# Weepingchestnut/SAVSR

Measured on NVIDIA B200. Metric: hr_mpix_per_s, higher is better.
Workload: dtype bf16

## Files before the change

### include/savsr_b200.h

```cpp
#ifndef SAVSR_B200_H_
#define SAVSR_B200_H_

#include <stddef.h>
#include <stdint.h>

#ifdef __cplusplus
extern "C" {
#endif

#define SAVSR_ABI_VERSION 4
#define SAVSR_MAX_SRC 5
#define SAVSR_MAX_GROUPS 25
#define SAVSR_TILE_W 8
#define SAVSR_TILE_H 16

typedef struct savsr_ctx savsr_ctx;
typedef struct savsr_arena savsr_arena;
typedef void* savsr_stream;

enum savsr_format { SAVSR_FMT_BF16 = 0, SAVSR_FMT_FP16 = 1 };
enum savsr_row_order { SAVSR_ROWS_LINEAR = 0, SAVSR_ROWS_QUAD = 1 };

enum savsr_act { SAVSR_ACT_NONE = 0, SAVSR_ACT_LRELU = 1, SAVSR_ACT_RELU = 2 };

enum savsr_dst_mode {
  SAVSR_DST_ARENA = 0,
  SAVSR_DST_AUX16 = 1
};

enum savsr_conv_impl {
  SAVSR_IMPL_TCGEN05_TAP = 0,
  SAVSR_IMPL_TCGEN05_HALO = 1,
  SAVSR_IMPL_CHECK = 2
};

typedef struct savsr_conv_group {
  int32_t src_slot[SAVSR_MAX_SRC];
  int32_t nsrc;
  int32_t dst_slot;
  int32_t res1_slot;
  int32_t res2_slot;
  float res2_scale;
  int32_t act;
  float slope;
  const void* weight;
  int64_t weight_sample_stride;
  const float* bias;
  const float* mask;
  float* pool;
  void* aux_dst;
  int32_t src_channels;
  int32_t reserved_;
} savsr_conv_group;

enum savsr_option {
  SAVSR_OPT_BIGK_ALL = 0,
  SAVSR_OPT_BIGK_ISSUERS = 1,
  SAVSR_OPT_PDL = 2,
  SAVSR_OPT_COUNT = 3
};

int savsr_abi_version(void);
const char* savsr_last_error(void);
int savsr_ctx_create(int device, savsr_ctx** out);
void savsr_ctx_destroy(savsr_ctx* ctx);
int savsr_ctx_sm_count(const savsr_ctx* ctx);
int savsr_ctx_set_format(savsr_ctx* ctx, int format);
int savsr_ctx_get_format(const savsr_ctx* ctx);
int savsr_ctx_set_option(savsr_ctx* ctx, int option, int value);
int savsr_ctx_get_option(const savsr_ctx* ctx, int option);

size_t savsr_arena_bytes(int nslots, int batch, int height, int width);
int savsr_arena_create(savsr_ctx* ctx, void* base, int nslots, int batch, int height, int width,
                       savsr_arena** out);
void savsr_arena_destroy(savsr_arena* a);
int savsr_arena_tiles(const savsr_arena* a);
int savsr_arena_import(savsr_arena* a, int slot, const float* nchw, savsr_stream st);
int savsr_arena_export(savsr_arena* a, int slot, float* nchw, savsr_stream st);

size_t savsr_packed_weight_bytes(int co, int ci, int ksize);
int savsr_pack_conv_weight(const float* w_oihw, int co_real, int co, int ci, int ksize, int n_tile,
                           int format , int row_order ,
                           void* packed, savsr_stream st);

int savsr_conv(savsr_ctx* ctx, savsr_arena* arena, const savsr_conv_group* groups, int ngroups,
               int ksize, int n_tile, int dst_mode, int impl, savsr_stream st);

int savsr_pack_frames(savsr_ctx* ctx, savsr_arena* arena, const float* x, int t, int h, int w, int dst_slot,
                      savsr_stream st);

int savsr_conv_wgrad(savsr_ctx* ctx, const void* x3_nchw16, const void* dy_nchw16, int batch, int ci, int height, int width,
                     int pitch, int per_sample, float* dw, savsr_stream st);

typedef struct savsr_axpby {
  int32_t dst_slot, x_slot, y_slot;
  float alpha, beta;
} savsr_axpby;
int savsr_slot_axpby(savsr_ctx* ctx, savsr_arena* arena, const savsr_axpby* entries, int n, savsr_stream st);

typedef struct savsr_grad_prep_entry {
  int32_t dv_slot, out_slot, g_slot, gt_tslot;
  int32_t act;
  float slope;
  const float* cscale; int64_t cscale_stride;
  const float* cadd; int64_t cadd_stride; float cadd_mul;
  int32_t reserved_;
  float* dbias;
} savsr_grad_prep_entry;
int savsr_grad_prep(savsr_ctx* ctx, savsr_arena* arena, void* tbase, int ntslots, int pitch, const savsr_grad_prep_entry* entries, int n,
                    savsr_stream st);

typedef struct savsr_nchw3 { int32_t x_slot, t_slot; } savsr_nchw3;
int savsr_slot_to_nchw3(savsr_ctx* ctx, savsr_arena* arena, void* tbase, int ntslots, int pitch, const savsr_nchw3* entries, int n,
                        savsr_stream st);

typedef struct savsr_pack_chunk {
  const float* w;
  void* dst;
  int32_t co_total, ci_total, o_base, i_base, ksize, transposed;
} savsr_pack_chunk;
int savsr_pack_conv_chunks(savsr_ctx* ctx, const savsr_pack_chunk* chunks_dev, int first, int count, savsr_stream st);

enum savsr_wgrad_layout {
  SAVSR_WGRAD_OIHW = 0,
  SAVSR_WGRAD_TIO = 1
};
typedef struct savsr_wgrad_item {
  int32_t x_tslot, g_tslot;
  float* dw;
  int32_t ci_total, ci_off, o_off, ksize, per_sample, layout;
  int64_t sample_stride;
} savsr_wgrad_item;
int savsr_conv_wgrad_batched(savsr_ctx* ctx, const void* tbase, int ntslots, int batch, int height, int width, int pitch,
                             const savsr_wgrad_item* items_dev, int first, int count, savsr_stream st);

int savsr_adam_ema(savsr_ctx* ctx, float* param, const float* grad, float* exp_avg, float* exp_avg_sq, float* ema, long n, float lr,
                   float beta1, float beta2, float eps, const float* step_dev, float ema_decay, float grad_scale, savsr_stream st);

typedef struct savsr_osa_params {
  int32_t ci, co, att;
  const float* bank;
  const float* r0_w; const float* r0_b;
  const float* r2_w; const float* r2_b;
  const float* fc_w;
  const float* bn_scale; const float* bn_shift;
  const float* ch_w; const float* ch_b;
  const float* fl_w; const float* fl_b;
  const float* sp_w; const float* sp_b;
  const float* kn_w; const float* kn_b;
  const float* pool[SAVSR_MAX_SRC];
  float* scratch;
  void* packed;
} savsr_osa_params;
int savsr_osa_prologue(savsr_ctx* ctx, const savsr_osa_params* convs, int nconvs, int batch,
                       int npart, int npix, float inv_scale_h, float inv_scale_w, savsr_stream st);

typedef struct savsr_osa_train {
  const float* bn_weight; const float* bn_bias;
  float* running_mean; float* running_var;
  float momentum, eps;
  float* state;
  void* packed_t;
} savsr_osa_train;
typedef struct savsr_osa_grads {
  float* dwfold;
  float* d_bank;
  float* d_r0_w; float* d_r0_b; float* d_r2_w; float* d_r2_b;
  float* d_fc_w; float* d_bn_w; float* d_bn_b;
  float* d_ch_w; float* d_ch_b; float* d_fl_w; float* d_fl_b; float* d_sp_w; float* d_sp_b; float* d_kn_w; float* d_kn_b;
  float* datt; float* dvec; float* dpool;
} savsr_osa_grads;
size_t savsr_osa_train_state_floats(int batch);
size_t savsr_osa_train_dvec_floats(int batch, int ci);
int savsr_osa_prologue_train(savsr_ctx* ctx, const savsr_osa_params* convs, const savsr_osa_train* extra, int nconvs, int batch,
                             int npart, int npix, float inv_scale_h, float inv_scale_w, savsr_stream st);
int savsr_osa_fold_backward(savsr_ctx* ctx, const savsr_osa_params* convs, const savsr_osa_train* extra, const savsr_osa_grads* grads,
                            int nconvs, int batch, savsr_stream st);

int savsr_slot_channel_dot(savsr_ctx* ctx, savsr_arena* arena, int a_slot, int b_slot, float* out, savsr_stream st);
int savsr_ca_backward(savsr_ctx* ctx, const float* pool, int npart, int npix, int batch, const float* w1, const float* b1, const float* w2,
                      const float* b2, const float* y, float* dy, float* dw1, float* db1, float* dw2, float* db2, float* dmean,
                      savsr_stream st);

typedef struct savsr_mask_train {
  const float *w4, *b4, *w7, *b7, *w11, *b11;
  const float* bn_w[4]; const float* bn_b[4];
  float* bn_rm[4]; float* bn_rv[4];
  const float* gamma;
  float momentum, eps;
  float *m0, *t2, *m4, *t3, *m7, *t5, *m11, *mask;
  float* stat; double* sums; float* coef;
  float *d_w4, *d_b4, *d_w7, *d_b7, *d_w11, *d_b11;
  float* d_bn_w[4]; float* d_bn_b[4];
  float* d_gamma;
  float *dmask, *dm11, *dt4, *dm7, *dt3, *dm4, *dt2;
} savsr_mask_train;
int savsr_mask_forward_train(savsr_ctx* ctx, savsr_arena* arena, const savsr_mask_train* m, int r_slot, int a_slot, int share_slot, int out_slot,
                             savsr_stream st);
int savsr_mask_backward_train(savsr_ctx* ctx, savsr_arena* arena, const savsr_mask_train* m, int dh_slot, int a_slot, int share_slot, int da_slot,
                              int gshare_slot, int dm0_slot, savsr_stream st);

int savsr_sta_lrelu_forward(savsr_ctx* ctx, const float* x, const float* kpre, float* out, int batch, int channels, int height, int width,
                            float slope, savsr_stream st);
int savsr_sta_lrelu_backward(savsr_ctx* ctx, const float* x, const float* kpre, const float* dout, float* dx, float* dkpre, int batch, int channels,
                             int height, int width, float slope, savsr_stream st);

int savsr_ca_scale_residual(savsr_ctx* ctx, savsr_arena* arena, int t_slot, int x_slot, int dst_slot,
                            const float* pool, int npart, const float* w1, const float* b1,
                            const float* w2, const float* b2, float* y_scratch , savsr_stream st);

int savsr_osadapt_mask(savsr_ctx* ctx, const float* in16, int batch, int height, int width,
                       const float* wa, const float* ba, const float* wb, const float* bb,
                       const float* wc, const float* bc, float* half0, float* half1, float* mask,
                       savsr_stream st);

typedef struct savsr_satu_weights {
  const float* body0_w; const float* body0_b;
  const float* body2_w; const float* body2_b;
  const float* routing_w; const float* routing_b;
  const float* offset_w; const float* offset_b;
  const float* st_offset_w; const float* st_offset_b;
  const float* compress;
  const float* expand;
} savsr_satu_weights;

int savsr_satu_index(savsr_ctx* ctx, const savsr_satu_weights* wts, int h, int w, int H, int W,
                     float s_h, float s_w, float* rel_y, float* rel_x, int32_t* cell_y,
                     int32_t* cell_x, float* base_y, float* base_x, int32_t* corner_y,
                     int32_t* corner_x, float* table, savsr_stream st);

int savsr_satu_kconv_sta(savsr_ctx* ctx, savsr_arena* arena, int a_slot, int x_slot, int dst_slot, int h, int w,
                         const void* weights, const float* bias, float slope, savsr_stream st);

int savsr_satu_hr(savsr_ctx* ctx, savsr_arena* lr, int x_slot, int sta_slot, int h, int w, int H, int W,
                  const float* table, const float* base_y, const float* base_x, const void* weights,
                  const float* zbias, const float* tail_bias, const float* x_in, int t, int centre, float* out,
                  savsr_stream st);

typedef struct savsr_plan savsr_plan;
int savsr_plan_create(savsr_ctx* ctx, savsr_plan** out);
void savsr_plan_destroy(savsr_plan* plan);
int savsr_plan_size(const savsr_plan* plan);
int savsr_plan_set_io(savsr_plan* plan, float* x_in, size_t x_bytes, float* out, size_t out_bytes, int format );
int savsr_plan_add_pack_frames(savsr_plan* plan, savsr_arena* arena, const float* x, int t, int h, int w, int dst_slot);
int savsr_plan_add_conv(savsr_plan* plan, savsr_arena* arena, const savsr_conv_group* groups, int ngroups, int ksize, int n_tile,
                        int dst_mode, int impl);
int savsr_plan_add_osa_prologue(savsr_plan* plan, const savsr_osa_params* convs, int nconvs, int batch, int npart, int npix,
                                float inv_scale_h, float inv_scale_w);
int savsr_plan_add_ca_scale_residual(savsr_plan* plan, savsr_arena* arena, int t_slot, int x_slot, int dst_slot, const float* pool, int npart,
                                     const float* w1, const float* b1, const float* w2, const float* b2, float* y_scratch);
int savsr_plan_add_osadapt_mask(savsr_plan* plan, const float* in16, int batch, int height, int width, const float* wa, const float* ba,
                                const float* wb, const float* bb, const float* wc, const float* bc, float* half0, float* half1, float* mask);
int savsr_plan_add_satu_kconv_sta(savsr_plan* plan, savsr_arena* arena, int a_slot, int x_slot, int dst_slot, int h, int w, const void* weights,
                                  const float* bias, float slope);
int savsr_plan_add_satu_hr(savsr_plan* plan, savsr_arena* lr, int x_slot, int sta_slot, int h, int w, int H, int W, const float* table,
                           const float* base_y, const float* base_x, const void* weights, const float* zbias, const float* tail_bias,
                           const float* x_in, int t, int centre, float* out);
int savsr_plan_add_arena_export(savsr_plan* plan, savsr_arena* arena, int slot, float* nchw);
int savsr_plan_run(savsr_plan* plan, savsr_stream st);
int savsr_forward(savsr_plan* plan, const float* x, float* out, savsr_stream st);

int savsr_img_metrics_blocks(const savsr_ctx* ctx, int height, int width);
int savsr_img_metrics(savsr_ctx* ctx, const float* sr, const float* gt, int batch, int height, int width,
                      uint8_t* bgr_u8, double* sse_y, savsr_stream st);

int savsr_ssim_y_blocks(int height, int width);
int savsr_ssim_y(savsr_ctx* ctx, const float* sr, const float* gt, int batch, int height, int width,
                 double* partials, savsr_stream st);

int savsr_aa_max_taps(int in_size, int out_size);
int savsr_aa_table(savsr_ctx* ctx, int in_size, int out_size, int max_taps, int32_t* xmin, int32_t* xsize,
                   float* weights, int32_t* overflow_flag, savsr_stream st);
int savsr_lr_synthesize(savsr_ctx* ctx, const uint8_t* frames_bgr, int nframes, int height, int width,
                        int crop_h, int crop_w, int out_h, int out_w,
                        const int32_t* xmin_w, const int32_t* xsize_w, const float* weights_w, int taps_w,
                        const int32_t* xmin_h, const int32_t* xsize_h, const float* weights_h, int taps_h,
                        float* tmp, float* lr, float* gt, savsr_stream st);
int savsr_resize_aa(savsr_ctx* ctx, const float* src, int nframes, int height, int width, int out_h, int out_w,
                    const int32_t* xmin_w, const int32_t* xsize_w, const float* weights_w, int taps_w,
                    const int32_t* xmin_h, const int32_t* xsize_h, const float* weights_h, int taps_h,
                    float* tmp, float* dst, savsr_stream st);

#ifdef __cplusplus
}
#endif
#endif
```

### savsr_b200/_capi.py

```python
from __future__ import annotations

import ctypes as C
import os
from typing import Optional

ABI_VERSION = 4
MAX_SRC = 5
MAX_GROUPS = 25
TILE_W, TILE_H = 8, 16

ACT_NONE, ACT_LRELU, ACT_RELU = 0, 1, 2
DST_ARENA, DST_AUX16 = 0, 1
IMPL_TAP, IMPL_HALO, IMPL_CHECK = 0, 1, 2
IMPL_NAMES = {"tap": IMPL_TAP, "halo": IMPL_HALO, "check": IMPL_CHECK}
FMT_BF16, FMT_FP16 = 0, 1
FMT_NAMES = {"bf16": FMT_BF16, "fp16": FMT_FP16}
OPT_BIGK_ALL, OPT_BIGK_ISSUERS, OPT_PDL = 0, 1, 2
WGRAD_OIHW, WGRAD_TIO = 0, 1
ROWS_LINEAR, ROWS_QUAD = 0, 1

LIB_PATH = os.environ.get("SAVSR_LIB_PATH") or os.path.join(os.path.dirname(os.path.abspath(__file__)), "lib", "libsavsr_sm100.so")


class SavsrError(RuntimeError):
    """A libsavsr_sm100 call returned non-zero."""


class ConvGroup(C.Structure):
    _fields_ = [
        ("src_slot", C.c_int32 * MAX_SRC),
        ("nsrc", C.c_int32),
        ("dst_slot", C.c_int32),
        ("res1_slot", C.c_int32),
        ("res2_slot", C.c_int32),
        ("res2_scale", C.c_float),
        ("act", C.c_int32),
        ("slope", C.c_float),
        ("weight", C.c_void_p),
        ("weight_sample_stride", C.c_int64),
        ("bias", C.c_void_p),
        ("mask", C.c_void_p),
        ("pool", C.c_void_p),
        ("aux_dst", C.c_void_p),
        ("src_channels", C.c_int32),
        ("reserved_", C.c_int32),
    ]


class OsaParams(C.Structure):
    _fields_ = [
        ("ci", C.c_int32), ("co", C.c_int32), ("att", C.c_int32),
        ("bank", C.c_void_p),
        ("r0_w", C.c_void_p), ("r0_b", C.c_void_p), ("r2_w", C.c_void_p), ("r2_b", C.c_void_p),
        ("fc_w", C.c_void_p), ("bn_scale", C.c_void_p), ("bn_shift", C.c_void_p),
        ("ch_w", C.c_void_p), ("ch_b", C.c_void_p), ("fl_w", C.c_void_p), ("fl_b", C.c_void_p),
        ("sp_w", C.c_void_p), ("sp_b", C.c_void_p), ("kn_w", C.c_void_p), ("kn_b", C.c_void_p),
        ("pool", C.c_void_p * MAX_SRC),
        ("scratch", C.c_void_p),
        ("packed", C.c_void_p),
    ]


class SatuWeights(C.Structure):
    _fields_ = [(n, C.c_void_p) for n in (
        "body0_w", "body0_b", "body2_w", "body2_b", "routing_w", "routing_b", "offset_w", "offset_b",
        "st_offset_w", "st_offset_b", "compress", "expand")]


class Axpby(C.Structure):
    _fields_ = [("dst_slot", C.c_int32), ("x_slot", C.c_int32), ("y_slot", C.c_int32), ("alpha", C.c_float), ("beta", C.c_float)]


class GradPrep(C.Structure):
    _fields_ = [("dv_slot", C.c_int32), ("out_slot", C.c_int32), ("g_slot", C.c_int32), ("gt_tslot", C.c_int32),
                ("act", C.c_int32), ("slope", C.c_float),
                ("cscale", C.c_void_p), ("cscale_stride", C.c_int64),
                ("cadd", C.c_void_p), ("cadd_stride", C.c_int64), ("cadd_mul", C.c_float), ("reserved_", C.c_int32),
                ("dbias", C.c_void_p)]


class Nchw3(C.Structure):
    _fields_ = [("x_slot", C.c_int32), ("t_slot", C.c_int32)]


class PackChunk(C.Structure):
    _fields_ = [("w", C.c_void_p), ("dst", C.c_void_p), ("co_total", C.c_int32), ("ci_total", C.c_int32), ("o_base", C.c_int32),
                ("i_base", C.c_int32), ("ksize", C.c_int32), ("transposed", C.c_int32)]


class WgradItem(C.Structure):
    _fields_ = [("x_tslot", C.c_int32), ("g_tslot", C.c_int32), ("dw", C.c_void_p), ("ci_total", C.c_int32), ("ci_off", C.c_int32),
                ("o_off", C.c_int32), ("ksize", C.c_int32), ("per_sample", C.c_int32), ("layout", C.c_int32),
                ("sample_stride", C.c_int64)]


class OsaTrain(C.Structure):
    _fields_ = [("bn_weight", C.c_void_p), ("bn_bias", C.c_void_p), ("running_mean", C.c_void_p), ("running_var", C.c_void_p),
                ("momentum", C.c_float), ("eps", C.c_float), ("state", C.c_void_p), ("packed_t", C.c_void_p)]


class OsaGrads(C.Structure):
    _fields_ = [(n, C.c_void_p) for n in (
        "dwfold", "d_bank", "d_r0_w", "d_r0_b", "d_r2_w", "d_r2_b", "d_fc_w", "d_bn_w", "d_bn_b", "d_ch_w", "d_ch_b", "d_fl_w", "d_fl_b",
        "d_sp_w", "d_sp_b", "d_kn_w", "d_kn_b", "datt", "dvec", "dpool")]


class MaskTrain(C.Structure):
    _fields_ = ([(n, C.c_void_p) for n in ("w4", "b4", "w7", "b7", "w11", "b11")]
                + [("bn_w", C.c_void_p * 4), ("bn_b", C.c_void_p * 4), ("bn_rm", C.c_void_p * 4), ("bn_rv", C.c_void_p * 4),
                   ("gamma", C.c_void_p), ("momentum", C.c_float), ("eps", C.c_float)]
                + [(n, C.c_void_p) for n in ("m0", "t2", "m4", "t3", "m7", "t5", "m11", "mask", "stat", "sums", "coef",
                                             "d_w4", "d_b4", "d_w7", "d_b7", "d_w11", "d_b11")]
                + [("d_bn_w", C.c_void_p * 4), ("d_bn_b", C.c_void_p * 4), ("d_gamma", C.c_void_p)]
                + [(n, C.c_void_p) for n in ("dmask", "dm11", "dt4", "dm7", "dt3", "dm4", "dt2")])

MAX_TRAIN_ENTRIES = 32


_VP, _I, _F, _SZ = C.c_void_p, C.c_int, C.c_float, C.c_size_t
SIGNATURES = {
    "savsr_abi_version": (_I, []),
    "savsr_last_error": (C.c_char_p, []),
    "savsr_ctx_create": (_I, [_I, C.POINTER(_VP)]),
    "savsr_ctx_destroy": (None, [_VP]),
    "savsr_ctx_sm_count": (_I, [_VP]),
    "savsr_ctx_set_format": (_I, [_VP, _I]),
    "savsr_ctx_get_format": (_I, [_VP]),
    "savsr_ctx_set_option": (_I, [_VP, _I, _I]),
    "savsr_ctx_get_option": (_I, [_VP, _I]),
    "savsr_arena_bytes": (_SZ, [_I, _I, _I, _I]),
    "savsr_arena_create": (_I, [_VP, _VP, _I, _I, _I, _I, C.POINTER(_VP)]),
    "savsr_arena_destroy": (None, [_VP]),
    "savsr_arena_tiles": (_I, [_VP]),
    "savsr_arena_import": (_I, [_VP, _I, _VP, _VP]),
    "savsr_arena_export": (_I, [_VP, _I, _VP, _VP]),
    "savsr_packed_weight_bytes": (_SZ, [_I, _I, _I]),
    "savsr_pack_conv_weight": (_I, [_VP, _I, _I, _I, _I, _I, _I, _I, _VP, _VP]),
    "savsr_conv": (_I, [_VP, _VP, C.POINTER(ConvGroup), _I, _I, _I, _I, _I, _VP]),
    "savsr_conv_wgrad": (_I, [_VP, _VP, _VP, _I, _I, _I, _I, _I, _I, _VP, _VP]),
    "savsr_slot_axpby": (_I, [_VP, _VP, C.POINTER(Axpby), _I, _VP]),
    "savsr_grad_prep": (_I, [_VP, _VP, _VP, _I, _I, C.POINTER(GradPrep), _I, _VP]),
    "savsr_slot_to_nchw3": (_I, [_VP, _VP, _VP, _I, _I, C.POINTER(Nchw3), _I, _VP]),
    "savsr_pack_conv_chunks": (_I, [_VP, _VP, _I, _I, _VP]),
    "savsr_conv_wgrad_batched": (_I, [_VP, _VP, _I, _I, _I, _I, _I, _VP, _I, _I, _VP]),
    "savsr_adam_ema": (_I, [_VP, _VP, _VP, _VP, _VP, _VP, C.c_long, _F, _F, _F, _F, _VP, _F, _F, _VP]),
    "savsr_osa_train_state_floats": (_SZ, [_I]),
    "savsr_osa_train_dvec_floats": (_SZ, [_I, _I]),
    "savsr_osa_prologue_train": (_I, [_VP, C.POINTER(OsaParams), C.POINTER(OsaTrain), _I, _I, _I, _I, _F, _F, _VP]),
    "savsr_osa_fold_backward": (_I, [_VP, C.POINTER(OsaParams), C.POINTER(OsaTrain), C.POINTER(OsaGrads), _I, _I, _VP]),
    "savsr_slot_channel_dot": (_I, [_VP, _VP, _I, _I, _VP, _VP]),
    "savsr_ca_backward": (_I, [_VP, _VP, _I, _I, _I] + [_VP] * 11 + [_VP]),
    "savsr_mask_forward_train": (_I, [_VP, _VP, C.POINTER(MaskTrain), _I, _I, _I, _I, _VP]),
    "savsr_mask_backward_train": (_I, [_VP, _VP, C.POINTER(MaskTrain), _I, _I, _I, _I, _I, _I, _VP]),
    "savsr_sta_lrelu_forward": (_I, [_VP, _VP, _VP, _VP, _I, _I, _I, _I, _F, _VP]),
    "savsr_sta_lrelu_backward": (_I, [_VP, _VP, _VP, _VP, _VP, _VP, _I, _I, _I, _I, _F, _VP]),
    "savsr_plan_create": (_I, [_VP, C.POINTER(_VP)]),
    "savsr_plan_destroy": (None, [_VP]),
    "savsr_plan_size": (_I, [_VP]),
    "savsr_plan_set_io": (_I, [_VP, _VP, _SZ, _VP, _SZ, _I]),
    "savsr_plan_add_pack_frames": (_I, [_VP, _VP, _VP, _I, _I, _I, _I]),
    "savsr_plan_add_conv": (_I, [_VP, _VP, C.POINTER(ConvGroup), _I, _I, _I, _I, _I]),
    "savsr_plan_add_osa_prologue": (_I, [_VP, C.POINTER(OsaParams), _I, _I, _I, _I, _F, _F]),
    "savsr_plan_add_ca_scale_residual": (_I, [_VP, _VP, _I, _I, _I, _VP, _I, _VP, _VP, _VP, _VP, _VP]),
    "savsr_plan_add_osadapt_mask": (_I, [_VP, _VP, _I, _I, _I, _VP, _VP, _VP, _VP, _VP, _VP, _VP, _VP, _VP]),
    "savsr_plan_add_satu_kconv_sta": (_I, [_VP, _VP, _I, _I, _I, _I, _I, _VP, _VP, _F]),
    "savsr_plan_add_satu_hr": (_I, [_VP, _VP, _I, _I, _I, _I, _I, _I, _VP, _VP, _VP, _VP, _VP, _VP, _VP, _I, _I, _VP]),
    "savsr_plan_add_arena_export": (_I, [_VP, _VP, _I, _VP]),
    "savsr_plan_run": (_I, [_VP, _VP]),
    "savsr_forward": (_I, [_VP, _VP, _VP, _VP]),
    "savsr_pack_frames": (_I, [_VP, _VP, _VP, _I, _I, _I, _I, _VP]),
    "savsr_osa_prologue": (_I, [_VP, C.POINTER(OsaParams), _I, _I, _I, _I, _F, _F, _VP]),
    "savsr_ca_scale_residual": (_I, [_VP, _VP, _I, _I, _I, _VP, _I, _VP, _VP, _VP, _VP, _VP, _VP]),
    "savsr_osadapt_mask": (_I, [_VP, _VP, _I, _I, _I, _VP, _VP, _VP, _VP, _VP, _VP, _VP, _VP, _VP, _VP]),
    "savsr_satu_index": (_I, [_VP, C.POINTER(SatuWeights), _I, _I, _I, _I, _F, _F] + [_VP] * 9 + [_VP]),
    "savsr_satu_kconv_sta": (_I, [_VP, _VP, _I, _I, _I, _I, _I, _VP, _VP, _F, _VP]),
    "savsr_satu_hr": (_I, [_VP, _VP, _I, _I, _I, _I, _I, _I, _VP, _VP, _VP, _VP, _VP, _VP, _VP, _I, _I, _VP, _VP]),
    "savsr_img_metrics_blocks": (_I, [_VP, _I, _I]),
    "savsr_img_metrics": (_I, [_VP, _VP, _VP, _I, _I, _I, _VP, _VP, _VP]),
    "savsr_ssim_y_blocks": (_I, [_I, _I]),
    "savsr_ssim_y": (_I, [_VP, _VP, _VP, _I, _I, _I, _VP, _VP]),
    "savsr_aa_max_taps": (_I, [_I, _I]),
    "savsr_aa_table": (_I, [_VP, _I, _I, _I, _VP, _VP, _VP, _VP, _VP]),
    "savsr_lr_synthesize": (_I, [_VP, _VP, _I, _I, _I, _I, _I, _I, _I, _VP, _VP, _VP, _I, _VP, _VP, _VP, _I, _VP, _VP, _VP, _VP]),
    "savsr_resize_aa": (_I, [_VP, _VP, _I, _I, _I, _I, _I, _VP, _VP, _VP, _I, _VP, _VP, _VP, _I, _VP, _VP, _VP]),
}

_lib: Optional[C.CDLL] = None


def load() -> C.CDLL:
    global _lib
    if _lib is not None:
        return _lib
    if not os.path.exists(LIB_PATH):
        raise SavsrError(
            f"{LIB_PATH} not found: build it with `python -m savsr_b200.build` (needs nvcc, sm_100a). "
            "savsr_b200 has no CPU or PyTorch fallback.")
    lib = C.CDLL(LIB_PATH)
    for name, (res, args) in SIGNATURES.items():
        fn = getattr(lib, name)
        fn.restype = res
        fn.argtypes = args
    if lib.savsr_abi_version() != ABI_VERSION:
        raise SavsrError(f"ABI version mismatch: library {lib.savsr_abi_version()}, binding {ABI_VERSION}")
    _lib = lib
    return lib


def check(rc: int) -> None:
    if rc != 0:
        msg = load().savsr_last_error()
        raise SavsrError(f"libsavsr_sm100 error {rc}: {msg.decode(errors='replace') if msg else '?'}")


class Context:

    def __init__(self, device: int):
        self.lib = load()
        h = C.c_void_p()
        check(self.lib.savsr_ctx_create(int(device), C.byref(h)))
        self.handle = h
        self.device = int(device)
        self.sm_count = self.lib.savsr_ctx_sm_count(h)

    def set_option(self, option: int, value: int) -> None:
        check(self.lib.savsr_ctx_set_option(self.handle, int(option), int(value)))

    def set_format(self, fmt: int) -> None:
        check(self.lib.savsr_ctx_set_format(self.handle, int(fmt)))

    def __del__(self):
        try:
            if getattr(self, "handle", None):
                self.lib.savsr_ctx_destroy(self.handle)
                self.handle = None
        except Exception:
            pass


class Arena:

    def __init__(self, ctx: Context, base_ptr: int, nslots: int, batch: int, height: int, width: int):
        self.ctx = ctx
        self.lib = ctx.lib
        h = C.c_void_p()
        check(self.lib.savsr_arena_create(ctx.handle, C.c_void_p(base_ptr), nslots, batch, height, width, C.byref(h)))
        self.handle = h
        self.nslots, self.batch, self.height, self.width = nslots, batch, height, width
        self.tiles = self.lib.savsr_arena_tiles(h)

    def __del__(self):
        try:
            if getattr(self, "handle", None):
                self.lib.savsr_arena_destroy(self.handle)
                self.handle = None
        except Exception:
            pass


class CPlan:

    def __init__(self, ctx: Context):
        self.lib = ctx.lib
        h = C.c_void_p()
        check(self.lib.savsr_plan_create(ctx.handle, C.byref(h)))
        self.handle = h

    def __len__(self) -> int:
        return int(self.lib.savsr_plan_size(self.handle))

    def __del__(self):
        try:
            if getattr(self, "handle", None):
                self.lib.savsr_plan_destroy(self.handle)
                self.handle = None
        except Exception:
            pass
```

### savsr_b200/csrc/capi.cu

```cuda
#include <cstdarg>
#include <cstdio>
#include <cstdlib>
#include <cstring>

#include "common.cuh"

namespace savsr {

static thread_local char g_err[512] = "";

void set_error(const char* fmt, ...) {
  va_list ap;
  va_start(ap, fmt);
  vsnprintf(g_err, sizeof(g_err), fmt, ap);
  va_end(ap);
}

int cuda_fail(cudaError_t e, const char* what) {
  set_error("CUDA error %d (%s) at %s", static_cast<int>(e), cudaGetErrorString(e), what);
  return 2;
}

typedef CUresult (*EncodeTiledFn)(CUtensorMap*, CUtensorMapDataType, cuuint32_t, void*, const cuuint64_t*, const cuuint64_t*,
                                  const cuuint32_t*, const cuuint32_t*, CUtensorMapInterleave, CUtensorMapSwizzle,
                                  CUtensorMapL2promotion, CUtensorMapFloatOOBfill);

static int encode_map(savsr_ctx* ctx, CUtensorMap* tm, void* base, int nimg, int height, int width, int bw, int bh) {
  const cuuint64_t dims[4] = {64, static_cast<cuuint64_t>(width), static_cast<cuuint64_t>(height), static_cast<cuuint64_t>(nimg)};
  const cuuint64_t strides[3] = {128, static_cast<cuuint64_t>(width) * 128, static_cast<cuuint64_t>(height) * width * 128};
  const cuuint32_t box[4] = {64, static_cast<cuuint32_t>(bw), static_cast<cuuint32_t>(bh), 1};
  const cuuint32_t estr[4] = {1, 1, 1, 1};
  const CUresult r = reinterpret_cast<EncodeTiledFn>(ctx->encode_tiled)(
      tm, CU_TENSOR_MAP_DATA_TYPE_UINT16, 4, base, dims, strides, box, estr, CU_TENSOR_MAP_INTERLEAVE_NONE,
      CU_TENSOR_MAP_SWIZZLE_128B, CU_TENSOR_MAP_L2_PROMOTION_L2_256B, CU_TENSOR_MAP_FLOAT_OOB_FILL_NONE);
  if (r != CUDA_SUCCESS) {
    set_error("cuTensorMapEncodeTiled failed with CUresult %d (images %d, %dx%d, box %dx%d)", static_cast<int>(r), nimg, height,
              width, bw, bh);
    return 3;
  }
  return 0;
}

}

using namespace savsr;

extern "C" int savsr_abi_version(void) { return SAVSR_ABI_VERSION; }
extern "C" const char* savsr_last_error(void) { return g_err; }

extern "C" int savsr_ctx_create(int device, savsr_ctx** out) {
  SAVSR_REQUIRE(out, "savsr_ctx_create: null output pointer");
  *out = nullptr;
  int count = 0;
  SAVSR_CUDA(cudaGetDeviceCount(&count));
  SAVSR_REQUIRE(device >= 0 && device < count, "savsr_ctx_create: device %d not present (%d CUDA devices)", device, count);
  cudaDeviceProp prop;
  SAVSR_CUDA(cudaGetDeviceProperties(&prop, device));
  SAVSR_REQUIRE(prop.major == 10, "savsr_ctx_create: device %d is sm_%d%d; this library contains sm_100a code only "
                "(tcgen05/TMEM/TMA) and has no fallback", device, prop.major, prop.minor);
  DeviceGuard guard(device);
  void* fn = nullptr;
  cudaDriverEntryPointQueryResult qres;
  SAVSR_CUDA(cudaGetDriverEntryPoint("cuTensorMapEncodeTiled", &fn, cudaEnableDefault, &qres));
  SAVSR_REQUIRE(qres == cudaDriverEntryPointSuccess && fn, "savsr_ctx_create: driver lacks cuTensorMapEncodeTiled");
  savsr_ctx* c = static_cast<savsr_ctx*>(calloc(1, sizeof(savsr_ctx)));
  SAVSR_REQUIRE(c, "savsr_ctx_create: out of host memory");
  c->device = device;
  c->sm_count = prop.multiProcessorCount;
  c->cc_major = prop.major;
  c->cc_minor = prop.minor;
  c->encode_tiled = fn;
  c->opt[SAVSR_OPT_BIGK_ALL] = 1;
  c->opt[SAVSR_OPT_BIGK_ISSUERS] = 2;
  *out = c;
  return 0;
}

extern "C" int savsr_ctx_set_format(savsr_ctx* ctx, int format) {
  SAVSR_REQUIRE(ctx, "savsr_ctx_set_format: null context");
  SAVSR_REQUIRE(format == SAVSR_FMT_BF16 || format == SAVSR_FMT_FP16, "savsr_ctx_set_format: unknown format %d", format);
  ctx->fmt = format;
  return 0;
}
extern "C" int savsr_ctx_get_format(const savsr_ctx* ctx) { return ctx ? ctx->fmt : -1; }

extern "C" int savsr_ctx_set_option(savsr_ctx* ctx, int option, int value) {
  SAVSR_REQUIRE(ctx, "savsr_ctx_set_option: null context");
  SAVSR_REQUIRE(option >= 0 && option < SAVSR_OPT_COUNT, "savsr_ctx_set_option: unknown option %d", option);
  if (option == SAVSR_OPT_BIGK_ALL) SAVSR_REQUIRE(value == 0 || value == 1, "savsr_ctx_set_option: BIGK_ALL must be 0 or 1, got %d", value);
  if (option == SAVSR_OPT_BIGK_ISSUERS) SAVSR_REQUIRE(value == 1 || value == 2, "savsr_ctx_set_option: BIGK_ISSUERS must be 1 or 2, got %d", value);
  if (option == SAVSR_OPT_PDL) SAVSR_REQUIRE(value == 0 || value == 1, "savsr_ctx_set_option: PDL must be 0 or 1, got %d", value);
  ctx->opt[option] = value;
  return 0;
}
extern "C" int savsr_ctx_get_option(const savsr_ctx* ctx, int option) {
  return (ctx && option >= 0 && option < SAVSR_OPT_COUNT) ? ctx->opt[option] : -1;
}

extern "C" void savsr_ctx_destroy(savsr_ctx* ctx) { free(ctx); }
extern "C" int savsr_ctx_sm_count(const savsr_ctx* ctx) { return ctx ? ctx->sm_count : 0; }

extern "C" size_t savsr_arena_bytes(int nslots, int batch, int height, int width) {
  if (nslots <= 0 || batch <= 0 || height <= 0 || width <= 0) return 0;
  return static_cast<size_t>(nslots) * batch * height * width * kC * sizeof(__nv_bfloat16);
}

extern "C" int savsr_arena_create(savsr_ctx* ctx, void* base, int nslots, int batch, int height, int width, savsr_arena** out) {
  SAVSR_REQUIRE(ctx && out, "savsr_arena_create: null pointer");
  *out = nullptr;
  DeviceGuard guard(ctx->device);
  SAVSR_REQUIRE(base && (reinterpret_cast<uintptr_t>(base) & 255) == 0, "savsr_arena_create: base must be a 256-byte aligned device pointer");
  SAVSR_REQUIRE(nslots > 0 && batch > 0 && height > 0 && width > 0, "savsr_arena_create: empty arena (%d slots, batch %d, %dx%d)", nslots,
                batch, height, width);
  savsr_arena* a = static_cast<savsr_arena*>(calloc(1, sizeof(savsr_arena)));
  SAVSR_REQUIRE(a, "savsr_arena_create: out of host memory");
  a->ctx = ctx;
  a->base = static_cast<__nv_bfloat16*>(base);
  a->nslots = nslots; a->batch = batch; a->height = height; a->width = width;
  a->tiles_x = (width + kTileW - 1) / kTileW;
  a->tiles_y = (height + kTileH - 1) / kTileH;
  int rc = encode_map(ctx, &a->tm_tile, base, nslots * batch, height, width, kTileW, kTileH);
  if (rc == 0) rc = encode_map(ctx, &a->tm_halo, base, nslots * batch, height, width, kTileW + 2, kTileH + 2);
  if (rc != 0) { free(a); return rc; }
  *out = a;
  return 0;
}

extern "C" void savsr_arena_destroy(savsr_arena* a) { free(a); }
extern "C" int savsr_arena_tiles(const savsr_arena* a) { return a ? a->tiles_x * a->tiles_y : 0; }
```

### savsr_b200/csrc/conv_igemm.cu

```cuda
#include <cstdio>
#include <cstdlib>

#include "common.cuh"

namespace savsr {

#ifdef SAVSR_DEBUG_COUNTERS
#define DBG_CLOCK() clock64()
#define DBG_ONLY(...) __VA_ARGS__
#else
#define DBG_CLOCK() 0ll
#define DBG_ONLY(...)
#endif

constexpr int kMaxAStages = 4;
constexpr int kHaloPitch = 10;
constexpr int kHaloStageBytes = 23552;
constexpr int kARegionBytes = 3 * kHaloStageBytes;
constexpr int kBBlocks = 18;
constexpr int kRing = 3;
constexpr int kEpiWarps = 8;
constexpr int kNumThreads = 64 + 32 * kEpiWarps;

struct ConvParams {
  CUtensorMap tm_tile;
  CUtensorMap tm_halo;
  savsr_conv_group g[SAVSR_MAX_GROUPS];
  __nv_bfloat16* arena;
  int ngroups, batch, height, width, tiles_x, tiles_y;
  int ntaps;
  int nsrc;
  int halo;
  int n_res;
  int chunk;
  uint32_t per_sample_mask;
  long long* dbg;
  int dst_mode;
  int fmt;
  int issuers;
  int ksteps;
};

__device__ __forceinline__ float apply_act(float v, int act, float slope) {
  if (act == SAVSR_ACT_LRELU) return v > 0.f ? v : v * slope;
  if (act == SAVSR_ACT_RELU) return fmaxf(v, 0.f);
  return v;
}

template <int NC>
struct EpiCtx {
  float bias[NC];
  uint4 r1[NC / 8], r2[NC / 8];
  float mk;
  long pix;
  bool valid;
  int bias_group;
  float neg_slope;
  float res2_scale;
  int res1_slot, res2_slot, dst_slot;
  bool has_mask;
  float* pool;
};

template <int NC>
__device__ __forceinline__ void epi_prefetch(const ConvParams& p, const savsr_conv_group& g, int gi, int n, int tile, int quad,
                                             int lane, int col0, EpiCtx<NC>& c) {
  const int tx = tile % p.tiles_x, ty = tile / p.tiles_x;
  const int m = quad * 32 + lane;
  const int px = tx * kTileW + (m & (kTileW - 1));
  const int py = ty * kTileH + (m >> 3);
  c.valid = (px < p.width) && (py < p.height);
  const long npix = static_cast<long>(p.height) * p.width;
  c.pix = static_cast<long>(py) * p.width + px;
  if (gi != c.bias_group) {
    c.bias_group = gi;
    c.neg_slope = g.act == SAVSR_ACT_NONE ? 1.f : (g.act == SAVSR_ACT_RELU ? 0.f : g.slope);
    c.res2_scale = g.res2_scale;
    c.res1_slot = g.res1_slot; c.res2_slot = g.res2_slot; c.dst_slot = g.dst_slot;
    c.has_mask = g.mask != nullptr;
    c.pool = g.pool;
    if (g.bias != nullptr) {
      const float4* b4 = reinterpret_cast<const float4*>(g.bias + col0);
#pragma unroll
      for (int j = 0; j < NC / 4; ++j) {
        const float4 b = __ldg(b4 + j);
        c.bias[4 * j + 0] = b.x; c.bias[4 * j + 1] = b.y; c.bias[4 * j + 2] = b.z; c.bias[4 * j + 3] = b.w;
      }
    } else {
#pragma unroll
      for (int j = 0; j < NC; ++j) c.bias[j] = 0.f;
    }
  }
  if constexpr (NC == 32) {
    c.mk = (c.has_mask && c.valid) ? __ldg(g.mask + n * npix + c.pix) : 0.f;
    if (c.res1_slot >= 0 && c.valid) {
      const uint4* r = reinterpret_cast<const uint4*>(p.arena + ((static_cast<long>(c.res1_slot) * p.batch + n) * npix + c.pix) * kC + col0);
#pragma unroll
      for (int j = 0; j < NC / 8; ++j) c.r1[j] = r[j];
    }
    if (c.res2_slot >= 0 && c.valid) {
      const uint4* r = reinterpret_cast<const uint4*>(p.arena + ((static_cast<long>(c.res2_slot) * p.batch + n) * npix + c.pix) * kC + col0);
#pragma unroll
      for (int j = 0; j < NC / 8; ++j) c.r2[j] = r[j];
    }
  }
}

__device__ __forceinline__ void add_h16x8(float* v, const uint4& u, float s, int fmt) {
  v[0] += s * h_lo(u.x, fmt); v[1] += s * h_hi(u.x, fmt); v[2] += s * h_lo(u.y, fmt); v[3] += s * h_hi(u.y, fmt);
  v[4] += s * h_lo(u.z, fmt); v[5] += s * h_hi(u.z, fmt); v[6] += s * h_lo(u.w, fmt); v[7] += s * h_hi(u.w, fmt);
}

template <int NC>
__device__ __forceinline__ void epi_finish(const ConvParams& p, const savsr_conv_group& g, int n, int tile, int quad, int lane,
                                           float (&v)[NC], int col0, const EpiCtx<NC>& c) {
  const long npix = static_cast<long>(p.height) * p.width;
  const float ns = c.neg_slope;
#pragma unroll
  for (int j = 0; j < NC; ++j) {
    const float t = v[j] + c.bias[j];
    v[j] = fmaxf(t, ns * t);
  }
  if constexpr (NC == 32) {
    if (c.has_mask) {
#pragma unroll
      for (int j = 0; j < NC; ++j) v[j] *= c.mk;
    }
    if (c.res1_slot >= 0 && c.valid) {
#pragma unroll
      for (int j = 0; j < NC / 8; ++j) add_h16x8(v + 8 * j, c.r1[j], 1.f, p.fmt);
    }
    if (c.res2_slot >= 0 && c.valid) {
      const float r2s = c.res2_scale;
#pragma unroll
      for (int j = 0; j < NC / 8; ++j) add_h16x8(v + 8 * j, c.r2[j], r2s, p.fmt);
    }
    if (c.valid) {
      uint4* d = reinterpret_cast<uint4*>(p.arena + ((static_cast<long>(c.dst_slot) * p.batch + n) * npix + c.pix) * kC + col0);
#pragma unroll
      for (int j = 0; j < NC / 8; ++j) {
        uint4 u;
        u.x = pack_h2(v[8 * j + 0], v[8 * j + 1], p.fmt);
        u.y = pack_h2(v[8 * j + 2], v[8 * j + 3], p.fmt);
        u.z = pack_h2(v[8 * j + 4], v[8 * j + 5], p.fmt);
        u.w = pack_h2(v[8 * j + 6], v[8 * j + 7], p.fmt);
        d[j] = u;
      }
    }
    if (c.pool != nullptr) {
      if (!c.valid) {
#pragma unroll
        for (int j = 0; j < NC; ++j) v[j] = 0.f;
      }
#pragma unroll
      for (int off = 16, cnt = 16; off >= 1; off >>= 1, cnt >>= 1) {
        const bool upper = (lane & off) != 0;
#pragma unroll
        for (int i = 0; i < cnt; ++i) {
          const float send = upper ? v[i] : v[i + cnt];
          const float keep = upper ? v[i + cnt] : v[i];
          v[i] = keep + __shfl_xor_sync(0xffffffffu, send, off);
        }
      }
      const int npart = p.tiles_x * p.tiles_y * 4;
      c.pool[(static_cast<long>(n) * npart + tile * 4 + quad) * kC + col0 + lane] = v[0];
    }
  } else {
    if (c.valid) {
      float4* d = reinterpret_cast<float4*>(static_cast<float*>(g.aux_dst) + (n * npix + c.pix) * 16);
#pragma unroll
      for (int j = 0; j < 4; ++j) d[j] = make_float4(v[4 * j], v[4 * j + 1], v[4 * j + 2], v[4 * j + 3]);
    }
  }
}


struct EpiQuad {
  float bias[8];
  uint4 r1[4], r2[4];
  float mk[4];
  long pix0;
  uint32_t valid;
  int bias_group;
  float neg_slope, res2_scale;
  int res1_slot, res2_slot, dst_slot;
  bool has_mask;
  float* pool;
  float psum[8];
};

__device__ __forceinline__ void epiq_prefetch(const ConvParams& p, const savsr_conv_group& g, int gi, int n, int tile, int quad,
                                              int lane, int half, EpiQuad& c) {
  const int tx = tile % p.tiles_x, ty = tile / p.tiles_x;
  const int px = tx * kTileW + (lane >> 2);
  const int py0 = ty * kTileH + quad * 4;
  const int rows = p.height - py0;
  c.valid = (px < p.width && rows > 0) ? (rows >= 4 ? 0xfu : ((1u << rows) - 1u)) : 0u;
  const long npix = static_cast<long>(p.height) * p.width;
  c.pix0 = static_cast<long>(py0) * p.width + px;
  const int ch0 = half * 32 + (lane & 3) * 8;
  if (gi != c.bias_group) {
    c.bias_group = gi;
    c.neg_slope = g.act == SAVSR_ACT_NONE ? 1.f : (g.act == SAVSR_ACT_RELU ? 0.f : g.slope);
    c.res2_scale = g.res2_scale;
    c.res1_slot = g.res1_slot; c.res2_slot = g.res2_slot; c.dst_slot = g.dst_slot;
    c.has_mask = g.mask != nullptr;
    c.pool = g.pool;
    if (g.bias != nullptr) {
      const float4 b0 = __ldg(reinterpret_cast<const float4*>(g.bias + ch0));
      const float4 b1 = __ldg(reinterpret_cast<const float4*>(g.bias + ch0) + 1);
      c.bias[0] = b0.x; c.bias[1] = b0.y; c.bias[2] = b0.z; c.bias[3] = b0.w;
      c.bias[4] = b1.x; c.bias[5] = b1.y; c.bias[6] = b1.z; c.bias[7] = b1.w;
    } else {
#pragma unroll
      for (int j = 0; j < 8; ++j) c.bias[j] = 0.f;
    }
  }
  if (c.has_mask) {
#pragma unroll
    for (int j = 0; j < 4; ++j) c.mk[j] = ((c.valid >> j) & 1u) ? __ldg(g.mask + n * npix + c.pix0 + j * p.width) : 0.f;
  }
  if (c.res1_slot >= 0) {
    const __nv_bfloat16* r = p.arena + ((static_cast<long>(c.res1_slot) * p.batch + n) * npix + c.pix0) * kC + ch0;
#pragma unroll
    for (int j = 0; j < 4; ++j)
      if ((c.valid >> j) & 1u) c.r1[j] = *reinterpret_cast<const uint4*>(r + static_cast<long>(j) * p.width * kC);
  }
  if (c.res2_slot >= 0) {
    const __nv_bfloat16* r = p.arena + ((static_cast<long>(c.res2_slot) * p.batch + n) * npix + c.pix0) * kC + ch0;
#pragma unroll
    for (int j = 0; j < 4; ++j)
      if ((c.valid >> j) & 1u) c.r2[j] = *reinterpret_cast<const uint4*>(r + static_cast<long>(j) * p.width * kC);
  }
}

template <class Release, class Next>
__device__ __forceinline__ void epiq_finish(const ConvParams& p, int n, int tile, int quad, int lane, int half, uint32_t taddr,
                                            EpiQuad& c, bool last_of_run, Release release, Next next) {
  uint32_t ra[16], rb[16];
  tmem_ld_16x256b_x4(taddr, ra);
  tmem_ld_16x256b_x4(taddr + (16u << 16), rb);
  tmem_ld_wait();
  tc_fence_before();
  __syncwarp();
  release();
  float v[4][8];
#pragma unroll
  for (int k = 0; k < 4; ++k) {
#pragma unroll
    for (int e = 0; e < 4; ++e) {
      v[e >> 1][2 * k + (e & 1)] = __uint_as_float(ra[4 * k + e]);
      v[2 + (e >> 1)][2 * k + (e & 1)] = __uint_as_float(rb[4 * k + e]);
    }
  }
  const long npix = static_cast<long>(p.height) * p.width;
  const int ch0 = half * 32 + (lane & 3) * 8;
  const float ns = c.neg_slope;
#pragma unroll
  for (int j = 0; j < 4; ++j) {
#pragma unroll
    for (int i = 0; i < 8; ++i) {
      const float t = v[j][i] + c.bias[i];
      v[j][i] = fmaxf(t, ns * t);
    }
  }
  if (c.has_mask) {
#pragma unroll
    for (int j = 0; j < 4; ++j) {
#pragma unroll
      for (int i = 0; i < 8; ++i) v[j][i] *= c.mk[j];
    }
  }
  if (c.res1_slot >= 0) {
#pragma unroll
    for (int j = 0; j < 4; ++j)
      if ((c.valid >> j) & 1u) add_h16x8(v[j], c.r1[j], 1.f, p.fmt);
  }
  if (c.res2_slot >= 0) {
    const float r2s = c.res2_scale;
#pragma unroll
    for (int j = 0; j < 4; ++j)
      if ((c.valid >> j) & 1u) add_h16x8(v[j], c.r2[j], r2s, p.fmt);
  }
  const uint32_t valid = c.valid;
  float* const pool = c.pool;
  __nv_bfloat16* d = p.arena + ((static_cast<long>(c.dst_slot) * p.batch + n) * npix + c.pix0) * kC + ch0;
  next();
#pragma unroll
  for (int j = 0; j < 4; ++j) {
    if ((valid >> j) & 1u) {
      uint4 u;
      u.x = pack_h2(v[j][0], v[j][1], p.fmt);
      u.y = pack_h2(v[j][2], v[j][3], p.fmt);
      u.z = pack_h2(v[j][4], v[j][5], p.fmt);
      u.w = pack_h2(v[j][6], v[j][7], p.fmt);
      *reinterpret_cast<uint4*>(d + static_cast<long>(j) * p.width * kC) = u;
    }
  }
  if (pool != nullptr) {
    if (valid == 0xfu) {
#pragma unroll
      for (int i = 0; i < 8; ++i) c.psum[i] += (v[0][i] + v[1][i]) + (v[2][i] + v[3][i]);
    } else {
#pragma unroll
      for (int i = 0; i < 8; ++i) {
        const float a0 = (valid & 1u) ? v[0][i] : 0.f, a1 = (valid & 2u) ? v[1][i] : 0.f;
        const float a2 = (valid & 4u) ? v[2][i] : 0.f, a3 = (valid & 8u) ? v[3][i] : 0.f;
        c.psum[i] += (a0 + a1) + (a2 + a3);
      }
    }
    const int npart = p.tiles_x * p.tiles_y * 4;
    const int ch = ch0 + ((lane >> 4) & 1) * 4 + ((lane >> 3) & 1) * 2 + ((lane >> 2) & 1);
    float total = 0.f;
    if (last_of_run) {
      float s[8];
#pragma unroll
      for (int i = 0; i < 8; ++i) { s[i] = c.psum[i]; c.psum[i] = 0.f; }
#pragma unroll
      for (int off = 16, cnt = 4; off >= 4; off >>= 1, cnt >>= 1) {
        const bool upper = (lane & off) != 0;
#pragma unroll
        for (int i = 0; i < cnt; ++i) {
          const float send = upper ? s[i] : s[i + cnt];
          const float keep = upper ? s[i + cnt] : s[i];
          s[i] = keep + __shfl_xor_sync(0xffffffffu, send, off);
        }
      }
      total = s[0];
    }
    pool[(static_cast<long>(n) * npart + tile * 4 + quad) * kC + ch] = total;
  }
}

__device__ __forceinline__ constexpr uint32_t desc_hi(uint32_t sbo_bytes) { return (sbo_bytes >> 4) | (1u << 14) | (2u << 29); }
__device__ __forceinline__ uint64_t make_desc(uint32_t hi, uint32_t lo) { return (static_cast<uint64_t>(hi) << 32) | lo; }

template <int BN, int KS, bool HALO>
__global__ void __launch_bounds__(kNumThreads, 1) conv_igemm_kernel(const __grid_constant__ ConvParams p) {
  constexpr int NT = KS * KS;
  extern __shared__ uint8_t smem_raw[];
  uint8_t* smem = reinterpret_cast<uint8_t*>((reinterpret_cast<uintptr_t>(smem_raw) + 1023) & ~static_cast<uintptr_t>(1023));
  constexpr int kBBytes = BN * 128;
  constexpr int kAStage = HALO ? kHaloStageBytes : kTileM * 128;
  constexpr int kAStages = HALO ? 3 : 4;
  uint8_t* smem_a = smem;
  uint8_t* smem_b = smem + kARegionBytes;
  uint8_t* smem_ring = smem_b + (kBBlocks - kRing) * kBBytes;
  uint64_t* bars = reinterpret_cast<uint64_t*>(smem_b + kBBlocks * kBBytes);
  uint64_t* a_full = bars;
  uint64_t* a_empty = a_full + kMaxAStages;
  uint64_t* res_full = a_empty + kMaxAStages;
  uint64_t* ring_full = res_full + kBBlocks;
  uint64_t* ring_empty = ring_full + kRing;
  uint64_t* res_free = ring_empty + kRing;
  uint64_t* t_full = res_free + 1;
  uint64_t* t_empty = t_full + 2;
  uint32_t* tmem_slot = reinterpret_cast<uint32_t*>(t_empty + 2);

  const int warp = threadIdx.x >> 5;
  const int lane = threadIdx.x & 31;
  const int tiles = p.tiles_x * p.tiles_y;
  const int total = p.ngroups * p.batch * tiles;
  const int item_begin = blockIdx.x * p.chunk;
  const int item_end = min(item_begin + p.chunk, total);
  const int nsrc = p.nsrc;
  const int n_res = p.n_res;
  constexpr int kTmemCols = 2 * BN < 32 ? 32 : 2 * BN;
  constexpr int kEpiArrivals = BN == 64 ? 8 : 4;

  if (warp == 0 && lane == 0) {
    prefetch_tensormap(HALO ? &p.tm_halo : &p.tm_tile);
    for (int i = 0; i < kMaxAStages; ++i) { mbar_init(a_full + i, 1); mbar_init(a_empty + i, 1); }
    for (int i = 0; i < kBBlocks; ++i) mbar_init(res_full + i, 1);
    for (int i = 0; i < kRing; ++i) { mbar_init(ring_full + i, 1); mbar_init(ring_empty + i, 1); }
    mbar_init(res_free, 1);
    for (int i = 0; i < 2; ++i) { mbar_init(t_full + i, 1); mbar_init(t_empty + i, kEpiArrivals); }
    fence_barrier_init();
  }
  if (warp == 1) tmem_alloc<kTmemCols>(tmem_slot);
  tc_fence_before();
  __syncthreads();
  tc_fence_after();
  const uint32_t tmem_base = *tmem_slot;

  if (warp == 0) {
    if (lane == 0) {
      int sa = 0, pa = 0, sr = 0, pr = 0;
      int gen = -1, cur_key = -1;
      long long dbg_ae = 0;
      const int nkb = nsrc * NT;
      int tile = item_begin % tiles;
      int gn = item_begin / tiles;
      for (int item = item_begin; item < item_end; ++item) {
        const int n = gn % p.batch;
        const int gi = gn / p.batch;
        const savsr_conv_group& g = p.g[gi];
        const int ty = tile / p.tiles_x;
        const int x0 = (tile - ty * p.tiles_x) * kTileW, y0 = ty * kTileH;
        const uint8_t* wptr = static_cast<const uint8_t*>(g.weight) + static_cast<long>(n) * g.weight_sample_stride;
        const int key = gi * p.batch + (g.weight_sample_stride != 0 ? n : 0);
        if (key != cur_key) {
          if (gen >= 0) mbar_wait(res_free, gen & 1);
          ++gen;
          cur_key = key;
          int kb = blockIdx.x % nkb;
          for (int i = 0; i < nkb; ++i) {
            if (kb < n_res) {
              mbar_expect_tx(res_full + kb, kBBytes);
              bulk_load(smem_b + kb * kBBytes, wptr + static_cast<long>(kb) * kBBytes, kBBytes, res_full + kb);
            }
            if (++kb == nkb) kb = 0;
          }
        }
        for (int s = 0; s < nsrc; ++s) {
          const int img = g.src_slot[s] * p.batch + n;
          if constexpr (HALO) {
            const long long c0 = DBG_CLOCK();
            mbar_wait(a_empty + sa, pa ^ 1);
            dbg_ae += DBG_CLOCK() - c0;
            mbar_expect_tx(a_full + sa, kHaloPitch * (kTileH + 2) * 128u);
            tma_load_4d(smem_a + sa * kAStage, &p.tm_halo, a_full + sa, 0, x0 - 1, y0 - 1, img);
            if (++sa == kAStages) { sa = 0; pa ^= 1; }
          }
#pragma unroll
          for (int tap = 0; tap < NT; ++tap) {
            const int kb = s * NT + tap;
            if constexpr (!HALO) {
              const int dx = KS == 3 ? tap % 3 - 1 : 0;
              const int dy = KS == 3 ? tap / 3 - 1 : 0;
              mbar_wait(a_empty + sa, pa ^ 1);
              mbar_expect_tx(a_full + sa, kTileM * 128u);
              tma_load_4d(smem_a + sa * kAStage, &p.tm_tile, a_full + sa, 0, x0 + dx, y0 + dy, img);
              if (++sa == kAStages) { sa = 0; pa ^= 1; }
            }
            if (kb >= n_res) {
              mbar_wait(ring_empty + sr, pr ^ 1);
              mbar_expect_tx(ring_full + sr, kBBytes);
              bulk_load(smem_ring + sr * kBBytes, wptr + static_cast<long>(kb) * kBBytes, kBBytes, ring_full + sr);
              if (++sr == kRing) { sr = 0; pr ^= 1; }
            }
          }
        }
        if (++tile == tiles) { tile = 0; ++gn; }
      }
      DBG_ONLY(if (p.dbg != nullptr) p.dbg[blockIdx.x * 8 + 6] = dbg_ae;)
      (void)dbg_ae;
    }
  } else if (warp == 1) {
    const uint32_t idesc = umma_idesc_f16(BN, p.fmt);
    constexpr uint32_t a_hi = desc_hi(HALO ? kHaloPitch * 128u : 1024u);
    constexpr uint32_t b_hi = desc_hi(1024u);
    const uint32_t a_lo0 = (smem_u32(smem_a) >> 4) & 0x3fffu;
    const uint32_t b_lo0 = (smem_u32(smem_b) >> 4) & 0x3fffu;
    const uint32_t ring_lo0 = (smem_u32(smem_ring) >> 4) & 0x3fffu;
    const bool all_resident = nsrc * NT <= n_res;
    int sa = 0, pa = 0, sr = 0, pr = 0;
    int gen = -1, cur_key = -1;
    int it = 0;
    int tile = item_begin % tiles;
    int n = (item_begin / tiles) % p.batch;
    int gi = (item_begin / tiles) / p.batch;
    const uint32_t ps_mask = p.per_sample_mask;
    const int batch = p.batch;
    long long dbg_te = 0, dbg_af = 0, dbg_t0 = DBG_CLOCK();
    for (int item = item_begin; item < item_end; ++item, ++it) {
      const int key = gi * batch + (((ps_mask >> gi) & 1u) ? n : 0);
      bool fresh = false;
      if (key != cur_key) {
        if (gen >= 0 && elect_one()) umma_commit(res_free);
        __syncwarp();
        ++gen;
        cur_key = key;
        fresh = true;
      }
      const int acc = it & 1;
      long long c0 = DBG_CLOCK();
      mbar_wait(t_empty + acc, ((it >> 1) & 1) ^ 1);
      dbg_te += DBG_CLOCK() - c0;
      tc_fence_after();
      const uint32_t d_tmem = tmem_base + static_cast<uint32_t>(acc * BN);
      if (HALO && all_resident && !fresh) {
        uint32_t b_lo = b_lo0;
        for (int s = 0; s < nsrc; ++s) {
          c0 = DBG_CLOCK();
          mbar_wait(a_full + sa, pa);
          dbg_af += DBG_CLOCK() - c0;
          tc_fence_after();
          const uint32_t al0 = a_lo0 + sa * (kAStage >> 4);
          if (elect_one()) {
#pragma unroll
            for (int tap = 0; tap < NT; ++tap) {
              const uint32_t al = al0 + ((tap / 3) * kHaloPitch + tap % 3) * 8;
              const uint32_t bl = b_lo + tap * (kBBytes >> 4);
#pragma unroll
              for (int k = 0; k < 4; ++k)
                umma_bf16(d_tmem, make_desc(a_hi, al + 2 * k), make_desc(b_hi, bl + 2 * k), idesc, (s | tap | k) ? 1u : 0u);
            }
            umma_commit(a_empty + sa);
          }
          __syncwarp();
          b_lo += NT * (kBBytes >> 4);
          if (++sa == kAStages) { sa = 0; pa ^= 1; }
        }
      } else {
        uint32_t accumulate = 0;
        uint32_t b_lo = b_lo0;
        int kb = 0;
        for (int s = 0; s < nsrc; ++s) {
          if constexpr (HALO) {
            mbar_wait(a_full + sa, pa);
            tc_fence_after();
          }
#pragma unroll
          for (int tap = 0; tap < NT; ++tap, ++kb, b_lo += kBBytes >> 4) {
            if constexpr (!HALO) {
              mbar_wait(a_full + sa, pa);
              tc_fence_after();
            }
            uint32_t bl = b_lo;
            const bool streamed = kb >= n_res;
            if (streamed) {
              mbar_wait(ring_full + sr, pr);
              tc_fence_after();
              bl = ring_lo0 + sr * (kBBytes >> 4);
            } else if (fresh) {
              mbar_wait(res_full + kb, gen & 1);
              tc_fence_after();
            }
            const uint32_t al = a_lo0 + sa * (kAStage >> 4) + (HALO ? ((tap / 3) * kHaloPitch + tap % 3) * 8 : 0);
            if (elect_one()) {
#pragma unroll
              for (int k = 0; k < 4; ++k) {
                umma_bf16(d_tmem, make_desc(a_hi, al + 2 * k), make_desc(b_hi, bl + 2 * k), idesc, accumulate);
                accumulate = 1;
              }
              if (streamed) umma_commit(ring_empty + sr);
              if (!HALO) umma_commit(a_empty + sa);
            }
            __syncwarp();
            accumulate = 1;
            if (streamed) {
              if (++sr == kRing) { sr = 0; pr ^= 1; }
            }
            if constexpr (!HALO) {
              if (++sa == kAStages) { sa = 0; pa ^= 1; }
            }
          }
          if constexpr (HALO) {
            if (elect_one()) umma_commit(a_empty + sa);
            __syncwarp();
            if (++sa == kAStages) { sa = 0; pa ^= 1; }
          }
        }
      }
      if (elect_one()) umma_commit(t_full + acc);
      __syncwarp();
      if (++tile == tiles) {
        tile = 0;
        if (++n == batch) { n = 0; ++gi; }
      }
    }
    DBG_ONLY(if (p.dbg != nullptr && lane == 0) {
      p.dbg[blockIdx.x * 8 + 0] = DBG_CLOCK() - dbg_t0;
      p.dbg[blockIdx.x * 8 + 1] = dbg_te;
      p.dbg[blockIdx.x * 8 + 2] = dbg_af;
      p.dbg[blockIdx.x * 8 + 3] = item_end - item_begin;
    })
    (void)dbg_te; (void)dbg_af; (void)dbg_t0;
  } else {
    const int quad = warp & 3;
    const int half = (warp - 2) >> 2;
    if (BN == 64 || half == 0) {
      constexpr int NC = 16;
      EpiCtx<NC> ec;
      EpiQuad eq;
      ec.bias_group = -1;
      eq.bias_group = -1;
#pragma unroll
      for (int i = 0; i < 8; ++i) eq.psum[i] = 0.f;
      int it = 0;
      int tile = item_begin % tiles;
      int gn = item_begin / tiles;
      long long dbg_tf = 0, dbg_t0 = DBG_CLOCK();
      if constexpr (BN == 64) {
        if (item_begin < item_end) epiq_prefetch(p, p.g[gn / p.batch], gn / p.batch, gn % p.batch, tile, quad, lane, half, eq);
      }
      for (int item = item_begin; item < item_end; ++item, ++it) {
        const int n = gn % p.batch;
        const int gi = gn / p.batch;
        const savsr_conv_group& g = p.g[gi];
        const int acc = it & 1;
        if constexpr (BN != 64) epi_prefetch<NC>(p, g, gi, n, tile, quad, lane, 0, ec);
        const long long c0 = DBG_CLOCK();
        mbar_wait(t_full + acc, (it >> 1) & 1);
        dbg_tf += DBG_CLOCK() - c0;
        tc_fence_after();
        const uint32_t taddr = tmem_base + (static_cast<uint32_t>(quad * 32) << 16) + static_cast<uint32_t>(acc * BN + half * 32);
        if constexpr (BN == 64) {
          epiq_finish(p, n, tile, quad, lane, half, taddr, eq, item + 1 >= item_end || tile + 1 == tiles,
                      [&] { if (lane == 0) mbar_arrive(t_empty + acc); }, [&] {
            if (item + 1 < item_end) {
              const int nt = tile + 1 == tiles ? 0 : tile + 1, ngn = tile + 1 == tiles ? gn + 1 : gn;
              epiq_prefetch(p, p.g[ngn / p.batch], ngn / p.batch, ngn % p.batch, nt, quad, lane, half, eq);
            }
          });
        } else {
          float v[NC];
          uint32_t r[16];
          tmem_ld16(taddr, r);
          tmem_ld_wait();
#pragma unroll
          for (int c = 0; c < 16; ++c) v[c] = __uint_as_float(r[c]);
          tc_fence_before();
          __syncwarp();
          if (lane == 0) mbar_arrive(t_empty + acc);
          epi_finish<NC>(p, g, n, tile, quad, lane, v, 0, ec);
        }
        if (++tile == tiles) { tile = 0; ++gn; }
      }
      DBG_ONLY(if (p.dbg != nullptr && warp == 2 && lane == 0) {
        p.dbg[blockIdx.x * 8 + 4] = DBG_CLOCK() - dbg_t0;
        p.dbg[blockIdx.x * 8 + 5] = dbg_tf;
      })
      (void)dbg_tf; (void)dbg_t0;
    }
  }

  tc_fence_before();
  __syncthreads();
  if (warp == 1) {
    tc_fence_after();
    tmem_dealloc<kTmemCols>(tmem_base);
  }
}

constexpr int kBatchTiles = 4;

constexpr int kBigkThreads = kNumThreads + 32;

__global__ void __launch_bounds__(kBigkThreads, 1) conv_igemm_bigk_kernel(const __grid_constant__ ConvParams p) {
  constexpr int BN = 64, NT = 9;
  constexpr int kBBytes = BN * 128;
  constexpr int kAStage = kHaloStageBytes, kAStages = 3;
  constexpr int kSetBlocks = 9, kSetBytes = kSetBlocks * kBBytes;
  extern __shared__ uint8_t smem_raw[];
  uint8_t* smem = reinterpret_cast<uint8_t*>((reinterpret_cast<uintptr_t>(smem_raw) + 1023) & ~static_cast<uintptr_t>(1023));
  uint8_t* smem_a = smem;
  uint8_t* smem_b = smem + kARegionBytes;
  uint64_t* bars = reinterpret_cast<uint64_t*>(smem_b + 2 * kSetBytes);
  uint64_t* a_full = bars;
  uint64_t* a_empty = a_full + kMaxAStages;
  uint64_t* set_full = a_empty + kMaxAStages;
  uint64_t* set_empty = set_full + 2;
  uint64_t* t_full = set_empty + 2;
  uint64_t* t_empty = t_full + 2 * kBatchTiles;
  uint32_t* tmem_slot = reinterpret_cast<uint32_t*>(t_empty + 2 * kBatchTiles);

  const int warp = threadIdx.x >> 5;
  const int lane = threadIdx.x & 31;
  const int tiles = p.tiles_x * p.tiles_y;
  const int total = p.ngroups * p.batch * tiles;
  const int item_begin = blockIdx.x * p.chunk;
  const int item_end = min(item_begin + p.chunk, total);
  const int nsrc = p.nsrc;
  const bool pinned = nsrc <= 2;
  const uint32_t ps_mask = p.per_sample_mask;

  if (warp == 0 && lane == 0) {
    prefetch_tensormap(&p.tm_halo);
    for (int i = 0; i < kMaxAStages; ++i) { mbar_init(a_full + i, 1); mbar_init(a_empty + i, p.issuers); }
    for (int i = 0; i < 2; ++i) { mbar_init(set_full + i, 1); mbar_init(set_empty + i, p.issuers); }
    for (int i = 0; i < 2 * kBatchTiles; ++i) { mbar_init(t_full + i, 1); mbar_init(t_empty + i, 8); }
    fence_barrier_init();
  }
  if (warp == 1) tmem_alloc<512>(tmem_slot);
  tc_fence_before();
  __syncthreads();
  tc_fence_after();
  const uint32_t tmem_base = *tmem_slot;
  pdl_wait();
  pdl_trigger();

  int item = item_begin;
  int tile = item_begin % tiles;
  int gn = item_begin / tiles;
  int bcount = 0;
  uint32_t use_bits = 0;
  uint32_t set_loads[2] = {0, 0};
  int cur_key = -1;

  if (warp == 0) {
    if (lane == 0) {
      int sa = 0, pa = 0;
      uint32_t u = 0;
      while (item < item_end) {
        const int cnt = min(kBatchTiles, min(item_end - item, tiles - tile));
        const int n = gn % p.batch;
        const int gi = gn / p.batch;
        const savsr_conv_group& g = p.g[gi];
        const uint8_t* wptr = static_cast<const uint8_t*>(g.weight) + static_cast<long>(n) * g.weight_sample_stride;
        const int key = gi * p.batch + (((ps_mask >> gi) & 1u) ? n : 0);
        const bool load = !pinned || key != cur_key;
        cur_key = key;
        for (int s = 0; s < nsrc; ++s) {
          if (load) {
            const int set = pinned ? s : static_cast<int>(u++ & 1);
            mbar_wait(set_empty + set, (set_loads[set] & 1u) ^ 1u);
            ++set_loads[set];
            mbar_expect_tx(set_full + set, kSetBytes);
            int kb = blockIdx.x % kSetBlocks;
            for (int i = 0; i < kSetBlocks; ++i) {
              bulk_load(smem_b + set * kSetBytes + kb * kBBytes, wptr + static_cast<long>(s * NT + kb) * kBBytes, kBBytes, set_full + set);
              if (++kb == kSetBlocks) kb = 0;
            }
          }
          const int img = g.src_slot[s] * p.batch + n;
          for (int j = 0; j < cnt; ++j) {
            const int tj = tile + j;
            const int ty = tj / p.tiles_x;
            mbar_wait(a_empty + sa, pa ^ 1);
            mbar_expect_tx(a_full + sa, kHaloPitch * (kTileH + 2) * 128u);
            tma_load_4d(smem_a + sa * kAStage, &p.tm_halo, a_full + sa, 0, (tj - ty * p.tiles_x) * kTileW - 1, ty * kTileH - 1, img);
            if (++sa == kAStages) { sa = 0; pa ^= 1; }
          }
        }
        item += cnt; tile += cnt;
        if (tile == tiles) { tile = 0; ++gn; }
      }
    }
  } else if (warp == 1 || (warp == 10 && p.issuers == 2)) {
    const int my = warp == 1 ? 0 : 1;
    const int own_mask = p.issuers == 2 ? 1 : 0;
    const uint32_t idesc = umma_idesc_f16(BN, p.fmt);
    constexpr uint32_t a_hi = desc_hi(kHaloPitch * 128u);
    constexpr uint32_t b_hi = desc_hi(1024u);
    const uint32_t a_lo0 = (smem_u32(smem_a) >> 4) & 0x3fffu;
    const uint32_t b_lo0 = (smem_u32(smem_b) >> 4) & 0x3fffu;
    int sa = 0, pa = 0;
    uint32_t u = 0;
    long long dbg_te = 0, dbg_af = 0, dbg_sf = 0, dbg_t0 = DBG_CLOCK(), c0;
    while (item < item_end) {
      const int cnt = min(kBatchTiles, min(item_end - item, tiles - tile));
      const int bb = bcount & 1;
      const int n = gn % p.batch;
      const int gi = gn / p.batch;
      const int key = gi * p.batch + (((ps_mask >> gi) & 1u) ? n : 0);
      const bool load = !pinned || key != cur_key;
      if (pinned && load && cur_key >= 0) {
        if (elect_one()) {
          for (int s = 0; s < nsrc; ++s) umma_commit(set_empty + s);
        }
        __syncwarp();
      }
      cur_key = key;
      c0 = DBG_CLOCK();
#pragma unroll
      for (int j = 0; j < kBatchTiles; ++j) {
        if (j < cnt && (j & own_mask) == my) mbar_wait(t_empty + bb * kBatchTiles + j, ((use_bits >> (bb * kBatchTiles + j)) & 1u) ^ 1u);
      }
      dbg_te += DBG_CLOCK() - c0;
      tc_fence_after();
      for (int s = 0; s < nsrc; ++s) {
        const int set = pinned ? s : static_cast<int>(u & 1);
        if (load) {
          c0 = DBG_CLOCK();
          mbar_wait(set_full + set, set_loads[set] & 1u);
          dbg_sf += DBG_CLOCK() - c0;
          ++set_loads[set];
          tc_fence_after();
          ++u;
        }
        const uint32_t bl0 = b_lo0 + set * (kSetBytes >> 4);
#pragma unroll
        for (int j = 0; j < kBatchTiles; ++j) {
          if (j < cnt) {
            c0 = DBG_CLOCK();
            mbar_wait(a_full + sa, pa);
            dbg_af += DBG_CLOCK() - c0;
            if ((j & own_mask) != my) {
              if (elect_one()) mbar_arrive(a_empty + sa);
              __syncwarp();
            } else {
              tc_fence_after();
              const uint32_t al0 = a_lo0 + sa * (kAStage >> 4);
              const uint32_t d_tmem = tmem_base + static_cast<uint32_t>((bb * kBatchTiles + j) * BN);
              if (elect_one()) {
                uint32_t al = al0, bl = bl0, acc = s ? 1u : 0u;
                if (p.ksteps == 4) {
#pragma unroll 1
                  for (int dy = 0; dy < 3; ++dy) {
#pragma unroll
                    for (int dx = 0; dx < 3; ++dx) {
#pragma unroll
                      for (int k = 0; k < 4; ++k) {
                        umma_bf16(d_tmem, make_desc(a_hi, al + dx * 8 + 2 * k), make_desc(b_hi, bl + dx * (kBBytes >> 4) + 2 * k), idesc, acc);
                        acc = 1u;
                      }
                    }
                    al += kHaloPitch * 8;
                    bl += 3 * (kBBytes >> 4);
                  }
                } else {
#pragma unroll 1
                  for (int dy = 0; dy < 3; ++dy) {
#pragma unroll
                    for (int dx = 0; dx < 3; ++dx) {
#pragma unroll 1
                      for (int k = 0; k < p.ksteps; ++k) {
                        umma_bf16(d_tmem, make_desc(a_hi, al + dx * 8 + 2 * k), make_desc(b_hi, bl + dx * (kBBytes >> 4) + 2 * k), idesc, acc);
                        acc = 1u;
                      }
                    }
                    al += kHaloPitch * 8;
                    bl += 3 * (kBBytes >> 4);
                  }
                }
                umma_commit(a_empty + sa);
                if (s == nsrc - 1) umma_commit(t_full + bb * kBatchTiles + j);
              }
              __syncwarp();
            }
            if (++sa == kAStages) { sa = 0; pa ^= 1; }
          }
        }
        if (!pinned) {
          if (elect_one()) umma_commit(set_empty + set);
          __syncwarp();
        }
      }
#pragma unroll
      for (int j = 0; j < kBatchTiles; ++j)
        if (j < cnt) use_bits ^= 1u << (bb * kBatchTiles + j);
      ++bcount;
      item += cnt; tile += cnt;
      if (tile == tiles) { tile = 0; ++gn; }
    }
    DBG_ONLY(if (p.dbg != nullptr && lane == 0 && my == 0) {
      p.dbg[blockIdx.x * 8 + 0] = DBG_CLOCK() - dbg_t0;
      p.dbg[blockIdx.x * 8 + 1] = dbg_te;
      p.dbg[blockIdx.x * 8 + 2] = dbg_af;
      p.dbg[blockIdx.x * 8 + 3] = item_end - item_begin;
      p.dbg[blockIdx.x * 8 + 7] = dbg_sf;
    })
    (void)dbg_te; (void)dbg_af; (void)dbg_sf; (void)dbg_t0;
  } else if (warp < 10) {
    const int quad = warp & 3;
    const int half = (warp - 2) >> 2;
    EpiQuad eq;
    eq.bias_group = -1;
#pragma unroll
    for (int i = 0; i < 8; ++i) eq.psum[i] = 0.f;
    long long dbg_tf = 0, dbg_t0 = DBG_CLOCK();
    if (item < item_end) epiq_prefetch(p, p.g[gn / p.batch], gn / p.batch, gn % p.batch, tile, quad, lane, half, eq);
    while (item < item_end) {
      const int cnt = min(kBatchTiles, min(item_end - item, tiles - tile));
      const int bb = bcount & 1;
      const int n = gn % p.batch;
      for (int j = 0; j < cnt; ++j) {
        const int acc = bb * kBatchTiles + j;
        const long long c0 = DBG_CLOCK();
        mbar_wait(t_full + acc, (use_bits >> acc) & 1u);
        dbg_tf += DBG_CLOCK() - c0;
        use_bits ^= 1u << acc;
        tc_fence_after();
        const uint32_t taddr = tmem_base + (static_cast<uint32_t>(quad * 32) << 16) + static_cast<uint32_t>(acc * BN + half * 32);
        epiq_finish(p, n, tile + j, quad, lane, half, taddr, eq, item + j + 1 >= item_end || tile + j + 1 == tiles,
                    [&] { if (lane == 0) mbar_arrive(t_empty + acc); }, [&] {
          if (item + j + 1 < item_end) {
            const int nt = tile + j + 1 == tiles ? 0 : tile + j + 1, ngn = tile + j + 1 == tiles ? gn + 1 : gn;
            epiq_prefetch(p, p.g[ngn / p.batch], ngn / p.batch, ngn % p.batch, nt, quad, lane, half, eq);
          }
        });
      }
      ++bcount;
      item += cnt; tile += cnt;
      if (tile == tiles) { tile = 0; ++gn; }
    }
    DBG_ONLY(if (p.dbg != nullptr && warp == 2 && lane == 0) {
      p.dbg[blockIdx.x * 8 + 4] = DBG_CLOCK() - dbg_t0;
      p.dbg[blockIdx.x * 8 + 5] = dbg_tf;
    })
    (void)dbg_tf; (void)dbg_t0;
  }

  tc_fence_before();
  __syncthreads();
  if (warp == 1) {
    tc_fence_after();
    tmem_dealloc<512>(tmem_base);
  }
}

template <int BN>
__global__ void __launch_bounds__(128) conv_check_kernel(const __grid_constant__ ConvParams p) {
  const int tiles = p.tiles_x * p.tiles_y;
  const int item = blockIdx.x;
  const int tile = item % tiles;
  const int gn = item / tiles;
  const int n = gn % p.batch;
  const int gi = gn / p.batch;
  const savsr_conv_group& g = p.g[gi];
  const int m = threadIdx.x;
  const int px = (tile % p.tiles_x) * kTileW + (m & 7);
  const int py = (tile / p.tiles_x) * kTileH + (m >> 3);
  const long npix = static_cast<long>(p.height) * p.width;
  const uint8_t* wptr = static_cast<const uint8_t*>(g.weight) + static_cast<long>(n) * g.weight_sample_stride;
  constexpr int NC = BN == 64 ? 32 : 16;
  for (int col0 = 0; col0 < BN; col0 += NC) {
    float v[NC];
#pragma unroll
    for (int c = 0; c < NC; ++c) v[c] = 0.f;
    for (int s = 0; s < g.nsrc; ++s) {
      const __nv_bfloat16* src = p.arena + (static_cast<long>(g.src_slot[s]) * p.batch + n) * npix * kC;
      for (int tap = 0; tap < p.ntaps; ++tap) {
        const int dx = p.ntaps == 9 ? tap % 3 - 1 : 0, dy = p.ntaps == 9 ? tap / 3 - 1 : 0;
        const int sx = px + dx, sy = py + dy;
        const bool in = sx >= 0 && sx < p.width && sy >= 0 && sy < p.height;
        const uint8_t* wb = wptr + static_cast<long>(s * p.ntaps + tap) * (BN * 128);
        for (int k = 0; k < 64; ++k) {
          const float a = in ? h_to_float(reinterpret_cast<const uint16_t*>(src)[(static_cast<long>(sy) * p.width + sx) * kC + k], p.fmt) : 0.f;
#pragma unroll
          for (int c = 0; c < NC; ++c) {
            const int row = BN == 64 ? quad_row(col0 + c) : col0 + c;
            const int off = row * 128 + (((k >> 3) ^ (row & 7)) << 4) + (k & 7) * 2;
            v[c] += a * h_to_float(*reinterpret_cast<const uint16_t*>(wb + off), p.fmt);
          }
        }
      }
    }
    EpiCtx<NC> ec;
    ec.bias_group = -1;
    epi_prefetch<NC>(p, g, gi, n, tile, m >> 5, m & 31, col0, ec);
    epi_finish<NC>(p, g, n, tile, m >> 5, m & 31, v, col0, ec);
  }
}

__global__ void pack_weight_kernel(const float* __restrict__ w, int co_real, int co, int ci, int ks, int n_tile, int fmt, int quad,
                                   uint16_t* __restrict__ out) {
  const long total = static_cast<long>(co) * ci * ks * ks;
  const int taps = ks * ks;
  for (long idx = blockIdx.x * static_cast<long>(blockDim.x) + threadIdx.x; idx < total;
       idx += static_cast<long>(gridDim.x) * blockDim.x) {
    const int k = idx & 63;
    long r = idx >> 6;
    const int n = r % n_tile; r /= n_tile;
    const int kb = r % ((ci / 64) * taps);
    const int ng = r / ((ci / 64) * taps);
    const int s = kb / taps, tap = kb % taps;
    const int o = ng * n_tile + (quad ? quad_row(n) : n), i = s * 64 + k;
    const float val = o < co_real ? w[(static_cast<long>(o) * ci + i) * taps + tap] : 0.f;
    const long block = static_cast<long>(ng) * ((ci / 64) * taps) + kb;
    const long off = block * (n_tile * 64) + n * 64 + ((((k >> 3) ^ (n & 7)) << 3) | (k & 7));
    out[off] = float_to_h(val, fmt);
  }
}

__global__ void arena_import_kernel(const float* __restrict__ nchw, uint16_t* __restrict__ dst, int batch, long npix, int fmt) {
  const long total = static_cast<long>(batch) * npix * kC;
  for (long idx = blockIdx.x * static_cast<long>(blockDim.x) + threadIdx.x; idx < total;
       idx += static_cast<long>(gridDim.x) * blockDim.x) {
    const int c = idx & 63;
    const long pn = idx >> 6;
    const long pix = pn % npix, n = pn / npix;
    dst[idx] = float_to_h(nchw[(n * kC + c) * npix + pix], fmt);
  }
}
__global__ void arena_export_kernel(const uint16_t* __restrict__ src, float* __restrict__ nchw, int batch, long npix, int fmt) {
  const long total = static_cast<long>(batch) * npix * kC;
  for (long idx = blockIdx.x * static_cast<long>(blockDim.x) + threadIdx.x; idx < total;
       idx += static_cast<long>(gridDim.x) * blockDim.x) {
    const long pix = idx % npix;
    const long nc = idx / npix;
    const int c = nc % kC;
    const long n = nc / kC;
    nchw[idx] = h_to_float(src[(n * npix + pix) * kC + c], fmt);
  }
}

template <int BN, int KS, bool HALO>
static int launch_igemm(savsr_ctx* ctx, ConvParams& p, int total, cudaStream_t st) {
  const size_t smem = 1024 + kARegionBytes + kBBlocks * BN * 128 + 512;
  constexpr int variant = (BN == 64 ? 0 : 3) + (KS == 1 ? 0 : (HALO ? 1 : 2));
  if (int rc = ensure_smem_attr(ctx, kAttrIgemm + variant, conv_igemm_kernel<BN, KS, HALO>, smem)) return rc;
  p.chunk = (total + ctx->sm_count - 1) / ctx->sm_count;
  const int grid = (total + p.chunk - 1) / p.chunk;
  conv_igemm_kernel<BN, KS, HALO><<<grid, kNumThreads, smem, st>>>(p);
  SAVSR_CUDA(cudaGetLastError());
  return 0;
}

template <int BN>
static int launch_conv(savsr_ctx* ctx, ConvParams& p, int impl, cudaStream_t st) {
  const int total = p.ngroups * p.batch * p.tiles_x * p.tiles_y;
  if (total == 0) return 0;
  if (impl == SAVSR_IMPL_CHECK) {
    conv_check_kernel<BN><<<total, 128, 0, st>>>(p);
    SAVSR_CUDA(cudaGetLastError());
    return 0;
  }
  if (p.ntaps == 1) return launch_igemm<BN, 1, false>(ctx, p, total, st);
  if constexpr (BN == 64) {
    if (p.halo && (ctx->opt[SAVSR_OPT_BIGK_ALL] || p.nsrc * p.ntaps > kBBlocks)) {
      const size_t smem = 1024 + kARegionBytes + kBBlocks * BN * 128 + 512;
      if (int rc = ensure_smem_attr(ctx, kAttrBigk, conv_igemm_bigk_kernel, smem)) return rc;
      p.chunk = (total + ctx->sm_count - 1) / ctx->sm_count;
      const int grid = (total + p.chunk - 1) / p.chunk;
      SAVSR_CUDA(launch_k(ctx->opt[SAVSR_OPT_PDL] != 0, conv_igemm_bigk_kernel, dim3(grid), dim3(kBigkThreads), smem, st, p));
      return 0;
    }
  }
  if (p.halo) return launch_igemm<BN, 3, true>(ctx, p, total, st);
  return launch_igemm<BN, 3, false>(ctx, p, total, st);
}

}

using namespace savsr;

#ifdef SAVSR_DEBUG_COUNTERS
extern "C" void savsr_debug_conv_counters(savsr_ctx* ctx, long long* dev_buf) { if (ctx) ctx->conv_dbg = dev_buf; }
#endif

extern "C" size_t savsr_packed_weight_bytes(int co, int ci, int ksize) {
  return static_cast<size_t>(co) * ci * ksize * ksize * sizeof(__nv_bfloat16);
}

extern "C" int savsr_pack_conv_weight(const float* w_oihw, int co_real, int co, int ci, int ksize, int n_tile, int format,
                                      int row_order, void* packed, savsr_stream st) {
  SAVSR_REQUIRE(format == SAVSR_FMT_BF16 || format == SAVSR_FMT_FP16, "savsr_pack_conv_weight: unknown format %d", format);
  SAVSR_REQUIRE(row_order == SAVSR_ROWS_LINEAR || row_order == SAVSR_ROWS_QUAD, "savsr_pack_conv_weight: unknown row_order %d", row_order);
  SAVSR_REQUIRE(w_oihw && packed, "savsr_pack_conv_weight: null pointer");
  SAVSR_REQUIRE(ksize == 1 || ksize == 3, "savsr_pack_conv_weight: ksize must be 1 or 3, got %d", ksize);
  SAVSR_REQUIRE(n_tile == 64 || n_tile == 16, "savsr_pack_conv_weight: n_tile must be 64 or 16, got %d", n_tile);
  SAVSR_REQUIRE(ci > 0 && ci % 64 == 0, "savsr_pack_conv_weight: ci (%d) must be a positive multiple of 64", ci);
  SAVSR_REQUIRE(co > 0 && co % n_tile == 0 && co_real <= co && co_real > 0,
                "savsr_pack_conv_weight: co (%d) must be a multiple of n_tile (%d) and >= co_real (%d)", co, n_tile, co_real);
  const long total = static_cast<long>(co) * ci * ksize * ksize;
  const int blocks = static_cast<int>((total + 255) / 256 < 2048 ? (total + 255) / 256 : 2048);
  pack_weight_kernel<<<blocks, 256, 0, static_cast<cudaStream_t>(st)>>>(w_oihw, co_real, co, ci, ksize, n_tile, format,
                                                                       (n_tile == 64 && row_order == SAVSR_ROWS_QUAD) ? 1 : 0,
                                                                       static_cast<uint16_t*>(packed));
  SAVSR_CUDA(cudaGetLastError());
  return 0;
}

extern "C" int savsr_arena_import(savsr_arena* a, int slot, const float* nchw, savsr_stream st) {
  SAVSR_REQUIRE(a && nchw, "savsr_arena_import: null pointer");
  SAVSR_REQUIRE(slot >= 0 && slot < a->nslots, "savsr_arena_import: slot %d out of range [0,%d)", slot, a->nslots);
  const long npix = static_cast<long>(a->height) * a->width;
  arena_import_kernel<<<1024, 256, 0, static_cast<cudaStream_t>(st)>>>(
      nchw, reinterpret_cast<uint16_t*>(a->base + static_cast<long>(slot) * a->batch * npix * kC), a->batch, npix, a->ctx->fmt);
  SAVSR_CUDA(cudaGetLastError());
  return 0;
}

extern "C" int savsr_arena_export(savsr_arena* a, int slot, float* nchw, savsr_stream st) {
  SAVSR_REQUIRE(a && nchw, "savsr_arena_export: null pointer");
  SAVSR_REQUIRE(slot >= 0 && slot < a->nslots, "savsr_arena_export: slot %d out of range [0,%d)", slot, a->nslots);
  const long npix = static_cast<long>(a->height) * a->width;
  arena_export_kernel<<<1024, 256, 0, static_cast<cudaStream_t>(st)>>>(
      reinterpret_cast<const uint16_t*>(a->base + static_cast<long>(slot) * a->batch * npix * kC), nchw, a->batch, npix, a->ctx->fmt);
  SAVSR_CUDA(cudaGetLastError());
  return 0;
}

extern "C" int savsr_conv(savsr_ctx* ctx, savsr_arena* arena, const savsr_conv_group* groups, int ngroups, int ksize,
                          int n_tile, int dst_mode, int impl, savsr_stream st) {
  SAVSR_REQUIRE(ctx && arena && groups, "savsr_conv: null pointer");
  DeviceGuard guard(ctx->device);
  SAVSR_REQUIRE(ngroups >= 0 && ngroups <= SAVSR_MAX_GROUPS, "savsr_conv: ngroups %d out of range [0,%d]", ngroups, SAVSR_MAX_GROUPS);
  SAVSR_REQUIRE(ksize == 1 || ksize == 3, "savsr_conv: ksize must be 1 or 3, got %d", ksize);
  SAVSR_REQUIRE(impl >= SAVSR_IMPL_TCGEN05_TAP && impl <= SAVSR_IMPL_CHECK, "savsr_conv: unknown impl %d", impl);
  SAVSR_REQUIRE((n_tile == 64 && dst_mode == SAVSR_DST_ARENA) || (n_tile == 16 && dst_mode == SAVSR_DST_AUX16),
                "savsr_conv: n_tile %d does not match dst_mode %d", n_tile, dst_mode);
  if (ngroups == 0) return 0;

  ConvParams p;
  memset(&p, 0, sizeof(p));
  p.tm_tile = arena->tm_tile;
  p.tm_halo = arena->tm_halo;
  for (int i = 0; i < ngroups; ++i) {
    const savsr_conv_group& g = groups[i];
    SAVSR_REQUIRE(g.nsrc >= 1 && g.nsrc <= SAVSR_MAX_SRC, "savsr_conv: group %d nsrc %d out of range", i, g.nsrc);
    SAVSR_REQUIRE(g.weight != nullptr, "savsr_conv: group %d has no weights", i);
    SAVSR_REQUIRE(g.nsrc == groups[0].nsrc, "savsr_conv: all groups of a launch must have the same nsrc (%d vs %d)", g.nsrc, groups[0].nsrc);
    SAVSR_REQUIRE(g.src_channels == groups[0].src_channels && g.src_channels >= 0 && g.src_channels <= 64 && g.src_channels % 16 == 0,
                  "savsr_conv: src_channels (%d) must be 0, 16, 32, 48 or 64 and equal for all groups of a launch", g.src_channels);
    SAVSR_REQUIRE(g.act != SAVSR_ACT_LRELU || (g.slope >= 0.f && g.slope <= 1.f), "savsr_conv: group %d LeakyReLU slope %g outside [0, 1]", i, g.slope);
    for (int s = 0; s < g.nsrc; ++s) {
      SAVSR_REQUIRE(g.src_slot[s] >= 0 && g.src_slot[s] < arena->nslots, "savsr_conv: group %d source slot %d out of range", i, g.src_slot[s]);
      SAVSR_REQUIRE(dst_mode != SAVSR_DST_ARENA || g.src_slot[s] != g.dst_slot, "savsr_conv: group %d writes slot %d that it also convolves", i, g.dst_slot);
    }
    if (dst_mode == SAVSR_DST_ARENA) {
      SAVSR_REQUIRE(g.dst_slot >= 0 && g.dst_slot < arena->nslots, "savsr_conv: group %d dst slot %d out of range", i, g.dst_slot);
      SAVSR_REQUIRE(g.res1_slot < arena->nslots && g.res2_slot < arena->nslots, "savsr_conv: group %d residual slot out of range", i);
    } else {
      SAVSR_REQUIRE(g.aux_dst != nullptr, "savsr_conv: group %d needs aux_dst for dst_mode %d", i, dst_mode);
    }
    p.g[i] = g;
  }
  p.arena = arena->base;
  p.ngroups = ngroups;
  p.batch = arena->batch;
  p.height = arena->height;
  p.width = arena->width;
  p.tiles_x = arena->tiles_x;
  p.tiles_y = arena->tiles_y;
  p.ntaps = ksize * ksize;
  p.halo = (impl == SAVSR_IMPL_TCGEN05_HALO && ksize == 3) ? 1 : 0;
  p.nsrc = groups[0].nsrc;
  for (int i = 0; i < ngroups; ++i) if (groups[i].weight_sample_stride != 0) p.per_sample_mask |= 1u << i;
  const int nkb = p.nsrc * p.ntaps;
  p.n_res = nkb <= kBBlocks ? nkb : kBBlocks - kRing;
  p.dst_mode = dst_mode;
  p.fmt = ctx->fmt;
  p.dbg = ctx->conv_dbg;
  p.issuers = ctx->opt[SAVSR_OPT_BIGK_ISSUERS];
  p.ksteps = groups[0].src_channels ? groups[0].src_channels / 16 : 4;
  if (n_tile == 64) return launch_conv<64>(ctx, p, impl, static_cast<cudaStream_t>(st));
  return launch_conv<16>(ctx, p, impl, static_cast<cudaStream_t>(st));
}
```

### savsr_b200/csrc/plan.cu

```cuda
#include <functional>
#include <vector>

#include "common.cuh"

struct savsr_plan {
  savsr_ctx* ctx;
  std::vector<std::function<int(savsr_stream)>> ops;
  float* x_in = nullptr;
  float* out = nullptr;
  size_t x_bytes = 0, out_bytes = 0;
  int format = SAVSR_FMT_BF16;
};

using namespace savsr;

extern "C" int savsr_plan_create(savsr_ctx* ctx, savsr_plan** out) {
  SAVSR_REQUIRE(ctx && out, "savsr_plan_create: null pointer");
  savsr_plan* p = new (std::nothrow) savsr_plan();
  SAVSR_REQUIRE(p, "savsr_plan_create: out of host memory");
  p->ctx = ctx;
  p->format = ctx->fmt;
  *out = p;
  return 0;
}
extern "C" void savsr_plan_destroy(savsr_plan* plan) { delete plan; }
extern "C" int savsr_plan_size(const savsr_plan* plan) { return plan ? static_cast<int>(plan->ops.size()) : 0; }

extern "C" int savsr_plan_set_io(savsr_plan* plan, float* x_in, size_t x_bytes, float* out, size_t out_bytes, int format) {
  SAVSR_REQUIRE(plan && x_in && out && x_bytes && out_bytes, "savsr_plan_set_io: null pointer / empty buffer");
  SAVSR_REQUIRE(format == SAVSR_FMT_BF16 || format == SAVSR_FMT_FP16, "savsr_plan_set_io: unknown format %d", format);
  plan->x_in = x_in; plan->x_bytes = x_bytes; plan->out = out; plan->out_bytes = out_bytes; plan->format = format;
  return 0;
}

extern "C" int savsr_plan_add_pack_frames(savsr_plan* plan, savsr_arena* arena, const float* x, int t, int h, int w, int dst_slot) {
  SAVSR_REQUIRE(plan && arena && x, "savsr_plan_add_pack_frames: null pointer");
  savsr_ctx* ctx = plan->ctx;
  plan->ops.push_back([=](savsr_stream st) { return savsr_pack_frames(ctx, arena, x, t, h, w, dst_slot, st); });
  return 0;
}

extern "C" int savsr_plan_add_conv(savsr_plan* plan, savsr_arena* arena, const savsr_conv_group* groups, int ngroups, int ksize, int n_tile,
                                   int dst_mode, int impl) {
  SAVSR_REQUIRE(plan && arena && groups, "savsr_plan_add_conv: null pointer");
  SAVSR_REQUIRE(ngroups >= 0 && ngroups <= SAVSR_MAX_GROUPS, "savsr_plan_add_conv: ngroups %d out of range", ngroups);
  std::vector<savsr_conv_group> g(groups, groups + ngroups);
  savsr_ctx* ctx = plan->ctx;
  plan->ops.push_back([=](savsr_stream st) { return savsr_conv(ctx, arena, g.data(), ngroups, ksize, n_tile, dst_mode, impl, st); });
  return 0;
}

extern "C" int savsr_plan_add_osa_prologue(savsr_plan* plan, const savsr_osa_params* convs, int nconvs, int batch, int npart, int npix,
                                           float inv_scale_h, float inv_scale_w) {
  SAVSR_REQUIRE(plan && convs && nconvs >= 0, "savsr_plan_add_osa_prologue: null pointer");
  std::vector<savsr_osa_params> c(convs, convs + nconvs);
  savsr_ctx* ctx = plan->ctx;
  plan->ops.push_back([=](savsr_stream st) { return savsr_osa_prologue(ctx, c.data(), nconvs, batch, npart, npix, inv_scale_h, inv_scale_w, st); });
  return 0;
}

extern "C" int savsr_plan_add_ca_scale_residual(savsr_plan* plan, savsr_arena* arena, int t_slot, int x_slot, int dst_slot, const float* pool,
                                                int npart, const float* w1, const float* b1, const float* w2, const float* b2, float* y_scratch) {
  SAVSR_REQUIRE(plan && arena, "savsr_plan_add_ca_scale_residual: null pointer");
  savsr_ctx* ctx = plan->ctx;
  plan->ops.push_back([=](savsr_stream st) { return savsr_ca_scale_residual(ctx, arena, t_slot, x_slot, dst_slot, pool, npart, w1, b1, w2, b2, y_scratch, st); });
  return 0;
}

extern "C" int savsr_plan_add_osadapt_mask(savsr_plan* plan, const float* in16, int batch, int height, int width, const float* wa, const float* ba,
                                           const float* wb, const float* bb, const float* wc, const float* bc, float* half0, float* half1, float* mask) {
  SAVSR_REQUIRE(plan, "savsr_plan_add_osadapt_mask: null pointer");
  savsr_ctx* ctx = plan->ctx;
  plan->ops.push_back([=](savsr_stream st) { return savsr_osadapt_mask(ctx, in16, batch, height, width, wa, ba, wb, bb, wc, bc, half0, half1, mask, st); });
  return 0;
}

extern "C" int savsr_plan_add_satu_kconv_sta(savsr_plan* plan, savsr_arena* arena, int a_slot, int x_slot, int dst_slot, int h, int w,
                                             const void* weights, const float* bias, float slope) {
  SAVSR_REQUIRE(plan && arena, "savsr_plan_add_satu_kconv_sta: null pointer");
  savsr_ctx* ctx = plan->ctx;
  plan->ops.push_back([=](savsr_stream st) { return savsr_satu_kconv_sta(ctx, arena, a_slot, x_slot, dst_slot, h, w, weights, bias, slope, st); });
  return 0;
}

extern "C" int savsr_plan_add_satu_hr(savsr_plan* plan, savsr_arena* lr, int x_slot, int sta_slot, int h, int w, int H, int W, const float* table,
                                      const float* base_y, const float* base_x, const void* weights, const float* zbias, const float* tail_bias,
                                      const float* x_in, int t, int centre, float* out) {
  SAVSR_REQUIRE(plan && lr, "savsr_plan_add_satu_hr: null pointer");
  savsr_ctx* ctx = plan->ctx;
  plan->ops.push_back([=](savsr_stream st) {
    return savsr_satu_hr(ctx, lr, x_slot, sta_slot, h, w, H, W, table, base_y, base_x, weights, zbias, tail_bias, x_in, t, centre, out, st);
  });
  return 0;
}

extern "C" int savsr_plan_add_arena_export(savsr_plan* plan, savsr_arena* arena, int slot, float* nchw) {
  SAVSR_REQUIRE(plan && arena && nchw, "savsr_plan_add_arena_export: null pointer");
  plan->ops.push_back([=](savsr_stream st) { return savsr_arena_export(arena, slot, nchw, st); });
  return 0;
}

extern "C" int savsr_plan_run(savsr_plan* plan, savsr_stream st) {
  SAVSR_REQUIRE(plan, "savsr_plan_run: null plan");
  plan->ctx->fmt = plan->format;
  for (size_t i = 0; i < plan->ops.size(); ++i) {
    const int rc = plan->ops[i](st);
    if (rc) return rc;
  }
  return 0;
}

extern "C" int savsr_forward(savsr_plan* plan, const float* x, float* out, savsr_stream st) {
  SAVSR_REQUIRE(plan && x && out, "savsr_forward: null pointer");
  SAVSR_REQUIRE(plan->x_in && plan->out, "savsr_forward: the plan has no I/O staging buffers (savsr_plan_set_io)");
  DeviceGuard guard(plan->ctx->device);
  cudaStream_t s = static_cast<cudaStream_t>(st);
  if (x != plan->x_in) SAVSR_CUDA(cudaMemcpyAsync(plan->x_in, x, plan->x_bytes, cudaMemcpyDeviceToDevice, s));
  if (int rc = savsr_plan_run(plan, st)) return rc;
  if (out != plan->out) SAVSR_CUDA(cudaMemcpyAsync(out, plan->out, plan->out_bytes, cudaMemcpyDeviceToDevice, s));
  return 0;
}
```

### savsr_b200/csrc/small_ops.cu

```cuda
#include "common.cuh"

namespace savsr {

__global__ void __launch_bounds__(256) pack_frames_kernel(const float* __restrict__ x, __nv_bfloat16* __restrict__ dst, int batch,
                                                          int t, int h, int w, int hp, int wp, int fmt) {
  const long npix = static_cast<long>(hp) * wp;
  const long total = static_cast<long>(batch) * npix * 8;
  for (long id = blockIdx.x * static_cast<long>(blockDim.x) + threadIdx.x; id < total; id += static_cast<long>(gridDim.x) * blockDim.x) {
    const int chunk = id & 7;
    const long pn = id >> 3;
    const long pix = pn % npix;
    const int n = pn / npix;
    const int py = pix / wp, px = pix % wp;
    const int ry = py < h ? py : 2 * h - 2 - py, rx = px < w ? px : 2 * w - 2 - px;
    float v[8];
#pragma unroll
    for (int e = 0; e < 8; ++e) {
      const int ch = chunk * 8 + e;
      v[e] = ch < 3 * t ? __ldg(x + ((static_cast<long>(n) * t * 3 + ch) * h + ry) * w + rx) : 0.f;
    }
    uint4 o;
    o.x = pack_h2(v[0], v[1], fmt); o.y = pack_h2(v[2], v[3], fmt); o.z = pack_h2(v[4], v[5], fmt); o.w = pack_h2(v[6], v[7], fmt);
    *reinterpret_cast<uint4*>(dst + (static_cast<long>(n) * npix + pix) * kC + chunk * 8) = o;
  }
}

constexpr int kMaxOsa = 4;
struct OsaLaunch {
  savsr_osa_params c[kMaxOsa];
  int nconvs, batch, npart, npix;
  float inv_h, inv_w;
  int fmt;
};
__host__ __device__ inline int osa_scratch_stride(int ci) { return 5 * ci + 192; }
__host__ __device__ inline int osa_off_h1(int ci) { return ci + 8; }
__host__ __device__ inline int osa_off_v2(int ci) { return 3 * ci + 8; }
__host__ __device__ inline int osa_off_att(int ci) { return 4 * ci + 8; }

__device__ __forceinline__ float sigmoidf_(float x) { return 1.f / (1.f + expf(-x)); }

constexpr int kOsaThreads = 1024;
__global__ void __launch_bounds__(kOsaThreads) osa_pool_kernel(const __grid_constant__ OsaLaunch L) {
  pdl_wait();
  pdl_trigger();
  const savsr_osa_params& c = L.c[blockIdx.z];
  const int s = blockIdx.x, n = blockIdx.y;
  if (s * 64 >= c.ci) return;
  __shared__ float red[16][64];
  const int ch = threadIdx.x & 63, part = threadIdx.x >> 6;
  const float* src = c.pool[s] + static_cast<long>(n) * L.npart * kC;
  float a0 = 0.f, a1 = 0.f;
  int q = part;
  for (; q + 16 < L.npart; q += 32) { a0 += src[q * kC + ch]; a1 += src[(q + 16) * kC + ch]; }
  if (q < L.npart) a0 += src[q * kC + ch];
  red[part][ch] = a0 + a1;
  __syncthreads();
  float* vin = c.scratch + static_cast<long>(n) * osa_scratch_stride(c.ci);
  if (part == 0) {
    float sum = 0.f;
#pragma unroll
    for (int k = 0; k < 16; ++k) sum += red[k][ch];
    vin[2 + s * 64 + ch] = sum / static_cast<float>(L.npix);
  }
  if (s == 0 && threadIdx.x == 0) { vin[0] = L.inv_h; vin[1] = L.inv_w; }
}

__global__ void __launch_bounds__(256) osa_linear_kernel(const __grid_constant__ OsaLaunch L, int layer) {
  pdl_wait();
  pdl_trigger();
  extern __shared__ float s_in[];
  const savsr_osa_params& c = L.c[blockIdx.y];
  const int rows = layer == 0 ? 2 * c.ci : c.ci;
  const int len = layer == 0 ? c.ci + 2 : 2 * c.ci;
  const int in_off = layer == 0 ? 0 : osa_off_h1(c.ci);
  const int out_off = layer == 0 ? osa_off_h1(c.ci) : osa_off_v2(c.ci);
  const float* W = layer == 0 ? c.r0_w : c.r2_w;
  const float* B = layer == 0 ? c.r0_b : c.r2_b;
  const int warp = threadIdx.x >> 5, lane = threadIdx.x & 31;
  if (blockIdx.x * 8 >= rows) return;
  const int stride = osa_scratch_stride(c.ci);
  const int per = (L.batch + gridDim.z - 1) / gridDim.z;
  const int n0 = blockIdx.z * per, n1 = min(L.batch, n0 + per);
  if (n0 >= n1) return;
  for (int i = threadIdx.x; i < (n1 - n0) * len; i += blockDim.x) {
    const int n = i / len, k = i - n * len;
    s_in[i] = c.scratch[static_cast<long>(n0 + n) * stride + in_off + k];
  }
  __syncthreads();
  const int row = blockIdx.x * 8 + warp;
  if (row >= rows) return;
  const float* wr = W + static_cast<long>(row) * len;
  float w[20];
#pragma unroll
  for (int j = 0; j < 20; ++j) w[j] = lane + 32 * j < len ? __ldg(wr + lane + 32 * j) : 0.f;
  const float bias = B[row];
  for (int n = n0; n < n1; ++n) {
    const float* in = s_in + (n - n0) * len;
    float acc = 0.f;
#pragma unroll
    for (int j = 0; j < 20; ++j) if (lane + 32 * j < len) acc += w[j] * in[lane + 32 * j];
#pragma unroll
    for (int off = 16; off >= 1; off >>= 1) acc += __shfl_xor_sync(0xffffffffu, acc, off);
    if (lane == 0) c.scratch[static_cast<long>(n) * stride + out_off + row] = fmaxf(acc + bias, 0.f);
  }
}

constexpr int kAsmMaxSamples = 8;
__global__ void __launch_bounds__(256) osa_assemble_kernel(const __grid_constant__ OsaLaunch L) {
  const savsr_osa_params& c = L.c[blockIdx.y];
  __shared__ float z_s[kAsmMaxSamples][32];
  __shared__ float att_s[kAsmMaxSamples][64 * SAVSR_MAX_SRC + 64 + 9 + 8];
  const int per = (L.batch + gridDim.z - 1) / gridDim.z;
  const int n0 = blockIdx.z * per, n1 = min(L.batch, n0 + per);
  if (n0 >= n1 || blockIdx.x * blockDim.x >= c.co * c.ci) return;
  const int ns = n1 - n0;
  const int warp = threadIdx.x >> 5, lane = threadIdx.x & 31;
  const int stride = osa_scratch_stride(c.ci);
  const int nout = c.ci + c.co + 9 + 8;
  for (int a = warp; a < c.att; a += 8) {
    float wr[10];
#pragma unroll
    for (int j = 0; j < 10; ++j) wr[j] = lane + 32 * j < c.ci ? __ldg(c.fc_w + a * c.ci + lane + 32 * j) : 0.f;
    const float bs = c.bn_scale[a], bh = c.bn_shift[a];
    for (int n = 0; n < ns; ++n) {
      const float* v2 = c.scratch + static_cast<long>(n0 + n) * stride + osa_off_v2(c.ci);
      float acc = 0.f;
#pragma unroll
      for (int j = 0; j < 10; ++j) if (lane + 32 * j < c.ci) acc += wr[j] * v2[lane + 32 * j];
#pragma unroll
      for (int off = 16; off >= 1; off >>= 1) acc += __shfl_xor_sync(0xffffffffu, acc, off);
      if (lane == 0) z_s[n][a] = fmaxf(acc * bs + bh, 0.f);
    }
  }
  __syncthreads();
  for (int j = threadIdx.x; j < nout; j += blockDim.x) {
    const float* w;
    float b;
    if (j < c.ci) { w = c.ch_w + j * c.att; b = c.ch_b[j]; }
    else if (j < c.ci + c.co) { w = c.fl_w + (j - c.ci) * c.att; b = c.fl_b[j - c.ci]; }
    else if (j < c.ci + c.co + 9) { w = c.sp_w + (j - c.ci - c.co) * c.att; b = c.sp_b[j - c.ci - c.co]; }
    else { w = c.kn_w + (j - c.ci - c.co - 9) * c.att; b = c.kn_b[j - c.ci - c.co - 9]; }
    float wv[32];
#pragma unroll
    for (int a = 0; a < 32; ++a) wv[a] = a < c.att ? __ldg(w + a) : 0.f;
    const bool sig = j < c.ci + c.co + 9;
    for (int n = 0; n < ns; ++n) {
      float acc = b;
#pragma unroll
      for (int a = 0; a < 32; ++a) if (a < c.att) acc += wv[a] * z_s[n][a];
      att_s[n][j] = sig ? sigmoidf_(acc) : acc;
    }
  }
  __syncthreads();
  if (threadIdx.x < ns) {
    float* ka = att_s[threadIdx.x] + c.ci + c.co + 9;
    float mx = ka[0];
    for (int k = 1; k < 8; ++k) mx = fmaxf(mx, ka[k]);
    float e[8], sum = 0.f;
    for (int k = 0; k < 8; ++k) { e[k] = expf(ka[k] - mx); sum += e[k]; }
    for (int k = 0; k < 8; ++k) ka[k] = e[k] / sum;
  }
  __syncthreads();
  if (blockIdx.x == 0) {
    for (int r = threadIdx.x; r < ns * nout; r += blockDim.x) {
      const int n = r / nout, j = r - n * nout;
      c.scratch[static_cast<long>(n0 + n) * stride + osa_off_att(c.ci) + j] = att_s[n][j];
    }
  }
  const int idx = blockIdx.x * blockDim.x + threadIdx.x;
  if (idx >= c.co * c.ci) return;
  const int i = idx % c.ci, o = idx / c.ci;
  float bk[8][9];
  const long per_k = static_cast<long>(c.co) * c.ci * 9;
#pragma unroll
  for (int k = 0; k < 8; ++k) {
    const float* src = c.bank + k * per_k + (static_cast<long>(o) * c.ci + i) * 9;
#pragma unroll
    for (int t = 0; t < 9; ++t) bk[k][t] = __ldg(src + t);
  }
  const int s = i >> 6, kk = i & 63;
  const long sample_elems = static_cast<long>(c.co) * c.ci * 9;
  const int row = quad_row(o);
  const int inner = row * 64 + ((((kk >> 3) ^ (row & 7)) << 3) | (kk & 7));
  for (int n = 0; n < ns; ++n) {
    const float* att = att_s[n];
    const float ca = att[i], fa = att[c.ci + o];
    const float* sa = att + c.ci + c.co;
    const float* ka = sa + 9;
    uint16_t* dst = static_cast<uint16_t*>(c.packed) + (n0 + n) * sample_elems;
#pragma unroll
    for (int t = 0; t < 9; ++t) {
      float acc = 0.f;
#pragma unroll
      for (int k = 0; k < 8; ++k) acc += ka[k] * bk[k][t];
      dst[static_cast<long>(s * 9 + t) * 4096 + inner] = float_to_h(acc * sa[t] * ca * fa, L.fmt);
    }
  }
}

struct CaParams {
  const __nv_bfloat16* t;
  const __nv_bfloat16* x;
  __nv_bfloat16* dst;
  const float* pool;
  const float *w1, *b1, *w2, *b2;
  float* y;
  int npart;
  int fmt;
  long npix;
};
__global__ void __launch_bounds__(1024) ca_vector_kernel(const CaParams p) {
  pdl_wait();
  pdl_trigger();
  __shared__ float red[16][64];
  __shared__ float mean[64];
  __shared__ float hid[4];
  const int n = blockIdx.x;
  const int ch = threadIdx.x & 63, part = threadIdx.x >> 6;
  const float* src = p.pool + static_cast<long>(n) * p.npart * kC;
  float a0 = 0.f, a1 = 0.f;
  int q = part;
  for (; q + 16 < p.npart; q += 32) { a0 += src[q * kC + ch]; a1 += src[(q + 16) * kC + ch]; }
  if (q < p.npart) a0 += src[q * kC + ch];
  red[part][ch] = a0 + a1;
  __syncthreads();
  if (part == 0) {
    float sum = 0.f;
#pragma unroll
    for (int k = 0; k < 16; ++k) sum += red[k][ch];
    mean[ch] = sum / static_cast<float>(p.npix);
  }
  __syncthreads();
  if (threadIdx.x < 4) {
    float a = p.b1[threadIdx.x];
    for (int i = 0; i < 64; ++i) a += p.w1[threadIdx.x * 64 + i] * mean[i];
    hid[threadIdx.x] = fmaxf(a, 0.f);
  }
  __syncthreads();
  if (threadIdx.x < 64) {
    float a = p.b2[threadIdx.x];
#pragma unroll
    for (int i = 0; i < 4; ++i) a += p.w2[threadIdx.x * 4 + i] * hid[i];
    p.y[n * 64 + threadIdx.x] = sigmoidf_(a);
  }
}
__global__ void __launch_bounds__(256) ca_scale_residual_kernel(const CaParams p) {
  pdl_wait();
  pdl_trigger();
  __shared__ float ys[64];
  const int n = blockIdx.y;
  if (threadIdx.x < 64) ys[threadIdx.x] = p.y[n * 64 + threadIdx.x];
  __syncthreads();
  const long chunks = p.npix * 8;
  const uint4* tt = reinterpret_cast<const uint4*>(p.t + static_cast<long>(n) * p.npix * kC);
  const uint4* xx = reinterpret_cast<const uint4*>(p.x + static_cast<long>(n) * p.npix * kC);
  uint4* dd = reinterpret_cast<uint4*>(p.dst + static_cast<long>(n) * p.npix * kC);
  for (long id = blockIdx.x * static_cast<long>(blockDim.x) + threadIdx.x; id < chunks;
       id += static_cast<long>(gridDim.x) * blockDim.x) {
    const int c0 = (id & 7) * 8;
    const uint4 a = tt[id], b = xx[id];
    uint4 o;
    o.x = pack_h2(h_lo(b.x, p.fmt) + h_lo(a.x, p.fmt) * ys[c0 + 0], h_hi(b.x, p.fmt) + h_hi(a.x, p.fmt) * ys[c0 + 1], p.fmt);
    o.y = pack_h2(h_lo(b.y, p.fmt) + h_lo(a.y, p.fmt) * ys[c0 + 2], h_hi(b.y, p.fmt) + h_hi(a.y, p.fmt) * ys[c0 + 3], p.fmt);
    o.z = pack_h2(h_lo(b.z, p.fmt) + h_lo(a.z, p.fmt) * ys[c0 + 4], h_hi(b.z, p.fmt) + h_hi(a.z, p.fmt) * ys[c0 + 5], p.fmt);
    o.w = pack_h2(h_lo(b.w, p.fmt) + h_lo(a.w, p.fmt) * ys[c0 + 6], h_hi(b.w, p.fmt) + h_hi(a.w, p.fmt) * ys[c0 + 7], p.fmt);
    dd[id] = o;
  }
}

template <bool kPool, bool kProj>
__global__ void __launch_bounds__(256) mask_conv16_kernel(const float* __restrict__ in, const float* __restrict__ w,
                                                          const float* __restrict__ b, const float* __restrict__ wf,
                                                          float* __restrict__ out, int h2, int w2) {
  __shared__ __align__(16) float w_s[9 * 16 * 16 + 36 * 4];
  __shared__ float wf_s[9 * 16];
  for (int i = threadIdx.x; i < 9 * 256; i += blockDim.x) {
    const int co = i & 15, ci = (i >> 4) & 15, tap = i >> 8;
    w_s[i + (i >> 6) * 4] = w[(co * 16 + ci) * 9 + tap];
  }
  if (kProj) {
    for (int i = threadIdx.x; i < 144; i += blockDim.x) wf_s[i] = wf[(i & 15) * 9 + (i >> 4)];
  }
  __syncthreads();
  const int n = blockIdx.y;
  const int q = threadIdx.x & 3;
  const long npix2 = static_cast<long>(h2) * w2;
  const long pix = blockIdx.x * static_cast<long>(blockDim.x >> 2) + (threadIdx.x >> 2);
  const bool live = pix < npix2;
  const int py = live ? pix / w2 : 0, px = live ? pix % w2 : 0;
  float acc[16];
#pragma unroll
  for (int o = 0; o < 16; ++o) acc[o] = 0.f;
  const int wfull = 2 * w2;
  const float* base = kPool ? in + static_cast<long>(n) * (4 * npix2) * 16 : in + static_cast<long>(n) * npix2 * 16;
#pragma unroll
  for (int tap = 0; tap < 9; ++tap) {
    const int sy = py + tap / 3 - 1, sx = px + tap % 3 - 1;
    if (!live || sy < 0 || sy >= h2 || sx < 0 || sx >= w2) continue;
    float4 a;
    if (kPool) {
      const float4 q0 = *reinterpret_cast<const float4*>(base + (static_cast<long>(2 * sy) * wfull + 2 * sx) * 16 + 4 * q);
      const float4 q1 = *reinterpret_cast<const float4*>(base + (static_cast<long>(2 * sy) * wfull + 2 * sx + 1) * 16 + 4 * q);
      const float4 q2 = *reinterpret_cast<const float4*>(base + (static_cast<long>(2 * sy + 1) * wfull + 2 * sx) * 16 + 4 * q);
      const float4 q3 = *reinterpret_cast<const float4*>(base + (static_cast<long>(2 * sy + 1) * wfull + 2 * sx + 1) * 16 + 4 * q);
      a.x = 0.25f * ((q0.x + q1.x) + (q2.x + q3.x)); a.y = 0.25f * ((q0.y + q1.y) + (q2.y + q3.y));
      a.z = 0.25f * ((q0.z + q1.z) + (q2.z + q3.z)); a.w = 0.25f * ((q0.w + q1.w) + (q2.w + q3.w));
    } else {
      a = *reinterpret_cast<const float4*>(base + (static_cast<long>(sy) * w2 + sx) * 16 + 4 * q);
    }
    const float av[4] = {a.x, a.y, a.z, a.w};
#pragma unroll
    for (int c = 0; c < 4; ++c) {
      const float4* wr = reinterpret_cast<const float4*>(w_s + (tap * 16 + 4 * q + c) * 16 + (tap * 4 + q) * 4);
#pragma unroll
      for (int o4 = 0; o4 < 4; ++o4) {
        const float4 wv = wr[o4];
        acc[4 * o4 + 0] += av[c] * wv.x; acc[4 * o4 + 1] += av[c] * wv.y;
        acc[4 * o4 + 2] += av[c] * wv.z; acc[4 * o4 + 3] += av[c] * wv.w;
      }
    }
  }
#pragma unroll
  for (int off = 2, cnt = 8; off >= 1; off >>= 1, cnt >>= 1) {
    const bool upper = (q & off) != 0;
#pragma unroll
    for (int i = 0; i < cnt; ++i) {
      const float send = upper ? acc[i] : acc[i + cnt];
      const float keep = upper ? acc[i + cnt] : acc[i];
      acc[i] = keep + __shfl_xor_sync(0xffffffffu, send, off);
    }
  }
  float o4v[4];
#pragma unroll
  for (int i = 0; i < 4; ++i) o4v[i] = fmaxf(acc[i] + b[4 * q + i], 0.f);
  if (!kProj) {
    if (live) *reinterpret_cast<float4*>(out + (static_cast<long>(n) * npix2 + pix) * 16 + 4 * q) = make_float4(o4v[0], o4v[1], o4v[2], o4v[3]);
  } else {
    float d[9];
#pragma unroll
    for (int t = 0; t < 9; ++t) {
      float v = 0.f;
#pragma unroll
      for (int i = 0; i < 4; ++i) v += wf_s[t * 16 + 4 * q + i] * o4v[i];
      v += __shfl_xor_sync(0xffffffffu, v, 1);
      v += __shfl_xor_sync(0xffffffffu, v, 2);
      d[t] = v;
    }
    if (live && q < 3) {
      float* dst = out + (static_cast<long>(n) * npix2 + pix) * 12 + 4 * q;
      *reinterpret_cast<float4*>(dst) = q == 0 ? make_float4(d[0], d[1], d[2], d[3])
                                     : q == 1 ? make_float4(d[4], d[5], d[6], d[7]) : make_float4(d[8], 0.f, 0.f, 0.f);
    }
  }
}

__global__ void __launch_bounds__(256) mask_final_kernel(const float* __restrict__ d, const float* __restrict__ b,
                                                         float* __restrict__ mask, int h2, int w2) {
  const int n = blockIdx.y;
  const int H = 2 * h2, W = 2 * w2;
  const long npix = static_cast<long>(H) * W;
  const long pix = blockIdx.x * static_cast<long>(blockDim.x) + threadIdx.x;
  if (pix >= npix) return;
  const int py = pix / W, px = pix % W;
  const float* base = d + static_cast<long>(n) * h2 * w2 * 12;
  float acc = b[0];
#pragma unroll
  for (int tap = 0; tap < 9; ++tap) {
    const int sy = py + tap / 3 - 1, sx = px + tap % 3 - 1;
    if (sy < 0 || sy >= H || sx < 0 || sx >= W) continue;
    float fy = 0.5f * (static_cast<float>(sy) + 0.5f) - 0.5f;
    float fx = 0.5f * (static_cast<float>(sx) + 0.5f) - 0.5f;
    fy = fy < 0.f ? 0.f : fy;
    fx = fx < 0.f ? 0.f : fx;
    const int y0 = static_cast<int>(fy), x0 = static_cast<int>(fx);
    const int y1 = y0 + (y0 < h2 - 1 ? 1 : 0), x1 = x0 + (x0 < w2 - 1 ? 1 : 0);
    const float ly = fy - y0, lx = fx - x0;
    const float v00 = base[(static_cast<long>(y0) * w2 + x0) * 12 + tap], v01 = base[(static_cast<long>(y0) * w2 + x1) * 12 + tap];
    const float v10 = base[(static_cast<long>(y1) * w2 + x0) * 12 + tap], v11 = base[(static_cast<long>(y1) * w2 + x1) * 12 + tap];
    acc += (1.f - ly) * ((1.f - lx) * v00 + lx * v01) + ly * ((1.f - lx) * v10 + lx * v11);
  }
  mask[static_cast<long>(n) * npix + pix] = sigmoidf_(acc);
}

__device__ __forceinline__ float y_of_u8(int b, int g, int r) {
  const double d = (static_cast<double>(static_cast<float>(b) / 255.f) * 24.966 + static_cast<double>(static_cast<float>(g) / 255.f) * 128.553) +
                   static_cast<double>(static_cast<float>(r) / 255.f) * 65.481 + 16.0;
  return static_cast<float>(d / 255.) * 255.f;
}
__global__ void __launch_bounds__(256) img_metrics_kernel(const float* __restrict__ sr, const float* __restrict__ gt, int H, int W,
                                                          uint8_t* __restrict__ bgr, double* __restrict__ sse) {
  const int n = blockIdx.y;
  const long npix = static_cast<long>(H) * W;
  const float* s = sr + static_cast<long>(n) * 3 * npix;
  const float* g = gt ? gt + static_cast<long>(n) * 3 * npix : nullptr;
  double acc = 0.0;
  for (long pix = blockIdx.x * static_cast<long>(blockDim.x) + threadIdx.x; pix < npix; pix += static_cast<long>(gridDim.x) * blockDim.x) {
    int q[3], qg[3];
#pragma unroll
    for (int c = 0; c < 3; ++c) {
      q[c] = __float2int_rn(fminf(fmaxf(s[c * npix + pix], 0.f), 1.f) * 255.0f);
      if (g) qg[c] = __float2int_rn(fminf(fmaxf(g[c * npix + pix], 0.f), 1.f) * 255.0f);
    }
    if (bgr) {
      uint8_t* o = bgr + (static_cast<long>(n) * npix + pix) * 3;
      o[0] = static_cast<uint8_t>(q[2]); o[1] = static_cast<uint8_t>(q[1]); o[2] = static_cast<uint8_t>(q[0]);
    }
    if (g) {
      const double d = static_cast<double>(y_of_u8(q[2], q[1], q[0])) - static_cast<double>(y_of_u8(qg[2], qg[1], qg[0]));
      acc += d * d;
    }
  }
  if (sse) {
    __shared__ double red[8];
#pragma unroll
    for (int off = 16; off >= 1; off >>= 1) acc += __shfl_xor_sync(0xffffffffu, acc, off);
    if ((threadIdx.x & 31) == 0) red[threadIdx.x >> 5] = acc;
    __syncthreads();
    if (threadIdx.x == 0) {
      double t = 0.0;
      for (int i = 0; i < 8; ++i) t += red[i];
      sse[static_cast<long>(n) * gridDim.x + blockIdx.x] = t;
    }
  }
}

}

using namespace savsr;

struct SsimParams {
  const float* sr;
  const float* gt;
  double* partials;
  int H, W, bx, by;
  double k[11];
};
__global__ void __launch_bounds__(256) ssim_y_kernel(const __grid_constant__ SsimParams p) {
  __shared__ double y1[26][27], y2[26][27];
  __shared__ double red[8];
  const int n = blockIdx.z;
  const long npix = static_cast<long>(p.H) * p.W;
  const float* s = p.sr + static_cast<long>(n) * 3 * npix;
  const float* g = p.gt + static_cast<long>(n) * 3 * npix;
  const int oy0 = blockIdx.y * 16, ox0 = blockIdx.x * 16;
  for (int i = threadIdx.x; i < 26 * 26; i += 256) {
    const int r = i / 26, c = i - r * 26;
    const int y = oy0 + r, x = ox0 + c;
    double a = 0.0, b = 0.0;
    if (y < p.H && x < p.W) {
      const long pix = static_cast<long>(y) * p.W + x;
      int q[3], qg[3];
#pragma unroll
      for (int ch = 0; ch < 3; ++ch) {
        q[ch] = __float2int_rn(fminf(fmaxf(s[ch * npix + pix], 0.f), 1.f) * 255.0f);
        qg[ch] = __float2int_rn(fminf(fmaxf(g[ch * npix + pix], 0.f), 1.f) * 255.0f);
      }
      a = static_cast<double>(y_of_u8(q[2], q[1], q[0]));
      b = static_cast<double>(y_of_u8(qg[2], qg[1], qg[0]));
    }
    y1[r][c] = a; y2[r][c] = b;
  }
  __syncthreads();
  const int ty = threadIdx.x >> 4, tx = threadIdx.x & 15;
  double val = 0.0;
  if (oy0 + ty < p.H - 10 && ox0 + tx < p.W - 10) {
    double mu1 = 0.0, mu2 = 0.0, s11 = 0.0, s22 = 0.0, s12 = 0.0;
    for (int i = 0; i < 11; ++i) {
#pragma unroll
      for (int j = 0; j < 11; ++j) {
        const double w = p.k[i] * p.k[j];
        const double a = y1[ty + i][tx + j], b = y2[ty + i][tx + j];
        mu1 += w * a; mu2 += w * b;
        s11 += w * (a * a); s22 += w * (b * b); s12 += w * (a * b);
      }
    }
    const double c1 = (0.01 * 255) * (0.01 * 255), c2 = (0.03 * 255) * (0.03 * 255);
    const double mu1_sq = mu1 * mu1, mu2_sq = mu2 * mu2, mu12 = mu1 * mu2;
    val = ((2 * mu12 + c1) * (2 * (s12 - mu12) + c2)) / ((mu1_sq + mu2_sq + c1) * ((s11 - mu1_sq) + (s22 - mu2_sq) + c2));
  }
#pragma unroll
  for (int off = 16; off >= 1; off >>= 1) val += __shfl_xor_sync(0xffffffffu, val, off);
  if ((threadIdx.x & 31) == 0) red[threadIdx.x >> 5] = val;
  __syncthreads();
  if (threadIdx.x == 0) {
    double t = 0.0;
    for (int i = 0; i < 8; ++i) t += red[i];
    p.partials[(static_cast<long>(n) * p.by + blockIdx.y) * p.bx + blockIdx.x] = t;
  }
}

extern "C" int savsr_pack_frames(savsr_ctx* ctx, savsr_arena* arena, const float* x, int t, int h, int w, int dst_slot, savsr_stream st) {
  SAVSR_REQUIRE(ctx && arena && x, "savsr_pack_frames: null pointer");
  DeviceGuard guard(ctx->device);
  SAVSR_REQUIRE(t >= 1 && 3 * t <= kC, "savsr_pack_frames: %d frames do not fit 64 channels", t);
  SAVSR_REQUIRE(h >= 2 && w >= 2, "savsr_pack_frames: LR frame %dx%d too small for reflect padding", h, w);
  SAVSR_REQUIRE(arena->height == h + (h & 1) && arena->width == w + (w & 1),
                "savsr_pack_frames: arena %dx%d is not the even-padded size of %dx%d", arena->height, arena->width, h, w);
  SAVSR_REQUIRE(dst_slot >= 0 && dst_slot < arena->nslots, "savsr_pack_frames: slot %d out of range", dst_slot);
  if (arena->batch == 0) return 0;
  const long npix = static_cast<long>(arena->height) * arena->width;
  const long total = arena->batch * npix * 8;
  const int blocks = static_cast<int>((total + 255) / 256 < 4096 ? (total + 255) / 256 : 4096);
  pack_frames_kernel<<<blocks, 256, 0, static_cast<cudaStream_t>(st)>>>(x, arena->base + static_cast<long>(dst_slot) * arena->batch * npix * kC,
                                                                       arena->batch, t, h, w, arena->height, arena->width, ctx->fmt);
  SAVSR_CUDA(cudaGetLastError());
  return 0;
}

namespace savsr {
int osa_prologue_front(savsr_ctx* ctx, const savsr_osa_params* convs, int nconvs, int batch, int npart, int npix, float inv_scale_h,
                       float inv_scale_w, cudaStream_t st) {
  OsaLaunch L;
  memset(&L, 0, sizeof(L));
  int max_ci = 0;
  for (int i = 0; i < nconvs; ++i) {
    L.c[i] = convs[i];
    max_ci = convs[i].ci > max_ci ? convs[i].ci : max_ci;
  }
  L.nconvs = nconvs; L.batch = batch; L.npart = npart; L.npix = npix;
  L.inv_h = inv_scale_h; L.inv_w = inv_scale_w;
  L.fmt = ctx->fmt;
  (void)launch_k(ctx->opt[SAVSR_OPT_PDL] != 0, osa_pool_kernel, dim3(max_ci / 64, batch, nconvs), dim3(kOsaThreads), 0, st, L);
  const int lin_split = batch >= 12 ? 3 : (batch >= 4 ? 2 : 1);
  const size_t lin_smem = static_cast<size_t>((batch + lin_split - 1) / lin_split) * 2 * max_ci * sizeof(float);
  SAVSR_REQUIRE(lin_smem <= 200 * 1024, "savsr_osa_prologue: batch %d too large for the routing kernel's shared memory", batch);
  if (lin_smem > 48 * 1024) {
    if (int rc = ensure_smem_attr(ctx, kAttrOsaLinear, osa_linear_kernel, 200 * 1024)) return rc;
  }
  (void)launch_k(ctx->opt[SAVSR_OPT_PDL] != 0, osa_linear_kernel, dim3((2 * max_ci + 7) / 8, nconvs, lin_split), dim3(256), lin_smem, st, L, 0);
  (void)launch_k(ctx->opt[SAVSR_OPT_PDL] != 0, osa_linear_kernel, dim3((max_ci + 7) / 8, nconvs, lin_split), dim3(256), lin_smem, st, L, 1);
  SAVSR_CUDA(cudaGetLastError());
  return 0;
}
}

extern "C" int savsr_osa_prologue(savsr_ctx* ctx, const savsr_osa_params* convs, int nconvs, int batch, int npart,
                                  int npix, float inv_scale_h, float inv_scale_w, savsr_stream st_) {
  SAVSR_REQUIRE(ctx && convs, "savsr_osa_prologue: null pointer");
  DeviceGuard guard(ctx->device);
  SAVSR_REQUIRE(nconvs >= 0 && nconvs <= kMaxOsa, "savsr_osa_prologue: nconvs %d out of range [0,%d]", nconvs, kMaxOsa);
  if (nconvs == 0 || batch == 0) return 0;
  cudaStream_t st = static_cast<cudaStream_t>(st_);
  OsaLaunch L;
  memset(&L, 0, sizeof(L));
  int max_ci = 0;
  for (int i = 0; i < nconvs; ++i) {
    const savsr_osa_params& c = convs[i];
    SAVSR_REQUIRE(c.ci > 0 && c.ci % 64 == 0 && c.ci <= 64 * SAVSR_MAX_SRC, "savsr_osa_prologue: conv %d ci %d unsupported", i, c.ci);
    SAVSR_REQUIRE(c.co == 64, "savsr_osa_prologue: conv %d co %d unsupported (64 only)", i, c.co);
    SAVSR_REQUIRE(c.att > 0 && c.att <= 32, "savsr_osa_prologue: conv %d attention channels %d out of range", i, c.att);
    SAVSR_REQUIRE(c.bank && c.r0_w && c.r0_b && c.r2_w && c.r2_b && c.fc_w && c.bn_scale && c.bn_shift && c.ch_w && c.ch_b &&
                  c.fl_w && c.fl_b && c.sp_w && c.sp_b && c.kn_w && c.kn_b && c.scratch && c.packed,
                  "savsr_osa_prologue: conv %d has a null parameter pointer", i);
    for (int s = 0; s < c.ci / 64; ++s) SAVSR_REQUIRE(c.pool[s], "savsr_osa_prologue: conv %d source %d has no pool buffer", i, s);
    L.c[i] = c;
    max_ci = c.ci > max_ci ? c.ci : max_ci;
  }
  L.nconvs = nconvs; L.batch = batch; L.npart = npart; L.npix = npix;
  L.inv_h = inv_scale_h; L.inv_w = inv_scale_w;
  L.fmt = ctx->fmt;
  if (int rc = osa_prologue_front(ctx, convs, nconvs, batch, npart, npix, inv_scale_h, inv_scale_w, st)) return rc;
  int asm_split = batch >= 16 ? 4 : (batch >= 6 ? 2 : 1);
  while ((batch + asm_split - 1) / asm_split > kAsmMaxSamples) ++asm_split;
  osa_assemble_kernel<<<dim3((64 * max_ci + 255) / 256, nconvs, asm_split), 256, 0, st>>>(L);
  SAVSR_CUDA(cudaGetLastError());
  return 0;
}

extern "C" int savsr_ca_scale_residual(savsr_ctx* ctx, savsr_arena* arena, int t_slot, int x_slot, int dst_slot,
                                       const float* pool, int npart, const float* w1, const float* b1, const float* w2,
                                       const float* b2, float* y_scratch, savsr_stream st) {
  SAVSR_REQUIRE(ctx && arena && pool && w1 && b1 && w2 && b2 && y_scratch, "savsr_ca_scale_residual: null pointer");
  DeviceGuard guard(ctx->device);
  SAVSR_REQUIRE(t_slot >= 0 && t_slot < arena->nslots && x_slot >= 0 && x_slot < arena->nslots && dst_slot >= 0 &&
                dst_slot < arena->nslots, "savsr_ca_scale_residual: slot out of range");
  CaParams p;
  p.npix = static_cast<long>(arena->height) * arena->width;
  const long img = p.npix * kC * arena->batch;
  p.t = arena->base + t_slot * img;
  p.x = arena->base + x_slot * img;
  p.dst = arena->base + dst_slot * img;
  p.fmt = ctx->fmt; p.pool = pool; p.npart = npart; p.w1 = w1; p.b1 = b1; p.w2 = w2; p.b2 = b2; p.y = y_scratch;
  long blocks = (p.npix * 8 + 255) / 256;
  const long cap = 8L * ctx->sm_count / (arena->batch > 0 ? arena->batch : 1) + 1;
  if (blocks > cap) blocks = cap;
  if (arena->batch == 0) return 0;
  (void)launch_k(ctx->opt[SAVSR_OPT_PDL] != 0, ca_vector_kernel, dim3(arena->batch), dim3(1024), 0, static_cast<cudaStream_t>(st), p);
  (void)launch_k(ctx->opt[SAVSR_OPT_PDL] != 0, ca_scale_residual_kernel, dim3(static_cast<unsigned>(blocks), arena->batch), dim3(256), 0, static_cast<cudaStream_t>(st), p);
  SAVSR_CUDA(cudaGetLastError());
  return 0;
}

extern "C" int savsr_osadapt_mask(savsr_ctx* ctx, const float* in16, int batch, int height, int width, const float* wa,
                                  const float* ba, const float* wb, const float* bb, const float* wc, const float* bc,
                                  float* half0, float* half1, float* mask, savsr_stream st_) {
  SAVSR_REQUIRE(ctx && in16 && wa && ba && wb && bb && wc && bc && half0 && half1 && mask, "savsr_osadapt_mask: null pointer");
  DeviceGuard guard(ctx->device);
  SAVSR_REQUIRE(height % 2 == 0 && width % 2 == 0, "savsr_osadapt_mask: size %dx%d must be even (pad_spatial)", height, width);
  if (batch == 0) return 0;
  cudaStream_t st = static_cast<cudaStream_t>(st_);
  const int h2 = height / 2, w2 = width / 2;
  const long npix2 = static_cast<long>(h2) * w2;
  dim3 g2(static_cast<unsigned>((npix2 + 63) / 64), batch);
  mask_conv16_kernel<true, false><<<g2, 256, 0, st>>>(in16, wa, ba, nullptr, half0, h2, w2);
  mask_conv16_kernel<false, true><<<g2, 256, 0, st>>>(half0, wb, bb, wc, half1, h2, w2);
  dim3 g1(static_cast<unsigned>((4 * npix2 + 255) / 256), batch);
  mask_final_kernel<<<g1, 256, 0, st>>>(half1, bc, mask, h2, w2);
  SAVSR_CUDA(cudaGetLastError());
  return 0;
}

static long img_metrics_grid(const savsr_ctx* ctx, int height, int width) {
  const long npix = static_cast<long>(height) * width;
  long blocks = (npix + 255) / 256;
  if (blocks > 4L * ctx->sm_count) blocks = 4L * ctx->sm_count;
  return blocks;
}

extern "C" int savsr_img_metrics_blocks(const savsr_ctx* ctx, int height, int width) {
  return (ctx && height > 0 && width > 0) ? static_cast<int>(img_metrics_grid(ctx, height, width)) : 0;
}

extern "C" int savsr_img_metrics(savsr_ctx* ctx, const float* sr, const float* gt, int batch, int height, int width, uint8_t* bgr_u8,
                                 double* sse_y, savsr_stream st_) {
  SAVSR_REQUIRE(ctx && sr, "savsr_img_metrics: null pointer");
  DeviceGuard guard(ctx->device);
  SAVSR_REQUIRE(batch >= 0 && height > 0 && width > 0, "savsr_img_metrics: bad shape");
  SAVSR_REQUIRE(!sse_y || gt, "savsr_img_metrics: sse_y requested without a ground-truth frame");
  if (batch == 0) return 0;
  cudaStream_t st = static_cast<cudaStream_t>(st_);
  const long blocks = img_metrics_grid(ctx, height, width);
  img_metrics_kernel<<<dim3(static_cast<unsigned>(blocks), batch), 256, 0, st>>>(sr, gt, height, width, bgr_u8, sse_y);
  SAVSR_CUDA(cudaGetLastError());
  return 0;
}

extern "C" int savsr_ssim_y_blocks(int height, int width) {
  if (height < 11 || width < 11) return 0;
  return ((height - 10 + 15) / 16) * ((width - 10 + 15) / 16);
}

extern "C" int savsr_ssim_y(savsr_ctx* ctx, const float* sr, const float* gt, int batch, int height, int width, double* partials,
                            savsr_stream st) {
  SAVSR_REQUIRE(ctx && sr && gt && partials, "savsr_ssim_y: null pointer");
  DeviceGuard guard(ctx->device);
  SAVSR_REQUIRE(batch >= 0 && height >= 11 && width >= 11, "savsr_ssim_y: frames of %dx%d are smaller than the 11x11 window", height, width);
  if (batch == 0) return 0;
  SsimParams p;
  p.sr = sr; p.gt = gt; p.partials = partials; p.H = height; p.W = width;
  p.bx = (width - 10 + 15) / 16; p.by = (height - 10 + 15) / 16;
  double sum = 0.0;
  for (int i = 0; i < 11; ++i) { p.k[i] = exp(-((i - 5.0) * (i - 5.0)) / (2.0 * 1.5 * 1.5)); sum += p.k[i]; }
  for (int i = 0; i < 11; ++i) p.k[i] /= sum;
  ssim_y_kernel<<<dim3(p.bx, p.by, batch), 256, 0, static_cast<cudaStream_t>(st)>>>(p);
  SAVSR_CUDA(cudaGetLastError());
  return 0;
}
```

### savsr_b200/engine.py

```python
from __future__ import annotations

import os

import ctypes as C
from typing import Callable, Dict, List, Optional, Sequence, Tuple

import numpy as np
import torch

from . import _capi as K

BN_EPS = 1e-5


def normalize_scale(scale) -> Tuple[float, float]:
    if isinstance(scale, (int, float)):
        return (scale, scale)
    s = tuple(scale)
    if len(s) != 2:
        raise ValueError(f"scale must be a number or a (s_h, s_w) pair, got {scale!r}")
    return (s[0], s[1])


def get_hw(h: int, w: int, scale) -> Tuple[int, int]:
    s = normalize_scale(scale)
    return round(h * s[0]), round(w * s[1])


_contexts: Dict[int, K.Context] = {}


def context(device_index: int) -> K.Context:
    if device_index not in _contexts:
        c = K.Context(device_index)
        if os.environ.get("SAVSR_BIGK_ALL") is not None:
            c.set_option(K.OPT_BIGK_ALL, int(os.environ["SAVSR_BIGK_ALL"] != "0"))
        if os.environ.get("SAVSR_BIGK_ISSUERS") is not None:
            c.set_option(K.OPT_BIGK_ISSUERS, int(os.environ["SAVSR_BIGK_ISSUERS"]))
        if os.environ.get("SAVSR_PDL") is not None:
            c.set_option(K.OPT_PDL, int(os.environ["SAVSR_PDL"] != "0"))
        _contexts[device_index] = c
    return _contexts[device_index]


class pdl:

    def __init__(self, ctx: K.Context, on: bool):
        self.ctx = ctx
        env = os.environ.get("SAVSR_PDL")
        self.on = int(on if env is None else env != "0")

    def __enter__(self):
        self.prev = self.ctx.lib.savsr_ctx_get_option(self.ctx.handle, K.OPT_PDL)
        self.ctx.set_option(K.OPT_PDL, self.on)
        return self

    def __exit__(self, *exc):
        self.ctx.set_option(K.OPT_PDL, max(self.prev, 0))
        return False


class WeightStore:

    def __init__(self, version: tuple = ()):
        self.version = version
        self.cache: Dict[tuple, torch.Tensor] = {}

    def get(self, key: tuple, make: Callable[[], torch.Tensor]) -> torch.Tensor:
        t = self.cache.get(key)
        if t is None:
            t = self.cache[key] = make()
        return t


class _Slots:

    def __init__(self):
        self.free: List[int] = []
        self.n = 0

    def get(self) -> int:
        if self.free:
            return self.free.pop()
        self.n += 1
        return self.n - 1

    def get_many(self, k: int) -> List[int]:
        return [self.get() for _ in range(k)]

    def get_contiguous(self, k: int) -> int:
        s = self.n
        self.n += k
        return s

    def put(self, *slots: int) -> None:
        self.free.extend(slots)


def satu_hr_compose(P: Dict[str, torch.Tensor], device: torch.device):
    g = lambda name: P[name].detach().to(device, torch.float64)
    u = "upsample"
    Wf = g(u + ".fusion.weight").view(64, 128)
    bf = g(u + ".fusion.bias")
    Wt = g("tail.weight").permute(2, 3, 0, 1).reshape(27, 64)
    comb = Wt @ Wf
    Wcs, Wcf = comb[:, :64], comb[:, 64:]
    We = g(u + ".weight_expand").view(4, 64, 8).permute(1, 0, 2).reshape(64, 32)
    Wv = Wcf @ We
    Wc = g(u + ".weight_compress").reshape(32, 64)
    zb = torch.zeros(32, dtype=torch.float64, device=device)
    zb[:27] = Wt @ bf
    return Wc.float(), Wcf.float().contiguous(), Wcs.float().contiguous(), Wv.float(), zb.float()


def satu_hr_pack(parts, fmt: int, device: torch.device) -> torch.Tensor:
    dt = torch.float16 if fmt == K.FMT_FP16 else torch.bfloat16
    n = torch.arange(32, device=device).view(32, 1)
    pos = torch.arange(8, device=device).view(1, 8) ^ (n & 7)
    tiles = []
    for m in parts[:4]:
        full = torch.zeros(32, 64, device=device)
        full[:m.shape[0], :m.shape[1]] = m
        src = full.to(dt).view(32, 8, 8)
        tile = torch.zeros_like(src)
        tile.scatter_(1, pos.view(32, 8, 1).expand(32, 8, 8), src)
        tiles.append(tile.reshape(-1))
    return torch.cat(tiles).view(torch.uint8).contiguous()


class Plan:
    def __init__(self, params: Dict[str, torch.Tensor], batch: int, h: int, w: int, scale, device: torch.device,
                 conv_impl: str = "tap", num_frame: int = 7, taps: Optional[Sequence[str]] = None, precision: str = "bf16",
                 store: Optional[WeightStore] = None):
        if device.type != "cuda":
            raise K.SavsrError("savsr_b200 runs on CUDA (sm_100a) only; there is no CPU fallback")
        if num_frame != 7:
            raise NotImplementedError("only the shipped 7-frame configuration is implemented")
        if h < 2 or w < 2:
            raise ValueError(f"LR frames must be at least 2x2, got {h}x{w}")
        self.device = device
        self.ctx = context(device.index if device.index is not None else torch.cuda.current_device())
        self.lib = self.ctx.lib
        self.impl = K.IMPL_NAMES[conv_impl]
        if precision not in K.FMT_NAMES:
            raise ValueError(f"precision must be one of {sorted(K.FMT_NAMES)}, got {precision!r}")
        self.fmt = K.FMT_NAMES[precision]
        self.B, self.h, self.w, self.t = batch, h, w, num_frame
        self.scale = normalize_scale(scale)
        self.hp, self.wp = h + (h & 1), w + (w & 1)
        self.H, self.W = get_hw(h, w, self.scale)
        self.P = params
        self._keep: List[object] = []
        self._pack_src: List[torch.Tensor] = []
        self.ops: List[Callable[[int], int]] = []
        self.op_meta: List[Tuple[str, float, int, str]] = []
        self.n_launches = 0
        self.taps = set(taps or ())
        self.tap_bufs: Dict[str, torch.Tensor] = {}
        self.graph: Optional[torch.cuda.CUDAGraph] = None
        self.store = store if store is not None else WeightStore()
        self.nbytes = 0
        self._pool_cache: Dict[str, int] = {}
        self._osa_cache: Dict[str, Tuple[K.OsaParams, int, int]] = {}
        self.cplan: Optional[K.CPlan] = K.CPlan(self.ctx) if hasattr(K, "CPlan") and hasattr(self.lib, "savsr_plan_create") else None
        self._recorded = 0
        with torch.cuda.device(device), torch.no_grad():
            self.ctx.set_format(self.fmt)
            self._build()
            if self.cplan is not None:
                if self._recorded == len(self.ops):
                    K.check(self.lib.savsr_plan_set_io(self.cplan.handle, self.x_in.data_ptr(), self.x_in.numel() * 4, self.out.data_ptr(),
                                                       self.out.numel() * 4, self.fmt))
                else:
                    self.cplan = None

    def _buf(self, *shape, dtype=torch.float32) -> torch.Tensor:
        t = torch.empty(*shape, dtype=dtype, device=self.device)
        self._keep.append(t)
        self.nbytes += t.numel() * t.element_size()
        return t

    def _p(self, name: str) -> torch.Tensor:
        t = self.P[name]
        if t.device != self.device or t.dtype != torch.float32 or not t.is_contiguous():
            t = t.detach().to(self.device, torch.float32).contiguous()
        self._keep.append(t)
        return t

    def _ptr(self, name: str) -> int:
        return self._p(name).data_ptr()

    def _derived(self, key, make: Callable[[], torch.Tensor]) -> torch.Tensor:
        return self.store.get(("derived", key), lambda: make().detach().to(self.device, torch.float32).contiguous())

    def _dev(self, key, make: Callable[[], torch.Tensor]) -> int:
        return self._derived(key, make).data_ptr()

    def _packp(self, name: str) -> int:
        return self._pack(name, lambda: self._p(name))

    def _pack(self, key, make: Callable[[], torch.Tensor], n_tile: int = 64, co_pad: Optional[int] = None,
              rows: int = K.ROWS_QUAD) -> int:
        def build() -> torch.Tensor:
            w = make().detach().to(self.device, torch.float32).contiguous()
            co_real, ci, ks, _ = w.shape
            co = co_pad or co_real
            out = torch.empty(self.lib.savsr_packed_weight_bytes(co, ci, ks), dtype=torch.uint8, device=self.device)
            K.check(self.lib.savsr_pack_conv_weight(w.data_ptr(), co_real, co, ci, ks, n_tile, self.fmt, rows, out.data_ptr(),
                                                    torch.cuda.current_stream(self.device).cuda_stream))
            self._pack_src.append(w)
            return out
        return self.store.get(("packed", key, n_tile, co_pad, rows, self.fmt), build).data_ptr()

    def _emit(self, fn: Callable[[int], int], launches: int = 1, kind: str = "other", flops: float = 0.0,
              detail: str = "", rec: Optional[Callable[[object], int]] = None) -> None:
        self.ops.append(fn)
        self.op_meta.append((kind, flops, launches, detail))
        self.n_launches += launches
        if rec is not None and self.cplan is not None:
            K.check(rec(self.cplan.handle))
            self._recorded += 1

    def _group(self, src: Sequence[int], dst: int, weight: int, bias: int = 0, act: int = K.ACT_NONE, slope: float = 0.2,
               res1: int = -1, res2: int = -1, res2_scale: float = 0.0, wstride: int = 0, mask: int = 0, pool: int = 0,
               aux: int = 0, src_channels: int = 0) -> K.ConvGroup:
        g = K.ConvGroup()
        for i, s in enumerate(src):
            g.src_slot[i] = s
        g.nsrc = len(src)
        g.dst_slot, g.res1_slot, g.res2_slot, g.res2_scale = dst, res1, res2, res2_scale
        g.act, g.slope = act, slope
        g.weight, g.weight_sample_stride = weight, wstride
        g.bias, g.mask, g.pool, g.aux_dst = bias or None, mask or None, pool or None, aux or None
        g.src_channels = src_channels
        return g

    def _conv(self, arena: K.Arena, groups: Sequence[K.ConvGroup], ksize: int = 3, n_tile: int = 64,
              dst_mode: int = K.DST_ARENA, alg_ci: Optional[Sequence[int]] = None, alg_co: Optional[int] = None,
              kind: Optional[str] = None) -> None:
        arr = (K.ConvGroup * len(groups))(*groups)
        self._keep.append(arr)
        lib, ctx, ah, n, impl = self.lib, self.ctx.handle, arena.handle, len(groups), self.impl
        co = alg_co if alg_co is not None else (64 if n_tile == 64 else 16)
        ci = list(alg_ci) if alg_ci is not None else [64 * g.nsrc for g in groups]
        flops = 2.0 * self.B * arena.height * arena.width * co * ksize * ksize * sum(ci)
        osa = any(g.weight_sample_stride != 0 for g in groups)
        self._emit(lambda st: lib.savsr_conv(ctx, ah, arr, n, ksize, n_tile, dst_mode, impl, st),
                   kind=kind or f"conv{ksize}x{ksize}_n{n_tile}", flops=flops,
                   detail=f"g{n}s{groups[0].nsrc}" + ("osa" if osa else ""),
                   rec=lambda cp: lib.savsr_plan_add_conv(cp, ah, arr, n, ksize, n_tile, dst_mode, impl))

    def _tap(self, name: str, arena: str, slot: int) -> None:
        if name not in self.taps:
            return
        a = self.lr
        buf = self._buf(self.B, 64, a.height, a.width)
        self.tap_bufs[name] = buf
        lib, ah, ptr = self.lib, a.handle, buf.data_ptr()
        self._emit(lambda st: lib.savsr_arena_export(ah, slot, ptr, st), kind="debug_tap", rec=lambda cp: lib.savsr_plan_add_arena_export(cp, ah, slot, ptr))

    def _osa_params(self, prefix: str, nsrc: int, pools: Sequence[int]) -> Tuple[K.OsaParams, int, int]:
        if prefix in self._osa_cache:
            return self._osa_cache[prefix]
        ci, co = 64 * nsrc, 64
        att = max(int(ci * 0.0625), 16)
        a = prefix + ".attention"
        def bn_s():
            return self._p(a + ".bn.weight") / torch.sqrt(self._p(a + ".bn.running_var") + BN_EPS)

        def bn_b():
            return self._p(a + ".bn.bias") - self._p(a + ".bn.running_mean") * bn_s()
        o = K.OsaParams()
        o.ci, o.co, o.att = ci, co, att
        o.bank = self._ptr(prefix + ".weight")
        o.r0_w, o.r0_b = self._ptr(prefix + ".scale_routing.0.weight"), self._ptr(prefix + ".scale_routing.0.bias")
        o.r2_w, o.r2_b = self._ptr(prefix + ".scale_routing.2.weight"), self._ptr(prefix + ".scale_routing.2.bias")
        o.fc_w = self._ptr(a + ".fc.weight")
        o.bn_scale, o.bn_shift = self._dev(a + ".bn_scale", bn_s), self._dev(a + ".bn_shift", bn_b)
        o.ch_w, o.ch_b = self._ptr(a + ".channel_fc.weight"), self._ptr(a + ".channel_fc.bias")
        o.fl_w, o.fl_b = self._ptr(a + ".filter_fc.weight"), self._ptr(a + ".filter_fc.bias")
        o.sp_w, o.sp_b = self._ptr(a + ".spatial_fc.weight"), self._ptr(a + ".spatial_fc.bias")
        o.kn_w, o.kn_b = self._ptr(a + ".kernel_fc.weight"), self._ptr(a + ".kernel_fc.bias")
        for i, pp in enumerate(pools):
            o.pool[i] = pp
        scratch = self._buf(self.B, 5 * ci + 192)
        packed = self._buf(self.B, co * ci * 9 * 2, dtype=torch.uint8)
        o.scratch, o.packed = scratch.data_ptr(), packed.data_ptr()
        self.osa_scratch[prefix] = scratch
        self._osa_cache[prefix] = (o, packed.data_ptr(), co * ci * 9 * 2)
        return self._osa_cache[prefix]

    def _osa_prologue(self, convs: Sequence[K.OsaParams]) -> None:
        arr = (K.OsaParams * len(convs))(*convs)
        self._keep.append(arr)
        inv_h = float(np.float32(1.0) / np.float32(self.scale[0]))
        inv_w = float(np.float32(1.0) / np.float32(self.scale[1]))
        lib, ctx, n, B = self.lib, self.ctx.handle, len(convs), self.B
        npart, npix = self.lr.tiles * 4, self.hp * self.wp
        self._emit(lambda st: lib.savsr_osa_prologue(ctx, arr, n, B, npart, npix, inv_h, inv_w, st), launches=4, kind="osa_prologue",
                   rec=lambda cp: lib.savsr_plan_add_osa_prologue(cp, arr, n, B, npart, npix, inv_h, inv_w))

    def _pool(self, key: str) -> int:
        if key not in self._pool_cache:
            self._pool_cache[key] = self._buf(self.B, self.lr.tiles * 4, 64).data_ptr()
        return self._pool_cache[key]

    def _residual_block(self, prefixes: Sequence[str], xs: Sequence[Sequence[int]], outs: Sequence[Sequence[int]],
                        tmp: Sequence[Sequence[int]], base: Sequence[int]) -> None:
        lr = self.lr
        nfr = len(xs[0])
        use_os = (prefixes[0] + ".osconv.weight") in self.P
        L = K.ACT_LRELU
        pools = [[self._pool(f"{p}.conv0.{i}") if use_os else 0 for i in range(nfr)] for p in prefixes]
        self._conv(lr, [self._group([xs[d][i]], tmp[d][i], self._packp(f"{p}.conv0.{i}.weight"),
                                    self._ptr(f"{p}.conv0.{i}.bias"), act=L, pool=pools[d][i])
                        for d, p in enumerate(prefixes) for i in range(nfr)])
        if use_os:
            osa = [self._osa_params(p + ".osconv", nfr, pools[d]) for d, p in enumerate(prefixes)]
            self._osa_prologue([o[0] for o in osa])
            self._conv(lr, [self._group(tmp[d], base[d], osa[d][1], act=L, wstride=osa[d][2]) for d in range(len(prefixes))])
        else:
            self._conv(lr, [self._group(tmp[d], base[d], self._packp(p + ".conv1.weight"), self._ptr(p + ".conv1.bias"), act=L)
                            for d, p in enumerate(prefixes)], ksize=1)
        self._conv(lr, [self._group([base[d], tmp[d][i]], outs[d][i], self._packp(f"{p}.conv2.{i}.weight"),
                                    self._ptr(f"{p}.conv2.{i}.bias"), act=L, res1=xs[d][i])
                        for d, p in enumerate(prefixes) for i in range(nfr)])

    def _build(self) -> None:
        P, B, t = self.P, self.B, self.t
        lib, ctx = self.lib, self.ctx.handle
        L = K.ACT_LRELU
        self.osa_scratch: Dict[str, torch.Tensor] = {}
        nf = 64
        sl = _Slots()
        zero = sl.get()
        FR = sl.get()
        dirs = ("f2p_win", "p2f_win")
        n_it = t - 3 + 1
        F = [[sl.get() for _ in range(n_it)] for _ in dirs]
        S0 = [sl.get_many(2) for _ in dirs]
        S1 = [sl.get_many(3) for _ in dirs]
        S2 = [sl.get_many(3) for _ in dirs]
        T = [sl.get_many(3) for _ in dirs]
        Bs = [sl.get() for _ in dirs]
        pool_free = [s for d in range(2) for s in (S0[d] + S1[d] + S2[d] + T[d])] + Bs
        extra_needed = 5 + 5 + 5 + 1 + 2 + 1 + 6 + 2
        while len(pool_free) < extra_needed:
            pool_free.append(sl.get())
        self.n_lr_slots = sl.n
        self.arena_lr_t = self._buf(self.n_lr_slots * B, self.hp, self.wp, 64, dtype=torch.bfloat16)
        self.arena_lr_t.zero_()
        self.lr = K.Arena(self.ctx, self.arena_lr_t.data_ptr(), self.n_lr_slots, B, self.hp, self.wp)
        lr = self.lr
        self.x_in = self._buf(B, t, 3, self.h, self.w)
        self.out = self._buf(B, 3, self.H, self.W)
        xin = self.x_in.data_ptr()

        lrh0, hh0, ww0 = lr.handle, self.h, self.w
        self._emit(lambda st: lib.savsr_pack_frames(ctx, lrh0, xin, t, hh0, ww0, FR, st), kind="pack_frames",
                   rec=lambda cp: lib.savsr_plan_add_pack_frames(cp, lrh0, xin, t, hh0, ww0, FR))
        hpast = [zero, zero]
        for idx in range(n_it):
            centre = [t - 1 - 1 - idx, idx + 1]
            fgroups = []
            for d, p in enumerate(dirs):
                c = centre[d]

                def wc(p=p, c=c):
                    wz = torch.zeros(64, 64, 3, 3, device=self.device)
                    wz[:, 3 * c:3 * c + 3] = self._p(p + ".conv_c.weight")
                    return wz

                def ws(p=p, c=c):
                    wz = torch.zeros(64, 64, 3, 3, device=self.device)
                    wsup = self._p(p + ".conv_sup.weight")
                    wz[:, 3 * (c - 1):3 * (c - 1) + 3] = wsup[:, 0:3]
                    wz[:, 3 * (c + 1):3 * (c + 1) + 3] = wsup[:, 3:6]
                    return wz
                fgroups.append(self._group([FR], S0[d][0], self._pack((p, "conv_c@", c), wc), self._ptr(p + ".conv_c.bias"), act=L, src_channels=32))
                fgroups.append(self._group([FR], S0[d][1], self._pack((p, "conv_sup@", c), ws), self._ptr(p + ".conv_sup.bias"), act=L, src_channels=32))
            self._conv(lr, fgroups, alg_ci=[3, 6, 3, 6])
            cur = [[S0[d][0], S0[d][1], hpast[d]] for d in range(2)]
            sets = [S1, S2]
            for j in range(4):
                nxt = sets[j % 2]
                self._residual_block([f"{p}.blocks.{j}" for p in dirs], cur, nxt, T, Bs)
                cur = [list(nxt[d]) for d in range(2)]
            self._conv(lr, [self._group(cur[d], F[d][idx], self._packp(p + ".merge.weight"), self._ptr(p + ".merge.bias"))
                            for d, p in enumerate(dirs)])
            hpast = [F[0][idx], F[1][idx]]
        self._tap("f2p_last", "lr", F[0][n_it - 1])
        self._tap("p2f_last", "lr", F[1][n_it - 1])

        free = list(pool_free)
        take = lambda k: [free.pop() for _ in range(k)]
        Gx, Gy, T5 = take(5), take(5), take(5)
        B5, = take(1)
        M = take(2)
        A, = take(1)
        p2 = "h_win.0"
        self._conv(lr, [self._group([F[0][n_it - 1 - i], F[1][i]], Gx[i], self._packp(f"{p2}.conv_h.{i}.weight"),
                                    self._ptr(f"{p2}.conv_h.{i}.bias"), act=L) for i in range(5)])
        cur5, nxt5 = Gx, Gy
        for j in range(2):
            self._residual_block([f"{p2}.blocks.{j}"], [cur5], [nxt5], [T5], [B5])
            cur5, nxt5 = nxt5, cur5
        wm = self._packp(p2 + ".merge.weight")
        half = 5 * 9 * 8192
        bm = self._p(p2 + ".merge.bias")
        self._conv(lr, [self._group(cur5, M[k], wm + k * half, bm[64 * k:].data_ptr()) for k in range(2)])
        self._tap("h_win0", "lr", M[0]); self._tap("h_win1", "lr", M[1])
        self._conv(lr, [self._group(M, A, self._packp("h_win_conv_h.weight"), self._ptr("h_win_conv_h.bias"), act=L)])
        self._tap("align", "lr", A)
        free += Gx + Gy + T5 + [B5] + M

        gamma = float(self._p("gamma").item())
        X0, X1, T1, T2, R, Hs = take(6)
        in16 = self._buf(B, self.hp * self.wp, 16)
        half0 = self._buf(B, (self.hp // 2) * (self.wp // 2), 16)
        half1 = self._buf(B, (self.hp // 2) * (self.wp // 2), 16)
        maskb = self._buf(B, self.hp * self.wp)
        ca_y = self._buf(B, 64).data_ptr()
        npart = lr.tiles * 4
        lrh = lr.handle
        h_cur = A
        for gi in range(4):
            x, xa, xb = h_cur, X0, X1
            for r in range(8):
                pr = f"RG.{gi}.residual_group.{r}.rcab"
                self._conv(lr, [self._group([x], T1, self._packp(pr + ".0.weight"), self._ptr(pr + ".0.bias"), act=K.ACT_RELU)])
                pl = self._pool(pr + ".2")
                self._conv(lr, [self._group([T1], T2, self._packp(pr + ".2.weight"), self._ptr(pr + ".2.bias"), pool=pl)])
                w1, b1 = self._ptr(pr + ".3.attention.1.weight"), self._ptr(pr + ".3.attention.1.bias")
                w2, b2 = self._ptr(pr + ".3.attention.3.weight"), self._ptr(pr + ".3.attention.3.bias")
                self._emit(lambda st, x=x, xa=xa, pl=pl, w1=w1, b1=b1, w2=w2, b2=b2:
                           lib.savsr_ca_scale_residual(ctx, lrh, T2, x, xa, pl, npart, w1, b1, w2, b2, ca_y, st),
                           launches=2, kind="ca_scale_residual",
                           rec=lambda cp, x=x, xa=xa, pl=pl, w1=w1, b1=b1, w2=w2, b2=b2:
                           lib.savsr_plan_add_ca_scale_residual(cp, lrh, T2, x, xa, pl, npart, w1, b1, w2, b2, ca_y))
                x, xa, xb = xa, xb, xa
            plr = self._pool(f"RG.{gi}.conv")
            self._conv(lr, [self._group([x], R, self._packp(f"RG.{gi}.conv.weight"), self._ptr(f"RG.{gi}.conv.bias"),
                                        res1=h_cur, pool=plr)])
            self._tap(f"rg{gi}", "lr", R)
            pa = f"adapt.{gi}"
            m = pa + ".mask"

            def fold(conv: str, bn: str):
                def sc():
                    return self._p(bn + ".weight") / torch.sqrt(self._p(bn + ".running_var") + BN_EPS)
                return (lambda: self._p(conv + ".weight") * sc().view(-1, 1, 1, 1),
                        lambda: (self._p(conv + ".bias") - self._p(bn + ".running_mean")) * sc() + self._p(bn + ".bias"))
            w0, b0 = fold(m + ".0", m + ".1")
            wa, ba = fold(m + ".4", m + ".5")
            wb, bb = fold(m + ".7", m + ".8")
            wc, bc = fold(m + ".11", m + ".12")
            self._conv(lr, [self._group([R], 0, self._pack(m + ".0+bn", w0, n_tile=16), self._dev(m + ".0+bn.bias", b0), act=K.ACT_RELU,
                                        aux=in16.data_ptr())], n_tile=16, dst_mode=K.DST_AUX16)
            args = (ctx, in16.data_ptr(), B, self.hp, self.wp, self._dev(m + ".4+bn.w", wa), self._dev(m + ".4+bn.b", ba),
                    self._dev(m + ".7+bn.w", wb), self._dev(m + ".7+bn.b", bb), self._dev(m + ".11+bn.w", wc), self._dev(m + ".11+bn.b", bc),
                    half0.data_ptr(), half1.data_ptr(), maskb.data_ptr())
            self._emit(lambda st, args=args: lib.savsr_osadapt_mask(*args, st), launches=3, kind="osadapt_mask",
                       rec=lambda cp, args=args: lib.savsr_plan_add_osadapt_mask(cp, *args[1:]))
            osa = self._osa_params(pa + ".adapt", 1, [plr])
            self._osa_prologue([osa[0]])
            self._conv(lr, [self._group([R], Hs, osa[1], wstride=osa[2], mask=maskb.data_ptr(), res1=R, res2=A, res2_scale=gamma)])
            self._tap(f"adapt{gi}", "lr", Hs)
            h_cur = Hs
        TR, = take(1)
        self._conv(lr, [self._group([h_cur], TR, self._packp("conv_last.weight"), self._ptr("conv_last.bias"), res1=A)])
        self._tap("trunk", "lr", TR)

        u = "upsample"
        wkp = self._pack(u + ".kernel_conv.tapmajor",
                         lambda: self._p(u + ".kernel_conv.0.weight").view(64, 25, 64).permute(1, 0, 2).reshape(1600, 64, 1, 1))
        bkp = self._dev(u + ".kernel_conv.tapmajor.bias", lambda: self._p(u + ".kernel_conv.0.bias").view(64, 25).t().contiguous())
        STA, = take(1)
        lrh, hh, ww = lr.handle, self.h, self.w
        kflops = 2.0 * B * self.hp * self.wp * 64 * 1600
        self._emit(lambda st: lib.savsr_satu_kconv_sta(ctx, lrh, A, TR, STA, hh, ww, wkp, bkp, 0.1, st), kind="satu_kconv_sta",
                   flops=kflops, rec=lambda cp: lib.savsr_plan_add_satu_kconv_sta(cp, lrh, A, TR, STA, hh, ww, wkp, bkp, 0.1))
        self._tap("satu_sta", "lr", STA)
        sw = K.SatuWeights()
        sw.body0_w, sw.body0_b = self._ptr(u + ".body.0.weight"), self._ptr(u + ".body.0.bias")
        sw.body2_w, sw.body2_b = self._ptr(u + ".body.2.weight"), self._ptr(u + ".body.2.bias")
        sw.routing_w, sw.routing_b = self._ptr(u + ".routing.0.weight"), self._ptr(u + ".routing.0.bias")
        sw.offset_w, sw.offset_b = self._ptr(u + ".offset.weight"), self._ptr(u + ".offset.bias")
        sw.st_offset_w, sw.st_offset_b = self._ptr(u + ".st_offset.weight"), self._ptr(u + ".st_offset.bias")
        sw.compress, sw.expand = self._ptr(u + ".weight_compress"), self._ptr(u + ".weight_expand")
        self._keep.append(sw)
        H, W = self.H, self.W
        self.rel_y, self.rel_x = self._buf(H), self._buf(W)
        self.base_y, self.base_x = self._buf(H), self._buf(W)
        self.cell_y, self.cell_x = self._buf(H, dtype=torch.int32), self._buf(W, dtype=torch.int32)
        self.corner_y, self.corner_x = self._buf(H, dtype=torch.int32), self._buf(W, dtype=torch.int32)
        self.table = self._buf(H * W, 8)
        K.check(lib.savsr_satu_index(ctx, C.byref(sw), self.h, self.w, H, W, float(self.scale[0]), float(self.scale[1]),
                                     self.rel_y.data_ptr(), self.rel_x.data_ptr(), self.cell_y.data_ptr(), self.cell_x.data_ptr(),
                                     self.base_y.data_ptr(), self.base_x.data_ptr(), self.corner_y.data_ptr(),
                                     self.corner_x.data_ptr(), self.table.data_ptr(), self._stream().cuda_stream))
        tab, by, bx = self.table.data_ptr(), self.base_y.data_ptr(), self.base_x.data_ptr()
        hw = self.store.get(("satu_hr_weights", self.fmt), lambda: satu_hr_pack(satu_hr_compose(P, self.device), self.fmt, self.device))
        zb = self._dev("satu_hr.zbias", lambda: satu_hr_compose(P, self.device)[4])
        tb = self._ptr("tail.bias")
        hwp, outp, cen = hw.data_ptr(), self.out.data_ptr(), t // 2
        hr_flops = 2.0 * B * self.H * self.W * (64 * 32 + 32 * 64 + 128 * 64 + 64 * 3 * 9)
        self._emit(lambda st: lib.savsr_satu_hr(ctx, lrh, TR, STA, hh, ww, H, W, tab, by, bx, hwp, zb, tb, xin, t, cen, outp, st),
                   kind="satu_hr", flops=hr_flops,
                   rec=lambda cp: lib.savsr_plan_add_satu_hr(cp, lrh, TR, STA, hh, ww, H, W, tab, by, bx, hwp, zb, tb, xin, t, cen, outp))
        self.satu_extra_bytes_per_sample = 2 * 64 * self.hp * self.wp * 2
        self._stream().synchronize()
        self._pack_src.clear()

    def _stream(self) -> "torch.cuda.Stream":
        return torch.cuda.current_stream(self.device)

    def run(self) -> None:
        with torch.cuda.device(self.device), pdl(self.ctx, self.B <= 2):
            self.ctx.set_format(self.fmt)
            st = self._stream().cuda_stream
            if self.cplan is not None:
                K.check(self.lib.savsr_plan_run(self.cplan.handle, st))
                return
            for op in self.ops:
                rc = op(st)
                if rc:
                    K.check(rc)

    def run_profiled(self, detail: bool = False) -> Dict[str, Dict[str, float]]:
        with torch.cuda.device(self.device):
            self.ctx.set_format(self.fmt)
            stream = self._stream()
            st = stream.cuda_stream
            evs = []
            for op in self.ops:
                e0, e1 = torch.cuda.Event(enable_timing=True), torch.cuda.Event(enable_timing=True)
                e0.record(stream)
                rc = op(st)
                e1.record(stream)
                if rc:
                    K.check(rc)
                evs.append((e0, e1))
            stream.synchronize()
        out: Dict[str, Dict[str, float]] = {}
        for (kind, flops, launches, tag), (e0, e1) in zip(self.op_meta, evs):
            d = out.setdefault(f"{kind}:{tag}" if (detail and tag) else kind, dict(ms=0.0, flops=0.0, ops=0, launches=0))
            d["ms"] += e0.elapsed_time(e1); d["flops"] += flops; d["ops"] += 1; d["launches"] += launches
        return out

    def time_ops_graph(self, select: Callable[[str, str], bool], reps: int = 5) -> Dict[str, float]:
        idx = [i for i, (kind, _, _, detail) in enumerate(self.op_meta) if select(kind, detail)]
        if not idx:
            return dict(ms=0.0, flops=0.0, launches=0, ops=0)
        with torch.cuda.device(self.device):
            self.ctx.set_format(self.fmt)
            torch.cuda.synchronize(self.device)
            g = torch.cuda.CUDAGraph()
            with torch.cuda.graph(g, stream=torch.cuda.Stream(self.device)):
                st = torch.cuda.current_stream(self.device).cuda_stream
                for i in idx:
                    rc = self.ops[i](st)
                    if rc:
                        K.check(rc)
            stream = self._stream()
            g.replay()
            e0, e1 = torch.cuda.Event(enable_timing=True), torch.cuda.Event(enable_timing=True)
            e0.record(stream)
            for _ in range(reps):
                g.replay()
            e1.record(stream)
            stream.synchronize()
        return dict(ms=e0.elapsed_time(e1) / reps, flops=sum(self.op_meta[i][1] for i in idx), launches=sum(self.op_meta[i][2] for i in idx), ops=len(idx))

    def capture(self) -> None:
        if self.graph is not None:
            return
        with torch.cuda.device(self.device):
            self.run()
            torch.cuda.synchronize(self.device)
            g = torch.cuda.CUDAGraph()
            with torch.cuda.graph(g, stream=torch.cuda.Stream(self.device)):
                self.run()
            self.graph = g

    def run_graph(self) -> None:
        if self.graph is None:
            self.capture()
        with torch.cuda.device(self.device):
            self.graph.replay()

    def forward_into(self, x: torch.Tensor, out: torch.Tensor, graph: bool = True) -> None:
        with torch.cuda.device(self.device):
            self.x_in.copy_(x, non_blocking=True)
            if graph:
                self.run_graph()
            else:
                self.run()
            out.copy_(self.out, non_blocking=True)

    def activation_absmax(self) -> float:
        dt = torch.float16 if self.fmt == K.FMT_FP16 else torch.bfloat16
        with torch.cuda.device(self.device):
            peak = float(torch.linalg.vector_norm(self.arena_lr_t.view(dt).reshape(-1), ord=float("inf")))
            return peak if peak == peak else float("inf")

    def forward_c(self, x: torch.Tensor, out: torch.Tensor) -> None:
        if self.cplan is None:
            raise K.SavsrError("this plan has no C-side launch list")
        if not (x.is_cuda and out.is_cuda and x.is_contiguous() and out.is_contiguous() and x.dtype == out.dtype == torch.float32):
            raise ValueError("savsr_forward takes contiguous fp32 CUDA tensors")
        if tuple(x.shape) != tuple(self.x_in.shape) or tuple(out.shape) != tuple(self.out.shape):
            raise ValueError(f"plan built for {tuple(self.x_in.shape)} -> {tuple(self.out.shape)}, got {tuple(x.shape)} -> {tuple(out.shape)}")
        with torch.cuda.device(self.device):
            K.check(self.lib.savsr_forward(self.cplan.handle, x.data_ptr(), out.data_ptr(), self._stream().cuda_stream))

    def release(self) -> None:
        self.graph = None
        self.cplan = None
        self.ops.clear()
        self._keep.clear()
        self._pack_src.clear()
        self.tap_bufs.clear()
        for name in ("arena_lr_t", "x_in", "out", "table", "lr"):
            if hasattr(self, name):
                setattr(self, name, None)
        self.nbytes = 0

    def read_tap(self, name: str) -> torch.Tensor:
        return self.tap_bufs[name]
```

Baseline: 270.7.

## Add serpentine tile traversal so consecutive kernels reuse L2-resident tiles

Adds a per-launch reverse flag so each conv and channel-attention kernel walks its tile range backward when the kernel that produced its input walked forward, and vice versa. The tiles written last by the producer should still be in L2 when the consumer reads them first. The channel-attention residual kernel is also restructured into per-SM tile chunks that mirror the conv work split, and the partial-sum reduction is widened to four accumulators. This adds traversal bookkeeping and an ABI change to the conv group struct and the plan API, and the reordering could hurt TMA prefetch locality.

```diff
diff --git a/include/savsr_b200.h b/include/savsr_b200.h
--- a/include/savsr_b200.h
+++ b/include/savsr_b200.h
@@ -50,14 +50,15 @@
   float* pool;
   void* aux_dst;
   int32_t src_channels;
-  int32_t reserved_;
+  int32_t reverse;
 } savsr_conv_group;
 
 enum savsr_option {
   SAVSR_OPT_BIGK_ALL = 0,
   SAVSR_OPT_BIGK_ISSUERS = 1,
   SAVSR_OPT_PDL = 2,
-  SAVSR_OPT_COUNT = 3
+  SAVSR_OPT_CA_REVERSE = 3,
+  SAVSR_OPT_COUNT = 4
 };
 
 int savsr_abi_version(void);
@@ -248,7 +249,7 @@
 int savsr_plan_add_osa_prologue(savsr_plan* plan, const savsr_osa_params* convs, int nconvs, int batch, int npart, int npix,
                                 float inv_scale_h, float inv_scale_w);
 int savsr_plan_add_ca_scale_residual(savsr_plan* plan, savsr_arena* arena, int t_slot, int x_slot, int dst_slot, const float* pool, int npart,
-                                     const float* w1, const float* b1, const float* w2, const float* b2, float* y_scratch);
+                                     const float* w1, const float* b1, const float* w2, const float* b2, float* y_scratch, int reverse);
 int savsr_plan_add_osadapt_mask(savsr_plan* plan, const float* in16, int batch, int height, int width, const float* wa, const float* ba,
                                 const float* wb, const float* bb, const float* wc, const float* bc, float* half0, float* half1, float* mask);
 int savsr_plan_add_satu_kconv_sta(savsr_plan* plan, savsr_arena* arena, int a_slot, int x_slot, int dst_slot, int h, int w, const void* weights,
diff --git a/savsr_b200/_capi.py b/savsr_b200/_capi.py
--- a/savsr_b200/_capi.py
+++ b/savsr_b200/_capi.py
@@ -15,7 +15,7 @@
 IMPL_NAMES = {"tap": IMPL_TAP, "halo": IMPL_HALO, "check": IMPL_CHECK}
 FMT_BF16, FMT_FP16 = 0, 1
 FMT_NAMES = {"bf16": FMT_BF16, "fp16": FMT_FP16}
-OPT_BIGK_ALL, OPT_BIGK_ISSUERS, OPT_PDL = 0, 1, 2
+OPT_BIGK_ALL, OPT_BIGK_ISSUERS, OPT_PDL, OPT_CA_REVERSE = 0, 1, 2, 3
 WGRAD_OIHW, WGRAD_TIO = 0, 1
 ROWS_LINEAR, ROWS_QUAD = 0, 1
 
@@ -43,7 +43,7 @@
         ("pool", C.c_void_p),
         ("aux_dst", C.c_void_p),
         ("src_channels", C.c_int32),
-        ("reserved_", C.c_int32),
+        ("reverse", C.c_int32),
     ]
 
 
@@ -161,7 +161,7 @@
     "savsr_plan_add_pack_frames": (_I, [_VP, _VP, _VP, _I, _I, _I, _I]),
     "savsr_plan_add_conv": (_I, [_VP, _VP, C.POINTER(ConvGroup), _I, _I, _I, _I, _I]),
     "savsr_plan_add_osa_prologue": (_I, [_VP, C.POINTER(OsaParams), _I, _I, _I, _I, _F, _F]),
-    "savsr_plan_add_ca_scale_residual": (_I, [_VP, _VP, _I, _I, _I, _VP, _I, _VP, _VP, _VP, _VP, _VP]),
+    "savsr_plan_add_ca_scale_residual": (_I, [_VP, _VP, _I, _I, _I, _VP, _I, _VP, _VP, _VP, _VP, _VP, _I]),
     "savsr_plan_add_osadapt_mask": (_I, [_VP, _VP, _I, _I, _I, _VP, _VP, _VP, _VP, _VP, _VP, _VP, _VP, _VP]),
     "savsr_plan_add_satu_kconv_sta": (_I, [_VP, _VP, _I, _I, _I, _I, _I, _VP, _VP, _F]),
     "savsr_plan_add_satu_hr": (_I, [_VP, _VP, _I, _I, _I, _I, _I, _I, _VP, _VP, _VP, _VP, _VP, _VP, _VP, _I, _I, _VP]),
diff --git a/savsr_b200/csrc/capi.cu b/savsr_b200/csrc/capi.cu
--- a/savsr_b200/csrc/capi.cu
+++ b/savsr_b200/csrc/capi.cu
@@ -90,6 +90,7 @@
   if (option == SAVSR_OPT_BIGK_ALL) SAVSR_REQUIRE(value == 0 || value == 1, "savsr_ctx_set_option: BIGK_ALL must be 0 or 1, got %d", value);
   if (option == SAVSR_OPT_BIGK_ISSUERS) SAVSR_REQUIRE(value == 1 || value == 2, "savsr_ctx_set_option: BIGK_ISSUERS must be 1 or 2, got %d", value);
   if (option == SAVSR_OPT_PDL) SAVSR_REQUIRE(value == 0 || value == 1, "savsr_ctx_set_option: PDL must be 0 or 1, got %d", value);
+  if (option == SAVSR_OPT_CA_REVERSE) SAVSR_REQUIRE(value == 0 || value == 1, "savsr_ctx_set_option: CA_REVERSE must be 0 or 1, got %d", value);
   ctx->opt[option] = value;
   return 0;
 }
diff --git a/savsr_b200/csrc/conv_igemm.cu b/savsr_b200/csrc/conv_igemm.cu
--- a/savsr_b200/csrc/conv_igemm.cu
+++ b/savsr_b200/csrc/conv_igemm.cu
@@ -39,7 +39,14 @@
   int fmt;
   int issuers;
   int ksteps;
+  int reverse;
 };
+
+__device__ __forceinline__ void walk_step(int& tile, int& gn, int tiles, int step) {
+  tile += step;
+  if (tile == tiles) { tile = 0; ++gn; }
+  else if (tile < 0) { tile = tiles - 1; --gn; }
+}
 
 __device__ __forceinline__ float apply_act(float v, int act, float slope) {
   if (act == SAVSR_ACT_LRELU) return v > 0.f ? v : v * slope;
@@ -363,6 +370,8 @@
   const int total = p.ngroups * p.batch * tiles;
   const int item_begin = blockIdx.x * p.chunk;
   const int item_end = min(item_begin + p.chunk, total);
+  const int step = p.reverse ? -1 : 1;
+  const int item_first = p.reverse ? item_end - 1 : item_begin;
   const int nsrc = p.nsrc;
   const int n_res = p.n_res;
   constexpr int kTmemCols = 2 * BN < 32 ? 32 : 2 * BN;
@@ -389,8 +398,8 @@
       int gen = -1, cur_key = -1;
       long long dbg_ae = 0;
       const int nkb = nsrc * NT;
-      int tile = item_begin % tiles;
-      int gn = item_begin / tiles;
+      int tile = item_first % tiles;
+      int gn = item_first / tiles;
       for (int item = item_begin; item < item_end; ++item) {
         const int n = gn % p.batch;
         const int gi = gn / p.batch;
@@ -441,7 +450,7 @@
             }
           }
         }
-        if (++tile == tiles) { tile = 0; ++gn; }
+        walk_step(tile, gn, tiles, step);
       }
       DBG_ONLY(if (p.dbg != nullptr) p.dbg[blockIdx.x * 8 + 6] = dbg_ae;)
       (void)dbg_ae;
@@ -457,9 +466,9 @@
     int sa = 0, pa = 0, sr = 0, pr = 0;
     int gen = -1, cur_key = -1;
     int it = 0;
-    int tile = item_begin % tiles;
-    int n = (item_begin / tiles) % p.batch;
-    int gi = (item_begin / tiles) / p.batch;
+    int tile = item_first % tiles;
+    int n = (item_first / tiles) % p.batch;
+    int gi = (item_first / tiles) / p.batch;
     const uint32_t ps_mask = p.per_sample_mask;
     const int batch = p.batch;
     long long dbg_te = 0, dbg_af = 0, dbg_t0 = DBG_CLOCK();
@@ -555,9 +564,11 @@
       }
       if (elect_one()) umma_commit(t_full + acc);
       __syncwarp();
-      if (++tile == tiles) {
-        tile = 0;
-        if (++n == batch) { n = 0; ++gi; }
+      tile += step;
+      if (tile == tiles || tile < 0) {
+        tile = tile < 0 ? tiles - 1 : 0;
+        n += step;
+        if (n == batch || n < 0) { n = n < 0 ? batch - 1 : 0; gi += step; }
       }
     }
     DBG_ONLY(if (p.dbg != nullptr && lane == 0) {
@@ -579,8 +590,8 @@
 #pragma unroll
       for (int i = 0; i < 8; ++i) eq.psum[i] = 0.f;
       int it = 0;
-      int tile = item_begin % tiles;
-      int gn = item_begin / tiles;
+      int tile = item_first % tiles;
+      int gn = item_first / tiles;
       long long dbg_tf = 0, dbg_t0 = DBG_CLOCK();
       if constexpr (BN == 64) {
         if (item_begin < item_end) epiq_prefetch(p, p.g[gn / p.batch], gn / p.batch, gn % p.batch, tile, quad, lane, half, eq);
@@ -597,12 +608,11 @@
         tc_fence_after();
         const uint32_t taddr = tmem_base + (static_cast<uint32_t>(quad * 32) << 16) + static_cast<uint32_t>(acc * BN + half * 32);
         if constexpr (BN == 64) {
-          epiq_finish(p, n, tile, quad, lane, half, taddr, eq, item + 1 >= item_end || tile + 1 == tiles,
+          int nt = tile, ngn = gn;
+          walk_step(nt, ngn, tiles, step);
+          epiq_finish(p, n, tile, quad, lane, half, taddr, eq, item + 1 >= item_end || ngn != gn,
                       [&] { if (lane == 0) mbar_arrive(t_empty + acc); }, [&] {
-            if (item + 1 < item_end) {
-              const int nt = tile + 1 == tiles ? 0 : tile + 1, ngn = tile + 1 == tiles ? gn + 1 : gn;
-              epiq_prefetch(p, p.g[ngn / p.batch], ngn / p.batch, ngn % p.batch, nt, quad, lane, half, eq);
-            }
+            if (item + 1 < item_end) epiq_prefetch(p, p.g[ngn / p.batch], ngn / p.batch, ngn % p.batch, nt, quad, lane, half, eq);
           });
         } else {
           float v[NC];
@@ -616,7 +626,7 @@
           if (lane == 0) mbar_arrive(t_empty + acc);
           epi_finish<NC>(p, g, n, tile, quad, lane, v, 0, ec);
         }
-        if (++tile == tiles) { tile = 0; ++gn; }
+        walk_step(tile, gn, tiles, step);
       }
       DBG_ONLY(if (p.dbg != nullptr && warp == 2 && lane == 0) {
         p.dbg[blockIdx.x * 8 + 4] = DBG_CLOCK() - dbg_t0;
@@ -662,6 +672,8 @@
   const int total = p.ngroups * p.batch * tiles;
   const int item_begin = blockIdx.x * p.chunk;
   const int item_end = min(item_begin + p.chunk, total);
+  const int step = p.reverse ? -1 : 1;
+  const int item_first = p.reverse ? item_end - 1 : item_begin;
   const int nsrc = p.nsrc;
   const bool pinned = nsrc <= 2;
   const uint32_t ps_mask = p.per_sample_mask;
@@ -682,8 +694,14 @@
   pdl_trigger();
 
   int item = item_begin;
-  int tile = item_begin % tiles;
-  int gn = item_begin / tiles;
+  int tile = item_first % tiles;
+  int gn = item_first / tiles;
+  auto batch_len = [&] { return min(kBatchTiles, min(item_end - item, step > 0 ? tiles - tile : tile + 1)); };
+  auto next_batch = [&](int cnt) {
+    item += cnt;
+    tile += step * (cnt - 1);
+    walk_step(tile, gn, tiles, step);
+  };
   int bcount = 0;
   uint32_t use_bits = 0;
   uint32_t set_loads[2] = {0, 0};
@@ -694,7 +712,7 @@
       int sa = 0, pa = 0;
       uint32_t u = 0;
       while (item < item_end) {
-        const int cnt = min(kBatchTiles, min(item_end - item, tiles - tile));
+        const int cnt = batch_len();
         const int n = gn % p.batch;
         const int gi = gn / p.batch;
         const savsr_conv_group& g = p.g[gi];
@@ -716,7 +734,7 @@
           }
           const int img = g.src_slot[s] * p.batch + n;
           for (int j = 0; j < cnt; ++j) {
-            const int tj = tile + j;
+            const int tj = tile + step * j;
             const int ty = tj / p.tiles_x;
             mbar_wait(a_empty + sa, pa ^ 1);
             mbar_expect_tx(a_full + sa, kHaloPitch * (kTileH + 2) * 128u);
@@ -724,8 +742,7 @@
             if (++sa == kAStages) { sa = 0; pa ^= 1; }
           }
         }
-        item += cnt; tile += cnt;
-        if (tile == tiles) { tile = 0; ++gn; }
+        next_batch(cnt);
       }
     }
   } else if (warp == 1 || (warp == 10 && p.issuers == 2)) {
@@ -740,7 +757,7 @@
     uint32_t u = 0;
     long long dbg_te = 0, dbg_af = 0, dbg_sf = 0, dbg_t0 = DBG_CLOCK(), c0;
     while (item < item_end) {
-      const int cnt = min(kBatchTiles, min(item_end - item, tiles - tile));
+      const int cnt = batch_len();
       const int bb = bcount & 1;
       const int n = gn % p.batch;
       const int gi = gn / p.batch;
@@ -832,8 +849,7 @@
       for (int j = 0; j < kBatchTiles; ++j)
         if (j < cnt) use_bits ^= 1u << (bb * kBatchTiles + j);
       ++bcount;
-      item += cnt; tile += cnt;
-      if (tile == tiles) { tile = 0; ++gn; }
+      next_batch(cnt);
     }
     DBG_ONLY(if (p.dbg != nullptr && lane == 0 && my == 0) {
       p.dbg[blockIdx.x * 8 + 0] = DBG_CLOCK() - dbg_t0;
@@ -853,7 +869,7 @@
     long long dbg_tf = 0, dbg_t0 = DBG_CLOCK();
     if (item < item_end) epiq_prefetch(p, p.g[gn / p.batch], gn / p.batch, gn % p.batch, tile, quad, lane, half, eq);
     while (item < item_end) {
-      const int cnt = min(kBatchTiles, min(item_end - item, tiles - tile));
+      const int cnt = batch_len();
       const int bb = bcount & 1;
       const int n = gn % p.batch;
       for (int j = 0; j < cnt; ++j) {
@@ -864,17 +880,16 @@
         use_bits ^= 1u << acc;
         tc_fence_after();
         const uint32_t taddr = tmem_base + (static_cast<uint32_t>(quad * 32) << 16) + static_cast<uint32_t>(acc * BN + half * 32);
-        epiq_finish(p, n, tile + j, quad, lane, half, taddr, eq, item + j + 1 >= item_end || tile + j + 1 == tiles,
+        const int tj = tile + step * j;
+        int nt = tj, ngn = gn;
+        walk_step(nt, ngn, tiles, step);
+        epiq_finish(p, n, tj, quad, lane, half, taddr, eq, item + j + 1 >= item_end || ngn != gn,
                     [&] { if (lane == 0) mbar_arrive(t_empty + acc); }, [&] {
-          if (item + j + 1 < item_end) {
-            const int nt = tile + j + 1 == tiles ? 0 : tile + j + 1, ngn = tile + j + 1 == tiles ? gn + 1 : gn;
-            epiq_prefetch(p, p.g[ngn / p.batch], ngn / p.batch, ngn % p.batch, nt, quad, lane, half, eq);
-          }
+          if (item + j + 1 < item_end) epiq_prefetch(p, p.g[ngn / p.batch], ngn / p.batch, ngn % p.batch, nt, quad, lane, half, eq);
         });
       }
       ++bcount;
-      item += cnt; tile += cnt;
-      if (tile == tiles) { tile = 0; ++gn; }
+      next_batch(cnt);
     }
     DBG_ONLY(if (p.dbg != nullptr && warp == 2 && lane == 0) {
       p.dbg[blockIdx.x * 8 + 4] = DBG_CLOCK() - dbg_t0;
@@ -1087,6 +1102,8 @@
     SAVSR_REQUIRE(g.src_channels == groups[0].src_channels && g.src_channels >= 0 && g.src_channels <= 64 && g.src_channels % 16 == 0,
                   "savsr_conv: src_channels (%d) must be 0, 16, 32, 48 or 64 and equal for all groups of a launch", g.src_channels);
     SAVSR_REQUIRE(g.act != SAVSR_ACT_LRELU || (g.slope >= 0.f && g.slope <= 1.f), "savsr_conv: group %d LeakyReLU slope %g outside [0, 1]", i, g.slope);
+    SAVSR_REQUIRE((g.reverse == 0 || g.reverse == 1) && g.reverse == groups[0].reverse,
+                  "savsr_conv: reverse (%d) must be 0 or 1 and equal for all groups of a launch", g.reverse);
     for (int s = 0; s < g.nsrc; ++s) {
       SAVSR_REQUIRE(g.src_slot[s] >= 0 && g.src_slot[s] < arena->nslots, "savsr_conv: group %d source slot %d out of range", i, g.src_slot[s]);
       SAVSR_REQUIRE(dst_mode != SAVSR_DST_ARENA || g.src_slot[s] != g.dst_slot, "savsr_conv: group %d writes slot %d that it also convolves", i, g.dst_slot);
@@ -1117,6 +1134,7 @@
   p.dbg = ctx->conv_dbg;
   p.issuers = ctx->opt[SAVSR_OPT_BIGK_ISSUERS];
   p.ksteps = groups[0].src_channels ? groups[0].src_channels / 16 : 4;
+  p.reverse = groups[0].reverse;
   if (n_tile == 64) return launch_conv<64>(ctx, p, impl, static_cast<cudaStream_t>(st));
   return launch_conv<16>(ctx, p, impl, static_cast<cudaStream_t>(st));
 }
diff --git a/savsr_b200/csrc/plan.cu b/savsr_b200/csrc/plan.cu
--- a/savsr_b200/csrc/plan.cu
+++ b/savsr_b200/csrc/plan.cu
@@ -60,10 +60,18 @@
 }
 
 extern "C" int savsr_plan_add_ca_scale_residual(savsr_plan* plan, savsr_arena* arena, int t_slot, int x_slot, int dst_slot, const float* pool,
-                                                int npart, const float* w1, const float* b1, const float* w2, const float* b2, float* y_scratch) {
+                                                int npart, const float* w1, const float* b1, const float* w2, const float* b2, float* y_scratch,
+                                                int reverse) {
   SAVSR_REQUIRE(plan && arena, "savsr_plan_add_ca_scale_residual: null pointer");
+  SAVSR_REQUIRE(reverse == 0 || reverse == 1, "savsr_plan_add_ca_scale_residual: reverse must be 0 or 1, got %d", reverse);
   savsr_ctx* ctx = plan->ctx;
-  plan->ops.push_back([=](savsr_stream st) { return savsr_ca_scale_residual(ctx, arena, t_slot, x_slot, dst_slot, pool, npart, w1, b1, w2, b2, y_scratch, st); });
+  plan->ops.push_back([=](savsr_stream st) {
+    const int prev = ctx->opt[SAVSR_OPT_CA_REVERSE];
+    ctx->opt[SAVSR_OPT_CA_REVERSE] = reverse;
+    const int rc = savsr_ca_scale_residual(ctx, arena, t_slot, x_slot, dst_slot, pool, npart, w1, b1, w2, b2, y_scratch, st);
+    ctx->opt[SAVSR_OPT_CA_REVERSE] = prev;
+    return rc;
+  });
   return 0;
 }
 
diff --git a/savsr_b200/csrc/small_ops.cu b/savsr_b200/csrc/small_ops.cu
--- a/savsr_b200/csrc/small_ops.cu
+++ b/savsr_b200/csrc/small_ops.cu
@@ -39,6 +39,16 @@
 
 __device__ __forceinline__ float sigmoidf_(float x) { return 1.f / (1.f + expf(-x)); }
 
+__device__ __forceinline__ float sum_partials(const float* src, int npart, int part, int ch) {
+  float a0 = 0.f, a1 = 0.f, a2 = 0.f, a3 = 0.f;
+  int q = part;
+  for (; q + 48 < npart; q += 64) {
+    a0 += src[q * kC + ch]; a1 += src[(q + 16) * kC + ch]; a2 += src[(q + 32) * kC + ch]; a3 += src[(q + 48) * kC + ch];
+  }
+  for (; q < npart; q += 16) a0 += src[q * kC + ch];
+  return (a0 + a1) + (a2 + a3);
+}
+
 constexpr int kOsaThreads = 1024;
 __global__ void __launch_bounds__(kOsaThreads) osa_pool_kernel(const __grid_constant__ OsaLaunch L) {
   pdl_wait();
@@ -49,11 +59,7 @@
   __shared__ float red[16][64];
   const int ch = threadIdx.x & 63, part = threadIdx.x >> 6;
   const float* src = c.pool[s] + static_cast<long>(n) * L.npart * kC;
-  float a0 = 0.f, a1 = 0.f;
-  int q = part;
-  for (; q + 16 < L.npart; q += 32) { a0 += src[q * kC + ch]; a1 += src[(q + 16) * kC + ch]; }
-  if (q < L.npart) a0 += src[q * kC + ch];
-  red[part][ch] = a0 + a1;
+  red[part][ch] = sum_partials(src, L.npart, part, ch);
   __syncthreads();
   float* vin = c.scratch + static_cast<long>(n) * osa_scratch_stride(c.ci);
   if (part == 0) {
@@ -208,6 +214,10 @@
   int npart;
   int fmt;
   long npix;
+  int batch, width, height, tiles_x, tiles;
+  int chunk;
+  int sweep;
+  int reverse;
 };
 __global__ void __launch_bounds__(1024) ca_vector_kernel(const CaParams p) {
   pdl_wait();
@@ -218,11 +228,7 @@
   const int n = blockIdx.x;
   const int ch = threadIdx.x & 63, part = threadIdx.x >> 6;
   const float* src = p.pool + static_cast<long>(n) * p.npart * kC;
-  float a0 = 0.f, a1 = 0.f;
-  int q = part;
-  for (; q + 16 < p.npart; q += 32) { a0 += src[q * kC + ch]; a1 += src[(q + 16) * kC + ch]; }
-  if (q < p.npart) a0 += src[q * kC + ch];
-  red[part][ch] = a0 + a1;
+  red[part][ch] = sum_partials(src, p.npart, part, ch);
   __syncthreads();
   if (part == 0) {
     float sum = 0.f;
@@ -244,27 +250,47 @@
     p.y[n * 64 + threadIdx.x] = sigmoidf_(a);
   }
 }
-__global__ void __launch_bounds__(256) ca_scale_residual_kernel(const CaParams p) {
+constexpr int kCaSweep = 8;
+__global__ void __launch_bounds__(256, kCaSweep) ca_scale_residual_kernel(const CaParams p) {
   pdl_wait();
   pdl_trigger();
-  __shared__ float ys[64];
-  const int n = blockIdx.y;
-  if (threadIdx.x < 64) ys[threadIdx.x] = p.y[n * 64 + threadIdx.x];
-  __syncthreads();
-  const long chunks = p.npix * 8;
-  const uint4* tt = reinterpret_cast<const uint4*>(p.t + static_cast<long>(n) * p.npix * kC);
-  const uint4* xx = reinterpret_cast<const uint4*>(p.x + static_cast<long>(n) * p.npix * kC);
-  uint4* dd = reinterpret_cast<uint4*>(p.dst + static_cast<long>(n) * p.npix * kC);
-  for (long id = blockIdx.x * static_cast<long>(blockDim.x) + threadIdx.x; id < chunks;
-       id += static_cast<long>(gridDim.x) * blockDim.x) {
-    const int c0 = (id & 7) * 8;
-    const uint4 a = tt[id], b = xx[id];
-    uint4 o;
-    o.x = pack_h2(h_lo(b.x, p.fmt) + h_lo(a.x, p.fmt) * ys[c0 + 0], h_hi(b.x, p.fmt) + h_hi(a.x, p.fmt) * ys[c0 + 1], p.fmt);
-    o.y = pack_h2(h_lo(b.y, p.fmt) + h_lo(a.y, p.fmt) * ys[c0 + 2], h_hi(b.y, p.fmt) + h_hi(a.y, p.fmt) * ys[c0 + 3], p.fmt);
-    o.z = pack_h2(h_lo(b.z, p.fmt) + h_lo(a.z, p.fmt) * ys[c0 + 4], h_hi(b.z, p.fmt) + h_hi(a.z, p.fmt) * ys[c0 + 5], p.fmt);
-    o.w = pack_h2(h_lo(b.w, p.fmt) + h_lo(a.w, p.fmt) * ys[c0 + 6], h_hi(b.w, p.fmt) + h_hi(a.w, p.fmt) * ys[c0 + 7], p.fmt);
-    dd[id] = o;
+  const int c = blockIdx.x / p.sweep, j = blockIdx.x - c * p.sweep;
+  const int item_begin = c * p.chunk;
+  const int len = min(p.chunk, p.batch * p.tiles - item_begin);
+  const int c0 = (threadIdx.x & 7) * 8;
+  for (int i = j; i < len; i += p.sweep) {
+    const int item = p.reverse ? item_begin + len - 1 - i : item_begin + i;
+    const int n = item / p.tiles, tile = item - n * p.tiles;
+    const long base = static_cast<long>(n) * p.npix * 8 + (threadIdx.x & 7);
+    const uint4* __restrict__ tt = reinterpret_cast<const uint4*>(p.t) + base;
+    const uint4* __restrict__ xx = reinterpret_cast<const uint4*>(p.x) + base;
+    uint4* __restrict__ dd = reinterpret_cast<uint4*>(p.dst) + base;
+    const float4* ys = reinterpret_cast<const float4*>(p.y + n * 64 + c0);
+    const int ty = tile / p.tiles_x;
+    const int px = (tile - ty * p.tiles_x) * kTileW + ((threadIdx.x >> 3) & (kTileW - 1));
+    const int py0 = ty * kTileH + (threadIdx.x >> 6);
+#pragma unroll
+    for (int h2 = 0; h2 < 2; ++h2) {
+      int off[2];
+      uint4 a[2], b[2];
+#pragma unroll
+      for (int r = 0; r < 2; ++r) {
+        const int py = py0 + 8 * h2 + 4 * r;
+        off[r] = (px < p.width && py < p.height) ? (py * p.width + px) * 8 : -1;
+        if (off[r] >= 0) { a[r] = tt[off[r]]; b[r] = xx[off[r]]; }
+      }
+#pragma unroll
+      for (int r = 0; r < 2; ++r) {
+        if (off[r] < 0) continue;
+        const float4 y0 = __ldg(ys), y1 = __ldg(ys + 1);
+        uint4 o;
+        o.x = pack_h2(h_lo(b[r].x, p.fmt) + h_lo(a[r].x, p.fmt) * y0.x, h_hi(b[r].x, p.fmt) + h_hi(a[r].x, p.fmt) * y0.y, p.fmt);
+        o.y = pack_h2(h_lo(b[r].y, p.fmt) + h_lo(a[r].y, p.fmt) * y0.z, h_hi(b[r].y, p.fmt) + h_hi(a[r].y, p.fmt) * y0.w, p.fmt);
+        o.z = pack_h2(h_lo(b[r].z, p.fmt) + h_lo(a[r].z, p.fmt) * y1.x, h_hi(b[r].z, p.fmt) + h_hi(a[r].z, p.fmt) * y1.y, p.fmt);
+        o.w = pack_h2(h_lo(b[r].w, p.fmt) + h_lo(a[r].w, p.fmt) * y1.z, h_hi(b[r].w, p.fmt) + h_hi(a[r].w, p.fmt) * y1.w, p.fmt);
+        dd[off[r]] = o;
+      }
+    }
   }
 }
 
@@ -581,12 +607,16 @@
   p.x = arena->base + x_slot * img;
   p.dst = arena->base + dst_slot * img;
   p.fmt = ctx->fmt; p.pool = pool; p.npart = npart; p.w1 = w1; p.b1 = b1; p.w2 = w2; p.b2 = b2; p.y = y_scratch;
-  long blocks = (p.npix * 8 + 255) / 256;
-  const long cap = 8L * ctx->sm_count / (arena->batch > 0 ? arena->batch : 1) + 1;
-  if (blocks > cap) blocks = cap;
+  p.batch = arena->batch; p.width = arena->width; p.height = arena->height;
+  p.tiles_x = arena->tiles_x; p.tiles = arena->tiles_x * arena->tiles_y;
   if (arena->batch == 0) return 0;
+  const int total = p.batch * p.tiles;
+  p.chunk = (total + ctx->sm_count - 1) / ctx->sm_count;
+  p.sweep = p.chunk < kCaSweep ? p.chunk : kCaSweep;
+  p.reverse = ctx->opt[SAVSR_OPT_CA_REVERSE];
+  const int blocks = (total + p.chunk - 1) / p.chunk * p.sweep;
   (void)launch_k(ctx->opt[SAVSR_OPT_PDL] != 0, ca_vector_kernel, dim3(arena->batch), dim3(1024), 0, static_cast<cudaStream_t>(st), p);
-  (void)launch_k(ctx->opt[SAVSR_OPT_PDL] != 0, ca_scale_residual_kernel, dim3(static_cast<unsigned>(blocks), arena->batch), dim3(256), 0, static_cast<cudaStream_t>(st), p);
+  (void)launch_k(ctx->opt[SAVSR_OPT_PDL] != 0, ca_scale_residual_kernel, dim3(blocks), dim3(256), 0, static_cast<cudaStream_t>(st), p);
   SAVSR_CUDA(cudaGetLastError());
   return 0;
 }
diff --git a/savsr_b200/engine.py b/savsr_b200/engine.py
--- a/savsr_b200/engine.py
+++ b/savsr_b200/engine.py
@@ -129,9 +129,11 @@
 
 
 class Plan:
+    serpentine: bool = True
+
     def __init__(self, params: Dict[str, torch.Tensor], batch: int, h: int, w: int, scale, device: torch.device,
                  conv_impl: str = "tap", num_frame: int = 7, taps: Optional[Sequence[str]] = None, precision: str = "bf16",
-                 store: Optional[WeightStore] = None):
+                 store: Optional[WeightStore] = None, serpentine: bool = True):
         if device.type != "cuda":
             raise K.SavsrError("savsr_b200 runs on CUDA (sm_100a) only; there is no CPU fallback")
         if num_frame != 7:
@@ -160,6 +162,7 @@
         self.graph: Optional[torch.cuda.CUDAGraph] = None
         self.store = store if store is not None else WeightStore()
         self.nbytes = 0
+        self.serpentine = serpentine
         self._pool_cache: Dict[str, int] = {}
         self._osa_cache: Dict[str, Tuple[K.OsaParams, int, int]] = {}
         self.cplan: Optional[K.CPlan] = K.CPlan(self.ctx) if hasattr(K, "CPlan") and hasattr(self.lib, "savsr_plan_create") else None
@@ -221,6 +224,15 @@
             K.check(rec(self.cplan.handle))
             self._recorded += 1
 
+    def _walk(self, reads: Sequence[int], writes: Sequence[int]) -> int:
+        rev = 0
+        if self.serpentine:
+            src = max(reads, key=lambda s: self._writer.get(s, (-1, 0))[0], default=None)
+            rev = 1 - self._writer[src][1] if src in self._writer else 0
+        for s in writes:
+            self._writer[s] = (len(self.ops), rev)
+        return rev
+
     def _group(self, src: Sequence[int], dst: int, weight: int, bias: int = 0, act: int = K.ACT_NONE, slope: float = 0.2,
                res1: int = -1, res2: int = -1, res2_scale: float = 0.0, wstride: int = 0, mask: int = 0, pool: int = 0,
                aux: int = 0, src_channels: int = 0) -> K.ConvGroup:
@@ -238,6 +250,10 @@
     def _conv(self, arena: K.Arena, groups: Sequence[K.ConvGroup], ksize: int = 3, n_tile: int = 64,
               dst_mode: int = K.DST_ARENA, alg_ci: Optional[Sequence[int]] = None, alg_co: Optional[int] = None,
               kind: Optional[str] = None) -> None:
+        rev = self._walk([g.src_slot[i] for g in groups for i in range(g.nsrc)],
+                         [g.dst_slot for g in groups] if dst_mode == K.DST_ARENA else [])
+        for g in groups:
+            g.reverse = rev
         arr = (K.ConvGroup * len(groups))(*groups)
         self._keep.append(arr)
         lib, ctx, ah, n, impl = self.lib, self.ctx.handle, arena.handle, len(groups), self.impl
@@ -331,6 +347,7 @@
         lib, ctx = self.lib, self.ctx.handle
         L = K.ACT_LRELU
         self.osa_scratch: Dict[str, torch.Tensor] = {}
+        self._writer: Dict[int, Tuple[int, int]] = {}
         nf = 64
         sl = _Slots()
         zero = sl.get()
@@ -357,6 +374,7 @@
         xin = self.x_in.data_ptr()
 
         lrh0, hh0, ww0 = lr.handle, self.h, self.w
+        self._walk([], [FR])
         self._emit(lambda st: lib.savsr_pack_frames(ctx, lrh0, xin, t, hh0, ww0, FR, st), kind="pack_frames",
                    rec=lambda cp: lib.savsr_plan_add_pack_frames(cp, lrh0, xin, t, hh0, ww0, FR))
         hpast = [zero, zero]
@@ -433,11 +451,16 @@
                 self._conv(lr, [self._group([T1], T2, self._packp(pr + ".2.weight"), self._ptr(pr + ".2.bias"), pool=pl)])
                 w1, b1 = self._ptr(pr + ".3.attention.1.weight"), self._ptr(pr + ".3.attention.1.bias")
                 w2, b2 = self._ptr(pr + ".3.attention.3.weight"), self._ptr(pr + ".3.attention.3.bias")
-                self._emit(lambda st, x=x, xa=xa, pl=pl, w1=w1, b1=b1, w2=w2, b2=b2:
-                           lib.savsr_ca_scale_residual(ctx, lrh, T2, x, xa, pl, npart, w1, b1, w2, b2, ca_y, st),
-                           launches=2, kind="ca_scale_residual",
-                           rec=lambda cp, x=x, xa=xa, pl=pl, w1=w1, b1=b1, w2=w2, b2=b2:
-                           lib.savsr_plan_add_ca_scale_residual(cp, lrh, T2, x, xa, pl, npart, w1, b1, w2, b2, ca_y))
+                rev = self._walk([T2], [xa])
+
+                def ca(st, x=x, xa=xa, pl=pl, w1=w1, b1=b1, w2=w2, b2=b2, rev=rev):
+                    lib.savsr_ctx_set_option(ctx, K.OPT_CA_REVERSE, rev)
+                    rc = lib.savsr_ca_scale_residual(ctx, lrh, T2, x, xa, pl, npart, w1, b1, w2, b2, ca_y, st)
+                    lib.savsr_ctx_set_option(ctx, K.OPT_CA_REVERSE, 0)
+                    return rc
+                self._emit(ca, launches=2, kind="ca_scale_residual",
+                           rec=lambda cp, x=x, xa=xa, pl=pl, w1=w1, b1=b1, w2=w2, b2=b2, rev=rev:
+                           lib.savsr_plan_add_ca_scale_residual(cp, lrh, T2, x, xa, pl, npart, w1, b1, w2, b2, ca_y, rev))
                 x, xa, xb = xa, xb, xa
             plr = self._pool(f"RG.{gi}.conv")
             self._conv(lr, [self._group([x], R, self._packp(f"RG.{gi}.conv.weight"), self._ptr(f"RG.{gi}.conv.bias"),
```

After: 271.3, median of 6. Within noise of the previous version (+0.2%).
